# nebula-beta/MonocularSfM

Measured on AMD Instinct MI355X. Metric: descriptor-pairs/sec (and image-pairs/sec); match-index bit-parity vs CPU, higher is better.
Workload: dtype f32

## Files before the change

### include/msfm_match.h

```cpp
#ifndef MSFM_MATCH_H
#define MSFM_MATCH_H

#include <stdint.h>

#ifdef __cplusplus
extern "C" {
#endif

#define MSFM_DIM 128
#define MSFM_MAX_IMAGES 10000

enum {
    MSFM_OK = 0,
    MSFM_E_INVALID = 1,
    MSFM_E_DEVICE = 2,
    MSFM_E_NOIMAGE = 3,
    MSFM_E_CAPACITY = 4,
    MSFM_E_STATE = 5
};

enum { MSFM_DTYPE_F32 = 0, MSFM_DTYPE_U8 = 1 };

enum {
    MSFM_ORDER_SSE4X4 = 0,
    MSFM_ORDER_AVX2_FMA = 1,
    MSFM_ORDER_AVX512_FMA = 3
};

typedef struct msfm_ctx msfm_ctx;

typedef struct msfm_match_params {
    float ratio;
    int cross_check;
    double max_distance;
} msfm_match_params;

typedef struct msfm_profile {
    double dist_kernel_ms;
    int dist_kernel_launches;
    double total_device_ms;
    int64_t descriptor_pairs;
    int64_t dist_algo_bytes;
    double approx_kernel_ms;
    int approx_kernel_launches;
    int prefilter_pairs;
    int fallback_pairs;
    int64_t candidates;
    int64_t prefilter_descriptor_pairs;
    int64_t exact_descriptor_pairs;
    int64_t tie_rows;
    double sweep2_ms;
    int sweep2_launches;
    int compacted_pairs;
    int64_t sweep2_descriptor_pairs;
    double verify_ms;
    int sub_batches;
    int tie_queue_regrows;
    int plan_regrows;
    int sweep1_i8_launches;
    int sweep1_q8_launches;
    int sweep1b_launches;
    double sweep1b_ms;
    int64_t sweep1b_descriptor_pairs;
    int64_t order_sensitive_rows;
    int demoted_pairs;
    int mixed_route_sub_batches;
    int memory_shrinks;
} msfm_profile;

int msfm_create(int device_ordinal, msfm_ctx** out_ctx);
void msfm_destroy(msfm_ctx* ctx);
const char* msfm_last_error(const msfm_ctx* ctx);
int msfm_device_info(const msfm_ctx* ctx, char* name, int name_cap, int* cu_count, int* clock_mhz);
int msfm_set_accum_order(msfm_ctx* ctx, int order);
int msfm_set_prefilter(msfm_ctx* ctx, int enable);
int msfm_get_profile(const msfm_ctx* ctx, msfm_profile* out);
int msfm_set_limits(msfm_ctx* ctx, int max_pairs_per_batch, int64_t scratch_bytes);
int msfm_set_pipeline(msfm_ctx* ctx, int min_sub_batches);

int msfm_upload_image(msfm_ctx* ctx, int image_id, const void* desc, int n, int dim, int dtype);
int msfm_subset_image(msfm_ctx* ctx, int src_image_id, int dst_image_id, const int32_t* rows, int count);
int msfm_image_rows(const msfm_ctx* ctx, int image_id, int* out_n);
int msfm_clear_images(msfm_ctx* ctx);
int msfm_finalize_store(msfm_ctx* ctx);
int msfm_store_info(const msfm_ctx* ctx, int64_t* out_device_bytes, int64_t* out_rows, int64_t* out_pending_images);

int msfm_match_pair(msfm_ctx* ctx, int id1, int id2, float ratio, int cross_check,
                    double max_distance, int32_t* out_qt, float* out_dist, int* out_count);

int msfm_match_pairs(msfm_ctx* ctx, const int32_t* pairs, int n_pairs,
                     const msfm_match_params* params, int64_t* out_offsets);
int msfm_fetch_matches(msfm_ctx* ctx, int32_t* out_qt, float* out_dist);
int msfm_fetch_order_certificate(msfm_ctx* ctx, int32_t* out_sensitive_rows);
int msfm_view_matches(msfm_ctx* ctx, const int32_t** out_qt, const float** out_dist, int64_t* out_count);
int msfm_fetch_matches_device(msfm_ctx* ctx, int32_t* d_out_qt, float* d_out_dist);

typedef struct msfm_chunk {
    int first_pair;
    int n_pairs;
    int64_t count;
    const int64_t* offsets;
    const int32_t* qt;
    const float* dist;
    const int32_t* d_qt;
    const float* d_dist;
    const int32_t* sensitive_rows;
} msfm_chunk;
struct msfm_verify_params;
int msfm_match_pairs_begin(msfm_ctx* ctx, const int32_t* pairs, int n_pairs, const msfm_match_params* params,
                           int geometric_verification, const struct msfm_verify_params* verify);
int msfm_match_pairs_next(msfm_ctx* ctx, msfm_chunk* out);
int msfm_match_pairs_end(msfm_ctx* ctx);
typedef struct msfm_memory {
    int64_t device_free, device_total;
    int64_t store, inbox, scratch, results_device;
    int64_t page_locked_host;
} msfm_memory;
int msfm_memory_info(msfm_ctx* ctx, msfm_memory* out);
int msfm_read_device(msfm_ctx* ctx, void* host_dst, const void* device_src, int64_t bytes);

typedef struct msfm_verify_params {
    double threshold;
    double confidence;
    int max_iters;
    unsigned long long seed;
} msfm_verify_params;
int msfm_upload_keypoints(msfm_ctx* ctx, int image_id, const float* kpts, int n, int stride_floats);

#define MSFM_VERIFY_FUNDAMENTAL 0
#define MSFM_VERIFY_ESSENTIAL 1
#define MSFM_VERIFY_HOMOGRAPHY 2
typedef struct msfm_camera {
    double fx, fy, cx, cy, k1, k2, p1, p2;
} msfm_camera;
int msfm_set_verification_model(msfm_ctx* ctx, int model, const msfm_camera* camera);
int msfm_get_verification_stats(const msfm_ctx* ctx, int64_t* hypotheses_solved, int* rounds);

int msfm_set_model_selection(msfm_ctx* ctx, int enable, double h_ratio);
int msfm_fetch_model_selection(msfm_ctx* ctx, int32_t* out_model, int32_t* out_n_epipolar, int32_t* out_n_homography);

typedef struct msfm_two_view_params {
    int32_t min_num_inliers;
    int32_t reserved;
    double tri_max_error;
    double tri_min_angle;
} msfm_two_view_params;
typedef struct msfm_two_view_record {
    int32_t valid;
    int32_t reserved;
    double R[9];
// ... 238 lines not shown
```

### monocularsfm_amd/_lib.py

```python
import ctypes as C
import os

import numpy as np

_HERE = os.path.dirname(os.path.abspath(__file__))
LIB_PATH = os.path.join(_HERE, "csrc", "libmsfm_match.so")
if os.environ.get("MSFM_LIBRARY"):
    LIB_PATH = os.path.abspath(os.environ["MSFM_LIBRARY"])

OK, E_INVALID, E_DEVICE, E_NOIMAGE, E_CAPACITY, E_STATE = range(6)
DTYPE_F32, DTYPE_U8 = 0, 1
ORDER_SSE4X4, ORDER_AVX2_FMA, ORDER_AVX512_FMA = 0, 1, 3
MAX_IMAGES = 10000
DIM = 128

EXPORTS = [
    "msfm_create", "msfm_destroy", "msfm_last_error", "msfm_device_info", "msfm_set_accum_order", "msfm_set_prefilter",
    "msfm_get_profile", "msfm_upload_image", "msfm_image_rows", "msfm_clear_images",
    "msfm_match_pair", "msfm_match_pairs", "msfm_fetch_matches", "msfm_knn2_pair",
    "msfm_topscale_select", "msfm_pair_id", "msfm_pair_from_id", "msfm_swap_image_pair",
    "msfm_version", "msfm_upload_keypoints", "msfm_match_pairs_verified", "msfm_subset_image", "msfm_view_matches", "msfm_set_limits", "msfm_fetch_matches_device",
    "msfm_fetch_order_certificate", "msfm_set_pipeline", "msfm_device_count", "msfm_finalize_store", "msfm_store_info",
    "msfm_match_pairs_begin", "msfm_match_pairs_next", "msfm_read_device", "msfm_memory_info", "msfm_match_pairs_end",
    "msfm_train_vocabulary", "msfm_set_vocabulary", "msfm_image_words", "msfm_retrieve_pairs", "msfm_get_retrieval_profile",
# ... 87 lines not shown
    _fields_ = [(k, C.c_int64) for k in ("images", "eligible", "refined", "rejected_by_inliers", "iterations", "observations",
                                         "points_reposed", "points_lost", "points_gained")] + \
               [(k, C.c_double) for k in ("cost_before", "cost_after", "refine_ms", "prepare_ms")]


def reposed(points):
    return (np.asarray(points)["status"] & TRI_REPOSED) != 0


def succeeded(points):
    want = TRI_POINT | TRI_ERROR_OK | TRI_ANGLE_OK
    return (np.asarray(points)["status"] & want) == want


REG_ATTEMPTED, REG_POSE, REG_SUCCEEDED, REG_REFINED = 1, 2, 4, 8
REGISTRATION = np.dtype([("image_id", "<i4"), ("status", "<i4"), ("n_correspondences", "<i4"), ("n_inliers", "<i4"), ("hypotheses", "<i4"),
                         ("reserved", "<i4"), ("R", "<f8", (9,)), ("t", "<f8", (3,)), ("mean_residual", "<f8")])


class RegisterParams(C.Structure):
    _fields_ = [("max_error", C.c_double), ("confidence", C.c_double), ("max_iters", C.c_int32), ("min_inliers", C.c_int32),
                ("refine_iters", C.c_int32), ("reserved", C.c_int32)]


class RegisterStats(C.Structure):
    _fields_ = [("images", C.c_int32), ("attempted", C.c_int32), ("succeeded", C.c_int32), ("rounds", C.c_int32),
                ("correspondences", C.c_int64), ("hypotheses", C.c_int64), ("device_bytes", C.c_int64), ("register_ms", C.c_double)]


def registered(records):
    return (np.asarray(records)["status"] & REG_SUCCEEDED) != 0


def registered_poses(records, poses=None):
    out = dict(poses) if poses else {}
    for r in np.asarray(records)[registered(records)]:
        out[int(r["image_id"])] = (r["R"].reshape(3, 3).copy(), r["t"].copy())
    return out


def camera_struct(camera):
    keys = ("fx", "fy", "cx", "cy", "k1", "k2", "p1", "p2")
    vals = [camera.get(k, 0.0) for k in keys] if isinstance(camera, dict) else list(camera) + [0.0] * (8 - len(camera))
    return Camera(*[float(v) for v in vals[:8]])


def pose_table(poses):
    ids = np.asarray(sorted(int(i) for i in poses), np.int32)
    tab = np.zeros(max(len(ids), 1), POSE_RT)
    for k, i in enumerate(ids):
        if poses[int(i)] is None:
            continue
        R, t = poses[int(i)]
        tab[k]["valid"] = 1
        tab[k]["R"] = np.asarray(R, np.float64).reshape(9)
        tab[k]["t"] = np.asarray(t, np.float64).reshape(3)
    return ids, tab[:len(ids)]


class MatchParams(C.Structure):
    _fields_ = [("ratio", C.c_float), ("cross_check", C.c_int), ("max_distance", C.c_double)]


class Camera(C.Structure):
    _fields_ = [(k, C.c_double) for k in ("fx", "fy", "cx", "cy", "k1", "k2", "p1", "p2")]


class VerifyParams(C.Structure):
    _fields_ = [("threshold", C.c_double), ("confidence", C.c_double), ("max_iters", C.c_int), ("seed", C.c_ulonglong)]


class Profile(C.Structure):
    _fields_ = [("dist_kernel_ms", C.c_double), ("dist_kernel_launches", C.c_int),
                ("total_device_ms", C.c_double), ("descriptor_pairs", C.c_int64),
                ("dist_algo_bytes", C.c_int64), ("approx_kernel_ms", C.c_double),
                ("approx_kernel_launches", C.c_int), ("prefilter_pairs", C.c_int), ("fallback_pairs", C.c_int),
                ("candidates", C.c_int64), ("prefilter_descriptor_pairs", C.c_int64),
                ("exact_descriptor_pairs", C.c_int64), ("tie_rows", C.c_int64),
                ("sweep2_ms", C.c_double), ("sweep2_launches", C.c_int), ("compacted_pairs", C.c_int),
                ("sweep2_descriptor_pairs", C.c_int64), ("verify_ms", C.c_double),
                ("sub_batches", C.c_int), ("tie_queue_regrows", C.c_int), ("plan_regrows", C.c_int),
                ("sweep1_i8_launches", C.c_int), ("sweep1_q8_launches", C.c_int), ("sweep1b_launches", C.c_int),
                ("sweep1b_ms", C.c_double), ("sweep1b_descriptor_pairs", C.c_int64), ("order_sensitive_rows", C.c_int64),
                ("demoted_pairs", C.c_int), ("mixed_route_sub_batches", C.c_int), ("memory_shrinks", C.c_int)]


class Chunk(C.Structure):
    _fields_ = [("first_pair", C.c_int), ("n_pairs", C.c_int), ("count", C.c_int64), ("offsets", C.POINTER(C.c_int64)),
                ("qt", C.POINTER(C.c_int32)), ("dist", C.POINTER(C.c_float)), ("d_qt", C.c_void_p), ("d_dist", C.c_void_p),
                ("sensitive_rows", C.POINTER(C.c_int32))]


class Memory(C.Structure):
    _fields_ = [(k, C.c_int64) for k in ("device_free", "device_total", "store", "inbox", "scratch", "results_device", "page_locked_host")]


class RetrievalParams(C.Structure):
    _fields_ = [("num_words", C.c_int), ("train_iters", C.c_int), ("train_rows", C.c_int64)]


class RetrievalProfile(C.Structure):
    _fields_ = [("train_ms", C.c_double), ("train_iterations", C.c_int), ("assign_ms", C.c_double), ("score_ms", C.c_double),
                ("topk_ms", C.c_double), ("rows", C.c_int64), ("num_words", C.c_int)]


class MsfmError(RuntimeError):
    def __init__(self, code, msg):
        super().__init__("msfm error %d: %s" % (code, msg))
        self.code = code


_lib = None


def load():
    global _lib
    if _lib is not None:
        return _lib
    if not os.path.exists(LIB_PATH):
        raise ImportError(
            "%s is missing: the HIP extension is not built. Run `python -c 'import __graft_entry__ as g; "
            "g.build()'` (or `make -C monocularsfm_amd/csrc`). There is no CPU fallback." % LIB_PATH)
    L = C.CDLL(LIB_PATH)
    vp, ip, fp = C.c_void_p, C.POINTER(C.c_int32), C.POINTER(C.c_float)
    L.msfm_create.argtypes = [C.c_int, C.POINTER(vp)]
    L.msfm_destroy.argtypes = [vp]
    L.msfm_destroy.restype = None
    L.msfm_last_error.argtypes = [vp]
    L.msfm_last_error.restype = C.c_char_p
    L.msfm_device_info.argtypes = [vp, C.c_char_p, C.c_int, C.POINTER(C.c_int), C.POINTER(C.c_int)]
    L.msfm_set_accum_order.argtypes = [vp, C.c_int]
    L.msfm_set_prefilter.argtypes = [vp, C.c_int]
    L.msfm_get_profile.argtypes = [vp, C.POINTER(Profile)]
    L.msfm_set_limits.argtypes = [vp, C.c_int, C.c_int64]
    L.msfm_set_pipeline.argtypes = [vp, C.c_int]
    L.msfm_upload_image.argtypes = [vp, C.c_int, vp, C.c_int, C.c_int, C.c_int]
    L.msfm_image_rows.argtypes = [vp, C.c_int, C.POINTER(C.c_int)]
    L.msfm_subset_image.argtypes = [vp, C.c_int, C.c_int, ip, C.c_int]
    L.msfm_clear_images.argtypes = [vp]
    try:
        L.msfm_finalize_store.argtypes = [vp]
        L.msfm_store_info.argtypes = [vp, C.POINTER(C.c_int64), C.POINTER(C.c_int64), C.POINTER(C.c_int64)]
        L.msfm_match_pairs_begin.argtypes = [vp, ip, C.c_int, C.POINTER(MatchParams), C.c_int, C.POINTER(VerifyParams)]
        L.msfm_match_pairs_next.argtypes = [vp, C.POINTER(Chunk)]
        L.msfm_read_device.argtypes = [vp, vp, vp, C.c_int64]
        L.msfm_memory_info.argtypes = [vp, C.POINTER(Memory)]
        L.msfm_match_pairs_end.argtypes = [vp]
    except AttributeError:
        pass
    L.msfm_match_pair.argtypes = [vp, C.c_int, C.c_int, C.c_float, C.c_int, C.c_double, ip, fp, C.POINTER(C.c_int)]
    L.msfm_match_pairs.argtypes = [vp, ip, C.c_int, C.POINTER(MatchParams), C.POINTER(C.c_int64)]
    L.msfm_fetch_matches.argtypes = [vp, ip, fp]
    L.msfm_view_matches.argtypes = [vp, C.POINTER(ip), C.POINTER(fp), C.POINTER(C.c_int64)]
    L.msfm_fetch_matches_device.argtypes = [vp, vp, vp]
    L.msfm_fetch_order_certificate.argtypes = [vp, ip]
    L.msfm_upload_keypoints.argtypes = [vp, C.c_int, fp, C.c_int, C.c_int]
    L.msfm_match_pairs_verified.argtypes = [vp, ip, C.c_int, C.POINTER(MatchParams), C.POINTER(VerifyParams),
                                            C.POINTER(C.c_int64)]
    L.msfm_knn2_pair.argtypes = [vp, C.c_int, C.c_int, ip, fp, fp, ip, fp, fp]
    L.msfm_topscale_select.argtypes = [fp, C.c_int, C.c_int, ip, C.POINTER(C.c_int)]
    L.msfm_pair_id.argtypes = [C.c_int, C.c_int, ip]
    L.msfm_pair_from_id.argtypes = [C.c_int32, C.POINTER(C.c_int), C.POINTER(C.c_int)]
    L.msfm_swap_image_pair.argtypes = [C.c_int, C.c_int]
    L.msfm_version.restype = C.c_char_p
    try:
        L.msfm_device_count.argtypes = []
        L.msfm_device_count.restype = C.c_int
# ... 540 lines not shown
```

### monocularsfm_amd/csrc/msfm_batch.hip.h

```cpp
#pragma once
namespace {
struct Batch {
    std::vector<PairDesc> pairs;
    std::vector<PfPair> pf;
    std::vector<int> id1, id2;
    std::vector<int> item_base;
    size_t n_items = 0, items_per_xcd = 0;
    long long rp_elems = 0, cp_elems = 0, kf_elems = 0, kr_elems = 0, out_elems = 0, cand_elems = 0;
    int max_npad = 0;
    int64_t desc_pairs = 0;
    int64_t algo_bytes = 0;
    MsfmRoute route;
    std::vector<CandList> dense_lists;
    std::vector<VerifyPair> verify_pairs;
};

void build_items(Batch& b, int path, const std::vector<char>* only = nullptr, std::vector<int>* base_out = nullptr, size_t* per_out = nullptr) {
    std::vector<int> order(b.pairs.size());
    for (size_t p = 0; p < order.size(); ++p) order[p] = (int)p;
    if (b.id2.size() == b.pairs.size())
        std::stable_sort(order.begin(), order.end(), [&](int x, int y) { return b.id2[(size_t)x] < b.id2[(size_t)y]; });
    std::vector<int>& base = base_out ? *base_out : b.item_base;
    base.assign(b.pairs.size(), -1);
    long long n = 0;
// ... 67 lines not shown
    pp.b_c = b.c;
    const bool scales_ok = a.nrm_max <= 8.f * b.nrm_max && b.nrm_max <= 8.f * a.nrm_max;
    pp.use = (ctx->prefilter && pd.valid && a.pf_safe && b.pf_safe && scales_ok) ? 1 : 0;
    pd.path = pp.use;
    return MSFM_OK;
}

int prepare_batch_images(msfm_ctx* ctx, Batch& b, const PruneParams& prune) {
    const size_t P = b.pairs.size();
    std::vector<MsfmRoutePair> rp(P);
    for (size_t p = 0; p < P; ++p) {
        const Image &ia = ctx->images[(size_t)b.id1[p]], &ib = ctx->images[(size_t)b.id2[p]];
        rp[p] = MsfmRoutePair{b.pairs[p].valid != 0, b.pf[p].use != 0, ia.is_u8, ib.is_u8, ia.q8 != nullptr, ib.q8 != nullptr, b.pairs[p].n1, b.pairs[p].n2};
    }
    b.route = msfm_route(ctx->route_knobs(), prune.prune, prune.ratio, rp);
    std::vector<int> wide, panel;
    for (size_t p = 0; p < P; ++p) {
        if (!b.pairs[p].valid) continue;
        const bool brute = !b.pf[p].use || b.pairs[p].path == 0;
        if (brute || b.route.kind != kRouteI8) {
            wide.push_back(b.id1[p]);
            wide.push_back(b.id2[p]);
        }
        if (brute) {
            panel.push_back(b.id1[p]);
            panel.push_back(b.id2[p]);
        }
    }
    auto uniq = [](std::vector<int>& v) {
        std::sort(v.begin(), v.end());
        v.erase(std::unique(v.begin(), v.end()), v.end());
    };
    uniq(wide);
    uniq(panel);
    bool need = false;
    for (int id : wide) need |= ctx->images[(size_t)id].n > 0 && !ctx->images[(size_t)id].rawp;
    for (int id : panel) need |= ctx->images[(size_t)id].n > 0 && (!ctx->images[(size_t)id].panel || ctx->images[(size_t)id].panel_order != ctx->order);
    if (need) {
        const int rc = ensure_forms(ctx, wide, panel);
        if (rc != MSFM_OK) return rc;
    }
    for (size_t p = 0; p < P; ++p) {
        const Image& ia = ctx->images[(size_t)b.id1[p]];
        const Image& ib = ctx->images[(size_t)b.id2[p]];
        PairDesc& pd = b.pairs[p];
        PfPair& pp = b.pf[p];
        pd.a_panel = ia.panel;
        pd.b_panel = ib.panel;
        pd.a_rawp = ia.rawp;
        pd.b_rawp = ib.rawp;
        pp.a_h = ia.h16;
        pp.b_h = ib.h16;
        pp.a_nrm = ia.nrm;
        pp.b_nrm = ib.nrm;
    }
    return MSFM_OK;
}

void assign_common(Batch& b) {
    for (auto& pd : b.pairs) {
        pd.kf_off = b.kf_elems;
        pd.kr_off = b.kr_elems;
        pd.out_off = b.out_elems;
        if (!pd.valid) continue;
        b.kf_elems += pd.n1pad;
        b.kr_elems += pd.n2pad;
        b.out_elems += pd.n1;
        b.desc_pairs += (int64_t)pd.n1 * pd.n2;
        b.algo_bytes += ((int64_t)pd.n1 + pd.n2) * kDim * 4 + ((int64_t)pd.n1 + pd.n2) * 12;
        b.max_npad = std::max(b.max_npad, std::max(pd.n1pad, pd.n2pad));
    }
    for (auto& pd : b.pairs) pd.kr_off += b.kf_elems;
}

void assign_partials(Batch& b, int path, int target_items) {
    b.rp_elems = b.cp_elems = 0;
    long long total_ablocks = 0;
    for (auto& pd : b.pairs)
        if (pd.valid && pd.path == path) total_ablocks += (path == 1 ? pd.a_blocks256 : pd.a_blocks);
    const int rmult = 1;
    for (auto& pd : b.pairs) {
        if (!pd.valid || pd.path != path) continue;
        pd.ranges = 1;
        if (total_ablocks > 0 && total_ablocks < target_items) {
            long long r = (target_items + total_ablocks - 1) / total_ablocks;
            pd.ranges = (int)std::max<long long>(1, std::min<long long>(r, pd.b_tiles));
        }
        pd.rp_off = b.rp_elems;
        pd.cp_off = b.cp_elems;
        b.rp_elems += (long long)pd.ranges * rmult * pd.n1pad;
        b.cp_elems += (long long)(path == 1 ? pd.a_blocks256 : pd.a_blocks) * pd.n2pad;
    }
}

hipEvent_t get_event(msfm_ctx* ctx, size_t i) {
    while (ctx->ev_pool.size() <= i) {
        hipEvent_t e;
        if (hipEventCreate(&e) != hipSuccess) return nullptr;
        ctx->ev_pool.push_back(e);
    }
    return ctx->ev_pool[i];
}

__global__ void fill_segs_kernel(FillSegs segs) {
    MSFM_TAIL_PRIO();
    const unsigned long long tid = (unsigned long long)blockIdx.x * blockDim.x + threadIdx.x, nt = (unsigned long long)gridDim.x * blockDim.x;
    for (int k = 0; k < segs.n; ++k) {
        const FillSeg e = segs.s[k];
        const unsigned w = e.value * 0x01010101u;
        const unsigned long long n16 = e.bytes >> 4;
        uint4* p16 = reinterpret_cast<uint4*>(e.p);
        for (unsigned long long i = tid; i < n16; i += nt) p16[i] = make_uint4(w, w, w, w);
        for (unsigned long long i = (n16 << 4) + tid; i < e.bytes; i += nt) reinterpret_cast<unsigned char*>(e.p)[i] = (unsigned char)e.value;
    }
}

struct FillBatch {
    FillSegs segs = {};
    unsigned long long bytes = 0;
    std::vector<FillSegs> full;
    void add(void* p, size_t n, unsigned value) {
        if (!p || n == 0) return;
        if (segs.n == kFillSegs) {
            full.push_back(segs);
            segs = FillSegs{};
        }
        segs.s[segs.n++] = FillSeg{p, (unsigned long long)n, value & 255u};
        bytes += n;
    }
    hipError_t launch(hipStream_t stream) {
        if (segs.n) full.push_back(segs);
        const unsigned grid = (unsigned)std::max<unsigned long long>(1, std::min<unsigned long long>(256, (bytes + 65535) / 65536));
        for (const FillSegs& f : full) hipLaunchKernelGGL(fill_segs_kernel, dim3(grid), dim3(256), 0, stream, f);
        full.clear();
        segs = FillSegs{};
        bytes = 0;
        return hipGetLastError();
    }
};

int upload_pair_tables(msfm_ctx* ctx, Batch& b, int path, const std::vector<PfPair>* pfq, FillBatch& fills, const std::vector<PfPair>* pf16 = nullptr,
                       const std::vector<int>* item_base16 = nullptr, size_t per16 = 0) {
    const size_t P = b.pairs.size();
    const int slot = path == 1 ? 0 : 2;
    UploadPlan up;
    up.add(SC.d_pairs, b.pairs.data(), P * sizeof(PairDesc));
    up.add(SC.d_pf, b.pf.data(), P * sizeof(PfPair));
    if (pfq) up.add(SC.d_pfq, pfq->data(), P * sizeof(PfPair));
    if (pf16) up.add(SC.d_pf16, pf16->data(), P * sizeof(PfPair));
    if (item_base16) up.add(SC.d_item_base16, item_base16->data(), item_base16->size() * 4);
    up.add(SC.d_item_base, b.item_base.data(), b.item_base.size() * 4);
    HIPCHK(ctx, up.place_and_copy(SC.d_up[slot], SC.h_up[slot], SC.stream));
    HIPCHK(ctx, SC.d_items.ensure(std::max<size_t>(1, b.n_items) * sizeof(WorkItem)));
    fills.add(SC.d_items.p, b.n_items * sizeof(WorkItem), 0xff);
    if (item_base16 && per16) {
        HIPCHK(ctx, SC.d_items16.ensure(per16 * 8 * sizeof(WorkItem)));
        fills.add(SC.d_items16.p, per16 * 8 * sizeof(WorkItem), 0xff);
    }
    HIPCHK(ctx, fills.launch(SC.stream));
    if (b.n_items == 0) return MSFM_OK;
    hipLaunchKernelGGL(build_items_kernel, dim3((unsigned)P), dim3(64), 0, SC.stream, (const PairDesc*)SC.d_pairs.as<PairDesc>(),
                       (const int*)SC.d_item_base.as<int>(), path, (int)b.items_per_xcd, SC.d_items.as<WorkItem>());
    HIPCHK(ctx, hipGetLastError());
    if (item_base16 && per16) {
        hipLaunchKernelGGL(build_items_kernel, dim3((unsigned)P), dim3(64), 0, SC.stream, (const PairDesc*)SC.d_pairs.as<PairDesc>(),
                           (const int*)SC.d_item_base16.as<int>(), path, (int)per16, SC.d_items16.as<WorkItem>());
        HIPCHK(ctx, hipGetLastError());
    }
    return MSFM_OK;
}

struct CompactPlan {
    std::vector<PlanGroup> groups;
    std::vector<int> member_group;
    std::vector<int> gmembers;
    std::vector<int> member_pair;
    std::vector<PlanPair> ppair;
    long long rows_ub = 0;
    long long rows_ub_all_bits = 0;
    int pairs = 0;
};

void build_compact_plan(msfm_ctx* ctx, const Batch& b, CompactPlan& cp, bool no_ranges) {
    const size_t P = b.pairs.size();
    cp.ppair.assign(P, PlanPair{-1, 0, 0, 0});
    static thread_local std::vector<int> dense;
    dense.assign((size_t)kSlots, -1);
    std::vector<int> img_slot;
    auto dense_of = [&](int slot) {
        if (dense[(size_t)slot] < 0) {
            dense[(size_t)slot] = (int)img_slot.size();
            img_slot.push_back(slot);
        }
        return dense[(size_t)slot];
    };
    std::vector<int> fwd_group_of_img, rev_group0_of_img;
    std::vector<int>& member_group = cp.member_group;
    for (size_t p = 0; p < P; ++p) {
        const PairDesc& pd = b.pairs[p];
        const PfPair& pp = b.pf[p];
        if (!pd.valid || !pp.use) continue;
        ++cp.pairs;
        const int di = dense_of(b.id1[p]), dj = dense_of(b.id2[p]);
        const size_t need = img_slot.size();
        if (fwd_group_of_img.size() < need) {
            fwd_group_of_img.resize(need, -1);
            rev_group0_of_img.resize(need, -1);
        }
        if (fwd_group_of_img[(size_t)dj] < 0) {
            fwd_group_of_img[(size_t)dj] = (int)cp.groups.size();
            PlanGroup g = {};
            g.b_h = pp.b_h;
            g.b_nrm = pp.b_nrm;
            g.b_c = pp.b_c;
            g.a_c = pp.a_c;
            g.b_h0 = pp.b_h0;
            g.b_n2 = pp.b_n2;
            g.dir = 0;
            g.bt_begin = 0;
            g.bt_end = pd.b_tiles;
            g.n2 = pd.n2;
            g.n2pad = pd.n2pad;
            g.b_tiles = pd.b_tiles;
            g.ranges = 1;
            cp.groups.push_back(g);
        }
        cp.ppair[p].fwd_member = (int)cp.member_pair.size();
        cp.member_pair.push_back((int)p);
        member_group.push_back(fwd_group_of_img[(size_t)dj]);
        cp.rows_ub += pd.n1;
        const int nb = pd.a_blocks256, gshift = (nb + 31) / 32, bits = (nb + gshift - 1) / gshift;
        if (rev_group0_of_img[(size_t)di] < 0) {
            rev_group0_of_img[(size_t)di] = (int)cp.groups.size();
            for (int bit = 0; bit < bits; ++bit) {
                PlanGroup g = {};
                g.b_h = pp.a_h;
                g.b_nrm = pp.a_nrm;
                g.b_c = pp.a_c;
                g.a_c = pp.b_c;
                g.b_h0 = pp.a_h0;
                g.b_n2 = pp.a_n2;
                g.dir = 1;
                g.bt_begin = std::min(pd.a_blocks, bit * gshift * (kPfWgRows / kBM));
                g.bt_end = std::min(pd.a_blocks, (bit + 1) * gshift * (kPfWgRows / kBM));
                g.n2 = pd.n1;
                g.n2pad = pd.n1pad;
                g.b_tiles = pd.a_blocks;
                g.ranges = 1;
                cp.groups.push_back(g);
            }
        }
        cp.ppair[p].rev_member0 = (int)cp.member_pair.size();
        cp.ppair[p].rev_bits = bits;
        for (int bit = 0; bit < bits; ++bit) {
            cp.member_pair.push_back((int)p);
            member_group.push_back(rev_group0_of_img[(size_t)di] + bit);
        }
        cp.rows_ub += pd.n2;
        cp.rows_ub_all_bits += (long long)pd.n1 + (long long)pd.n2 * bits;
    }
    const size_t G = cp.groups.size(), M = cp.member_pair.size();
    for (size_t m = 0; m < M; ++m) cp.groups[(size_t)member_group[m]].count += 1;
    int at = 0;
    for (size_t g = 0; g < G; ++g) {
        cp.groups[g].first = at;
        at += cp.groups[g].count;
        cp.groups[g].count = 0;
    }
    cp.gmembers.assign(M, 0);
    for (size_t m = 0; m < M; ++m) {
        PlanGroup& g = cp.groups[(size_t)member_group[m]];
        cp.gmembers[(size_t)(g.first + g.count++)] = (int)m;
    }
    const long long target = 4LL * ctx->cu_count;
    if ((long long)G < target && !no_ranges)
        for (PlanGroup& g : cp.groups) {
            const long long r = (target + (long long)G - 1) / (long long)G;
            g.ranges = (int)std::max<long long>(1, std::min<long long>(r, g.bt_end - g.bt_begin));
        }
}

constexpr size_t kHsTotals = 2 * sizeof(PlanSummary), kHsOverflow = kHsTotals + 16;

struct PrefilterLaunch {
    msfm_ctx* ctx;
    Batch& b;
    size_t ev_base;
    PruneParams prune;
    size_t P = 0;
    HostClock hc;
    const MsfmRoute& route;
    std::vector<PfPair> pfq, pf16;
    long long dense_cand = 0;
    std::vector<int> item_base16;
    size_t per16 = 0;
    long long kn = 1;
    hipEvent_t e0 = nullptr, e1 = nullptr, e2 = nullptr, e3 = nullptr;
    dim3 block, mgrid;
    unsigned sweep_grid = 8;
    const PairDesc* dp = nullptr;
    const PfPair* dpf = nullptr;
    float* tuv = nullptr;
    unsigned* colmask = nullptr;
    size_t n_lists = 0;
    const CandList* dl = nullptr;
    CompactPlan cp;
    size_t G = 0, M = 0;
    long long rows_cap = 0, cand_cap = 0, items_cap = 0;
    const PlanPair* dpp = nullptr;
    PlanCounts pc = {};
    PlanOut po = {};

    PrefilterLaunch(msfm_ctx* c, Batch& batch, size_t ev, PruneParams pr) : ctx(c), b(batch), ev_base(ev), prune(pr), route(batch.route) {}

    int apply_route() {
        P = b.pairs.size();
        hc = HostClock();
        SC.pf_pending = PfPending{};
        assign_partials(b, 1, 4 * ctx->cu_count);
        SC.prof.demoted_pairs += route.demoted_pairs;
        SC.pf_pending.refine = route.kind == kRouteQ8Refine;
        dense_cand = 0;
        for (size_t p = 0; p < P; ++p) {
            b.pf[p].tu_off = b.pairs[p].kf_off;
            b.pf[p].tv_off = b.pairs[p].kr_off;
            b.pf[p].cand_off = 0;
            b.pf[p].cand_cap = 0;
            if (!route.compact() && b.pairs[p].valid && b.pf[p].use) {
                b.pf[p].cand_off = dense_cand;
                b.pf[p].cand_cap = 16 * (b.pairs[p].n1 + b.pairs[p].n2) + 2048;
                dense_cand += b.pf[p].cand_cap;
                SC.pf_pending.dense_swept += (long long)b.pairs[p].n1pad * b.pairs[p].n2;
            }
        }
        pfq.clear(), pf16.clear();
        if (route.q8()) pfq = b.pf;
        for (size_t p = 0; p < P && (route.kind == kRouteI8 || route.q8()); ++p) {
            if (!b.pairs[p].valid || !b.pf[p].use) continue;
            PfPair& pp = route.q8() ? pfq[p] : b.pf[p];
            pp.use = route.q8() ? route.twin[p] : 1;
            if (!pp.use) continue;
            const Image &ia = ctx->images[b.id1[p]], &ib = ctx->images[b.id2[p]];
            pp.i8 = 1;
            if (route.q8()) {
                pp.a_h = reinterpret_cast<const _Float16*>(ia.q8);
                pp.b_h = reinterpret_cast<const _Float16*>(ib.q8);
                pp.a_nrm = ia.nrm_q8, pp.b_nrm = ib.nrm_q8;
                pp.a_c = ia.err_q8_max, pp.b_c = ib.err_q8_max;
                pp.a_h0 = ia.h0_q8, pp.b_h0 = ib.h0_q8;
                pp.a_err = ia.err_q8, pp.b_err = ib.err_q8;
            } else {
                pp.a_h = reinterpret_cast<const _Float16*>(ia.i8);
                pp.b_h = reinterpret_cast<const _Float16*>(ib.i8);
                pp.a_nrm = ia.nrm_i8, pp.b_nrm = ib.nrm_i8;
                pp.a_nrm_max = ia.nrm_i8_max, pp.b_nrm_max = ib.nrm_i8_max;
                pp.a_c = pp.b_c = 0.f;
                pp.a_h0 = ia.h0_i8, pp.b_h0 = ib.h0_i8;
                pp.a_n2 = ia.n2_i8, pp.b_n2 = ib.n2_i8;
            }
        }
        if (route.kind == kRouteQ8Mixed) {
            pf16 = b.pf;
            for (size_t p = 0; p < P; ++p)
                if (route.twin[p]) pf16[p].use = 0, b.pairs[p].cp_off *= 2;
        }
        return MSFM_OK;
    }

    int build_and_upload() {
        item_base16.clear();
        per16 = 0;
        build_items(b, 1);
        if (b.n_items == 0) return MSFM_OK;
        if (route.kind == kRouteQ8Mixed) {
            std::vector<char> only(P, 0);
            for (size_t p = 0; p < P; ++p) only[p] = (b.pairs[p].valid && b.pf[p].use && !route.twin[p]) ? 1 : 0;
            build_items(b, 1, &only, &item_base16, &per16);
    }
    kn = std::max<long long>(1, b.kf_elems + b.kr_elems);
    HIPCHK(ctx, SC.d_rp_s0.ensure(std::max<long long>(1, b.rp_elems) * 4));
    HIPCHK(ctx, SC.d_rp_s1.ensure(std::max<long long>(1, b.rp_elems) * 4));
    HIPCHK(ctx, SC.d_cp_s0.ensure(std::max<long long>(1, b.cp_elems) * ((route.kind == kRouteI8 || route.kind == kRouteQ8Direct) ? 4 : 8)));
    HIPCHK(ctx, SC.d_tu.ensure(kn * 4));
    HIPCHK(ctx, SC.d_colmask.ensure(kn * 4));
    HIPCHK(ctx, SC.d_best.ensure(kn * 8));
    HIPCHK(ctx, SC.d_second.ensure(kn * 8));
    HIPCHK(ctx, SC.d_overflow.ensure(P));
    HIPCHK(ctx, SC.d_totals.ensure(128));
    FillBatch fills;
    if (!route.compact()) {
        fills.add(SC.d_best.p, (size_t)kn * 8, 0xff);
        fills.add(SC.d_second.p, (size_t)kn * 8, 0xff);
    }
    fills.add(SC.d_totals.p, 128, 0);
    fills.add(SC.d_overflow.p, P, 0);
    const int rc = upload_pair_tables(ctx, b, 1, route.q8() ? &pfq : nullptr, fills, route.kind == kRouteQ8Mixed ? &pf16 : nullptr,
                                        route.kind == kRouteQ8Mixed ? &item_base16 : nullptr, per16);
    if (rc != MSFM_OK) return rc;
    return MSFM_OK;
    }

    int launch_sweep1() {
        e0 = get_event(ctx, ev_base), e1 = get_event(ctx, ev_base + 1);
        e2 = get_event(ctx, ev_base + 2), e3 = get_event(ctx, ev_base + 3);
        if (!e0 || !e1 || !e2 || !e3) return fail(ctx, MSFM_E_DEVICE, "hipEventCreate failed");
        block = dim3(kPfThreads);
        sweep_grid = (unsigned)std::max(8, (ctx->cu_count / 8) * 8);
        dp = SC.d_pairs.as<PairDesc>();
        dpf = SC.d_pf.as<PfPair>();
        tuv = SC.d_tu.as<float>();
        colmask = SC.d_colmask.as<unsigned>();
        hc.lap("sweep-1 setup + uploads");
        if (ctx->last_sweep1 && ctx->last_sweep1 != ctx->cur)
            HIPCHK(ctx, hipStreamWaitEvent(SC.stream, ctx->last_sweep1->sweep1_done, 0));
        for (Scratch& other : ctx->sc)
            if (&other != ctx->cur && other.sweep2_recorded && other.seq + 2 <= SC.seq)
                HIPCHK(ctx, hipStreamWaitEvent(SC.stream, other.sweep2_done, 0));
        HIPCHK(ctx, hipEventRecord(e0, SC.stream));
        if (route.kind == kRouteI8 || route.q8())
            hipLaunchKernelGGL(sweep_i8_kernel<1>, dim3(std::min<unsigned>(sweep_grid, (unsigned)b.n_items)), dim3(kI8Threads), kI8LdsBytes, SC.stream, dp,
                               route.q8() ? (const PfPair*)SC.d_pfq.as<PfPair>() : dpf,
                               SC.d_items.as<WorkItem>(), SC.d_rp_s0.as<float>(), SC.d_rp_s1.as<float>(), SC.d_cp_s0.as<float>(),
                               (const float*)nullptr, (int2*)nullptr, (unsigned long long*)nullptr, (const int*)nullptr, (int)b.n_items, (int*)nullptr,
                               (int*)nullptr);
        else
            hipLaunchKernelGGL(sweep_kernel<1>, dim3(std::min<unsigned>(sweep_grid, (unsigned)b.n_items)), block, kPfLdsBytes, SC.stream, dp, dpf,
                               SC.d_items.as<WorkItem>(), SC.d_rp_s0.as<float>(), SC.d_rp_s1.as<float>(),
                               SC.d_cp_s0.as<float>(), (float*)nullptr, (const float*)nullptr, (const float*)nullptr,
                               (int2*)nullptr, (unsigned long long*)nullptr, (const int*)nullptr, (int)b.n_items, (int*)nullptr);
        HIPCHK(ctx, hipGetLastError());
        if (route.kind == kRouteQ8Mixed && per16) {
            hipLaunchKernelGGL(sweep_kernel<1>, dim3(std::min<unsigned>(sweep_grid, (unsigned)(per16 * 8))), block, kPfLdsBytes, SC.stream, dp,
                               (const PfPair*)SC.d_pf16.as<PfPair>(), SC.d_items16.as<WorkItem>(), SC.d_rp_s0.as<float>(), SC.d_rp_s1.as<float>(),
                               SC.d_cp_s0.as<float>(), (float*)nullptr, (const float*)nullptr, (const float*)nullptr,
                               (int2*)nullptr, (unsigned long long*)nullptr, (const int*)nullptr, (int)(per16 * 8), (int*)nullptr);
            HIPCHK(ctx, hipGetLastError());
            SC.prof.mixed_route_sub_batches += 1;
    }
    DBGSYNC(ctx, "sweep_kernel<1>");
    HIPCHK(ctx, hipEventRecord(e1, SC.stream));
    HIPCHK(ctx, hipEventRecord(SC.sweep1_done, SC.stream));
    SC.sweep1_recorded = true;
    ctx->last_sweep1 = ctx->cur;
    SC.prof.approx_kernel_launches += 1;
    if (route.kind == kRouteI8 || route.q8()) SC.prof.sweep1_i8_launches += 1;
    if (route.q8()) SC.prof.sweep1_q8_launches += 1;
    mgrid = dim3((unsigned)((b.max_npad + 255) / 256), (unsigned)P);
    if (!route.compact()) {
        hipLaunchKernelGGL(pf_thresholds_kernel, mgrid, dim3(256), 0, SC.stream, dp, dpf, SC.d_rp_s0.as<float>(),
                           SC.d_rp_s1.as<float>(), SC.d_cp_s0.as<float>(), (unsigned*)nullptr, tuv, tuv, prune, PlanCounts{}, 0);
        HIPCHK(ctx, hipGetLastError());
        DBGSYNC(ctx, "pf_thresholds_kernel");
    }
    hc.lap("launch sweep 1 (+ thresholds)");
    return MSFM_OK;
    }

    int plan_buffers() {
        cp = CompactPlan{};
        const bool refine = route.kind == kRouteQ8Refine;
        build_compact_plan(ctx, b, cp, refine);
        G = cp.groups.size(), M = cp.member_pair.size();
        n_lists = G;
        long long max_ranges = 1;
        for (const PlanGroup& g : cp.groups) max_ranges = std::max<long long>(max_ranges, g.ranges);
        const long long ub = refine ? cp.rows_ub_all_bits : cp.rows_ub;
        long long rows_have = (long long)std::min(std::min(SC.d_cmp_tu.cap / 4, SC.d_live_idx.cap / 4), std::min(SC.d_row_pair.cap / 4, SC.d_row_src.cap / 8));
        if (route.kind == kRouteI8) rows_have = std::min<long long>(rows_have, (long long)(SC.d_cmp_n2.cap / 4));
        if (refine) rows_have = std::min<long long>(rows_have, (long long)std::min(SC.d_cmp_s0.cap / 4, SC.d_cmp_s1.cap / 4));
        long long cand_have = (long long)(SC.d_cand.cap / sizeof(int2));
        if (route.kind == kRouteI8) cand_have = std::min<long long>(cand_have, (long long)(SC.d_cand_val.cap / 4));
        const long long items_have = (long long)(SC.d_vitems.cap / sizeof(WorkItem)) / 8 * 8;
        const MsfmPlanRoom room = msfm_plan_room(ub, refine ? cp.rows_ub_all_bits * 5 / 32 : cp.rows_ub * 5 / 16, (long long)G, max_ranges, kPfWgRows,
                                                 ctx->hint_rows_ub, ctx->cmp_rows_hint, ctx->cand_hint, ctx->items_hint, rows_have, cand_have, items_have);
        rows_cap = room.rows, cand_cap = room.cand, items_cap = room.items;
        SC.pf_pending.rows_ub = ub;
        HIPCHK(ctx, SC.d_gtot.ensure(std::max<size_t>(1, G) * 4));
        HIPCHK(ctx, SC.d_grow0.ensure((4 * std::max<size_t>(1, G) + 8) * 8));
        HIPCHK(ctx, SC.d_cnt.ensure(std::max<size_t>(1, M) * 4));
        HIPCHK(ctx, SC.d_mrow.ensure(std::max<size_t>(1, M) * 8));
        HIPCHK(ctx, SC.d_summary.ensure(sizeof(PlanSummary)));
        HIPCHK(ctx, SC.d_vpairs.ensure(std::max<size_t>(1, G) * sizeof(PairDesc)));
        HIPCHK(ctx, SC.d_vpf.ensure(std::max<size_t>(1, G) * sizeof(PfPair)));
        HIPCHK(ctx, SC.d_lists.ensure(std::max<size_t>(1, G) * sizeof(CandList)));
        HIPCHK(ctx, SC.d_vitems.ensure((size_t)items_cap * sizeof(WorkItem)));
        HIPCHK(ctx, SC.d_cmp_tu.ensure((size_t)rows_cap * 4));
        HIPCHK(ctx, SC.d_live_idx.ensure((size_t)rows_cap * 4));
        HIPCHK(ctx, SC.d_row_pair.ensure((size_t)rows_cap * 4));
        HIPCHK(ctx, SC.d_row_src.ensure((size_t)rows_cap * 8));
        HIPCHK(ctx, SC.d_cand.ensure((size_t)cand_cap * sizeof(int2)));
        if (route.kind == kRouteI8) {
            HIPCHK(ctx, SC.d_cand_val.ensure((size_t)cand_cap * 4));
            HIPCHK(ctx, SC.d_cmp_n2.ensure((size_t)rows_cap * 4));
        }
        HIPCHK(ctx, SC.d_cand_count.ensure(std::max<size_t>(1, G) * 8));
        {
            UploadPlan up;
            up.add(SC.d_groups, cp.groups.data(), G * sizeof(PlanGroup));
            up.add(SC.d_gmembers, cp.gmembers.data(), M * 4);
            up.add(SC.d_member_pair, cp.member_pair.data(), M * 4);
            up.add(SC.d_member_group, cp.member_group.data(), M * 4);
            up.add(SC.d_ppair, cp.ppair.data(), P * sizeof(PlanPair));
            HIPCHK(ctx, up.place_and_copy(SC.d_up[1], SC.h_up[1], SC.stream));
            FillBatch fb;
            fb.add(SC.d_gtot.p, std::max<size_t>(1, G) * 4, 0);
            fb.add(SC.d_cnt.p, std::max<size_t>(1, M) * 4, 0);
            fb.add(SC.d_vpairs.p, std::max<size_t>(1, G) * sizeof(PairDesc), 0);
            fb.add(SC.d_vpf.p, std::max<size_t>(1, G) * sizeof(PfPair), 0);
            fb.add(SC.d_lists.p, std::max<size_t>(1, G) * sizeof(CandList), 0);
            fb.add(SC.d_summary.p, sizeof(PlanSummary), 0);
            fb.add(SC.d_vitems.p, (size_t)items_cap * sizeof(WorkItem), 0xff);
            fb.add(SC.d_row_src.p, (size_t)rows_cap * 8, 0);
            fb.add(SC.d_cand_count.p, std::max<size_t>(1, G) * 8, 0);
            HIPCHK(ctx, fb.launch(SC.stream));
        }
        hc.lap("plan tables + uploads");
        dpp = SC.d_ppair.as<PlanPair>();
        pc = PlanCounts{dpp, (const int*)SC.d_member_group.as<int>(), SC.d_cnt.as<int>(), SC.d_gtot.as<int>()};
        HIPCHK(ctx, SC.d_summary_a.ensure(sizeof(PlanSummary)));
        po = PlanOut{};
        po.vpairs = SC.d_vpairs.as<PairDesc>();
        po.vpf = SC.d_vpf.as<PfPair>();
        po.lists = SC.d_lists.as<CandList>();
        po.items = SC.d_vitems.as<WorkItem>();
        po.grow0 = SC.d_grow0.as<long long>();
        po.gpos = SC.d_grow0.as<long long>() + std::max<size_t>(1, G);
        po.fwd_items_x = SC.d_grow0.as<long long>() + 4 * std::max<size_t>(1, G);
        po.summary = SC.d_summary.as<PlanSummary>();
        po.row_src = SC.d_row_src.as<const _Float16*>();
        po.zero_row = ctx->d_zero_row.as<_Float16>();
        po.live_idx = SC.d_live_idx.as<int>();
        po.row_pair = SC.d_row_pair.as<int>();
        po.rows_cap = rows_cap;
        po.cand_cap = cand_cap;
        po.items_cap = items_cap;
        po.cmp_tu = SC.d_cmp_tu.as<float>();
        po.cmp_n2 = route.kind == kRouteI8 ? SC.d_cmp_n2.as<int>() : nullptr;
        return MSFM_OK;
    }

    int launch_plan(PlanSummary* summary, int norms_only) {
        po.summary = summary;
        hipLaunchKernelGGL(pf_plan_scan_kernel, dim3(1), dim3(64), 0, SC.stream, SC.d_groups.as<PlanGroup>(), (int)G,
                           (const int*)SC.d_gtot.as<int>(), po);
        HIPCHK(ctx, hipGetLastError());
        DBGSYNC(ctx, "pf_plan_scan_kernel");
        if (G > 0)
            hipLaunchKernelGGL(pf_plan_write_kernel, dim3((unsigned)((G + 63) / 64)), dim3(64), 0, SC.stream, SC.d_groups.as<PlanGroup>(), (int)G,
                               (const int*)SC.d_gtot.as<int>(), po);
        HIPCHK(ctx, hipGetLastError());
        DBGSYNC(ctx, "pf_plan_write_kernel");
        if (G > 0)
            hipLaunchKernelGGL(pf_member_rows_kernel, dim3((unsigned)((G + 3) / 4)), dim3(256), 0, SC.stream, SC.d_groups.as<PlanGroup>(), (int)G,
                               (const int*)SC.d_gmembers.as<int>(), (const int*)SC.d_cnt.as<int>(),
                               (const long long*)SC.d_grow0.as<long long>(), SC.d_mrow.as<long long>());
        HIPCHK(ctx, hipGetLastError());
        DBGSYNC(ctx, "pf_member_rows_kernel");
        hipLaunchKernelGGL(pf_assign_kernel, dim3((unsigned)(2 * P), (unsigned)((b.max_npad + kAssignChunk - 1) / kAssignChunk)), dim3(256), 0,
                           SC.stream, dp, dpf, dpp, (const float*)tuv,
                           (const unsigned*)colmask, (const long long*)SC.d_mrow.as<long long>(), SC.d_cnt.as<int>(),
                           SC.d_live_idx.as<int>(), SC.d_row_pair.as<int>(), SC.d_cmp_tu.as<float>(),
                           SC.d_row_src.as<const _Float16*>(), route.kind == kRouteI8 ? kI8RowBytes / 2 : kPfRowHalfs,
                           SC.d_best.as<unsigned long long>(), SC.d_second.as<unsigned long long>(), norms_only,
                           route.kind == kRouteI8 ? SC.d_cmp_n2.as<int>() : (int*)nullptr);
        HIPCHK(ctx, hipGetLastError());
        DBGSYNC(ctx, "pf_assign_kernel");
        return MSFM_OK;
    }

    int launch_route_q() {
        hipLaunchKernelGGL(pf_prune_q8_kernel, mgrid, dim3(256), 0, SC.stream, dp, dpf, (const PfPair*)SC.d_pfq.as<PfPair>(),
                           (const float*)SC.d_rp_s0.as<float>(), (const float*)SC.d_rp_s1.as<float>(), (const float*)SC.d_cp_s0.as<float>(),
                           colmask, tuv, prune, pc, ctx->q8_level / 255.f, route.kind == kRouteQ8Refine ? 0 : 1);
        HIPCHK(ctx, hipGetLastError());
        DBGSYNC(ctx, "pf_prune_q8_kernel");
        if (route.kind == kRouteQ8Refine) {
            HIPCHK(ctx, hipMemsetAsync(SC.d_summary_a.p, 0, sizeof(PlanSummary), SC.stream));
            int rc = launch_plan(SC.d_summary_a.as<PlanSummary>(), 1);
            if (rc != MSFM_OK) return rc;
            HIPCHK(ctx, SC.d_cmp_s0.ensure((size_t)rows_cap * 4));
            HIPCHK(ctx, SC.d_cmp_s1.ensure((size_t)rows_cap * 4));
            hipEvent_t e4 = get_event(ctx, ev_base + 6), e5 = get_event(ctx, ev_base + 7);
            if (!e4 || !e5) return fail(ctx, MSFM_E_DEVICE, "hipEventCreate failed");
            HIPCHK(ctx, hipEventRecord(e4, SC.stream));
            hipLaunchKernelGGL(sweep_kernel<4>, dim3(sweep_grid), block, kPfLdsBytes, SC.stream,
                               (const PairDesc*)SC.d_vpairs.as<PairDesc>(), (const PfPair*)SC.d_vpf.as<PfPair>(),
                               (const WorkItem*)SC.d_vitems.as<WorkItem>(), SC.d_cmp_s0.as<float>(), SC.d_cmp_s1.as<float>(), (float*)nullptr,
                               (float*)nullptr, (const float*)SC.d_cmp_tu.as<float>(), (const float*)nullptr, (int2*)nullptr,
                               (unsigned long long*)nullptr, (const int*)&SC.d_summary_a.as<PlanSummary>()->n_items, 0,
                               SC.d_totals.as<int>() + 8);
            HIPCHK(ctx, hipGetLastError());
            DBGSYNC(ctx, "sweep_kernel<4>");
            HIPCHK(ctx, hipEventRecord(e5, SC.stream));
            SC.prof.sweep1b_launches += 1;
            if (G > 0)
                hipLaunchKernelGGL(q8_scatter_kernel, dim3(16, (unsigned)std::min<size_t>(G, 65535)), dim3(256), 0, SC.stream, dp,
                                   (const PairDesc*)SC.d_vpairs.as<PairDesc>(), (const CandList*)SC.d_lists.as<CandList>(),
                                   (const PlanGroup*)SC.d_groups.as<PlanGroup>(), (int)G, (const long long*)SC.d_grow0.as<long long>(),
                                   (const float*)SC.d_cmp_s0.as<float>(), (const float*)SC.d_cmp_s1.as<float>(),
                                   SC.d_rp_s0.as<float>(), SC.d_rp_s1.as<float>(), SC.d_cp_s0.as<float>());
            HIPCHK(ctx, hipGetLastError());
            DBGSYNC(ctx, "q8_scatter_kernel");
            FillBatch fb;
            fb.add(SC.d_gtot.p, std::max<size_t>(1, G) * 4, 0);
            fb.add(SC.d_cnt.p, std::max<size_t>(1, M) * 4, 0);
            fb.add(SC.d_vpairs.p, std::max<size_t>(1, G) * sizeof(PairDesc), 0);
            fb.add(SC.d_vpf.p, std::max<size_t>(1, G) * sizeof(PfPair), 0);
            fb.add(SC.d_lists.p, std::max<size_t>(1, G) * sizeof(CandList), 0);
            fb.add(SC.d_vitems.p, (size_t)items_cap * sizeof(WorkItem), 0xff);
            fb.add(SC.d_row_src.p, (size_t)rows_cap * 8, 0);
            fb.add(SC.d_totals.p, 64, 0);
            HIPCHK(ctx, fb.launch(SC.stream));
        }
        return MSFM_OK;
    }

    int launch_compact_sweep2() {
        if (route.kind != kRouteQ8Direct)
            hipLaunchKernelGGL(pf_thresholds_kernel, mgrid, dim3(256), 0, SC.stream, dp, route.kind == kRouteQ8Mixed ? (const PfPair*)SC.d_pf16.as<PfPair>() : dpf,
                               SC.d_rp_s0.as<float>(), SC.d_rp_s1.as<float>(), SC.d_cp_s0.as<float>(), colmask, tuv, tuv, prune, pc,
                               route.kind == kRouteQ8Refine ? 1 : 0);
        HIPCHK(ctx, hipGetLastError());
        DBGSYNC(ctx, "pf_thresholds_kernel");
        const int rc = launch_plan(SC.d_summary.as<PlanSummary>(), 0);
        if (rc != MSFM_OK) return rc;
        HIPCHK(ctx, hipEventRecord(e2, SC.stream));
        if (route.kind == kRouteI8)
            hipLaunchKernelGGL(sweep_i8_kernel<3>, dim3(sweep_grid), dim3(kI8Threads), kI8LdsBytes3, SC.stream,
                               (const PairDesc*)SC.d_vpairs.as<PairDesc>(), (const PfPair*)SC.d_vpf.as<PfPair>(),
                               (const WorkItem*)SC.d_vitems.as<WorkItem>(), (float*)nullptr, (float*)nullptr, (float*)nullptr,
                               (const float*)SC.d_cmp_tu.as<float>(), SC.d_cand.as<int2>(),
                               SC.d_cand_count.as<unsigned long long>(), (const int*)&SC.d_summary.as<PlanSummary>()->n_items, 0,
                               SC.d_totals.as<int>() + 8, SC.d_cand_val.as<int>());
        else
            hipLaunchKernelGGL(sweep_kernel<3>, dim3(sweep_grid), block, kPfLdsBytes, SC.stream,
                               (const PairDesc*)SC.d_vpairs.as<PairDesc>(), (const PfPair*)SC.d_vpf.as<PfPair>(),
                               (const WorkItem*)SC.d_vitems.as<WorkItem>(), (float*)nullptr, (float*)nullptr, (float*)nullptr,
                               (float*)nullptr, (const float*)SC.d_cmp_tu.as<float>(), (const float*)nullptr, SC.d_cand.as<int2>(),
                               SC.d_cand_count.as<unsigned long long>(), (const int*)&SC.d_summary.as<PlanSummary>()->n_items, 0,
                               SC.d_totals.as<int>() + 8);
        HIPCHK(ctx, hipGetLastError());
        DBGSYNC(ctx, "sweep_kernel<3>");
        SC.prof.sweep2_launches += 1;
        HIPCHK(ctx, hipEventRecord(e3, SC.stream));
        HIPCHK(ctx, hipEventRecord(SC.sweep2_done, SC.stream));
        SC.sweep2_recorded = true;
        dl = SC.d_lists.as<CandList>();
        SC.pf_pending.compact = true;
        SC.pf_pending.rows_cap = rows_cap;
        SC.pf_pending.cand_cap = cand_cap;
        SC.pf_pending.items_cap = items_cap;
        SC.pf_pending.compact_pairs = cp.pairs;
        return MSFM_OK;
    }

    int launch_dense_sweep2() {
        n_lists = P;
        std::vector<CandList>& lists = b.dense_lists;
        lists.resize(P);
        for (size_t p = 0; p < P; ++p)
            lists[p] = CandList{(int)p, 0, b.pf[p].cand_off, b.pf[p].cand_cap, 0, nullptr, nullptr};
        HIPCHK(ctx, SC.d_cand.ensure(std::max<long long>(1, dense_cand) * sizeof(int2)));
        HIPCHK(ctx, SC.d_cand_count.ensure(P * 8));
        HIPCHK(ctx, SC.d_lists.ensure(P * sizeof(CandList)));
        HIPCHK(ctx, hipMemsetAsync(SC.d_cand_count.p, 0, P * 8, SC.stream));
        HIPCHK(ctx, hipMemcpyAsync(SC.d_lists.p, lists.data(), P * sizeof(CandList), hipMemcpyHostToDevice, SC.stream));
        HIPCHK(ctx, hipEventRecord(e2, SC.stream));
        hipLaunchKernelGGL(sweep_kernel<2>, dim3(std::min<unsigned>(sweep_grid, (unsigned)b.n_items)), block, kPfLdsBytes, SC.stream, dp, dpf,
                           SC.d_items.as<WorkItem>(), (float*)nullptr, (float*)nullptr, (float*)nullptr, (float*)nullptr,
                           (const float*)tuv, (const float*)tuv, SC.d_cand.as<int2>(), SC.d_cand_count.as<unsigned long long>(),
                           (const int*)nullptr, (int)b.n_items, (int*)nullptr);
        HIPCHK(ctx, hipGetLastError());
        DBGSYNC(ctx, "sweep_kernel<2>");
        SC.prof.sweep2_launches += 1;
        HIPCHK(ctx, hipEventRecord(e3, SC.stream));
        HIPCHK(ctx, hipEventRecord(SC.sweep2_done, SC.stream));
        SC.sweep2_recorded = true;
        dl = SC.d_lists.as<CandList>();
        return MSFM_OK;
    }

    int launch_exact_and_finalize() {
        if (n_lists > 0) {
            const int wgs_per_xcd = std::max(1, ctx->cu_count / 8) * 8;
            const dim3 cgrid((unsigned)(8 * wgs_per_xcd));
            const unsigned long long* dcount = SC.d_cand_count.as<unsigned long long>();
#define MSFM_LAUNCH_EXACT(O)                                                                                             \
        hipLaunchKernelGGL(pf_exact_candidates_kernel<O>, cgrid, dim3(kExSpan), 0, SC.stream, dp, dl, dcount,                  \
                           (const int2*)SC.d_cand.as<int2>(), SC.d_best.as<unsigned long long>(), SC.d_second.as<unsigned long long>(), \
                           (int)n_lists, SC.d_totals.as<int>() + 16, (const int*)SC.d_cand_val.as<int>(), 0)
            if (route.kind == kRouteI8) MSFM_LAUNCH_EXACT(4);
            else if (ctx->order == MSFM_ORDER_SSE4X4) MSFM_LAUNCH_EXACT(0);
            else if (ctx->order == MSFM_ORDER_AVX2_FMA) MSFM_LAUNCH_EXACT(1);
            else MSFM_LAUNCH_EXACT(3);
#undef MSFM_LAUNCH_EXACT
            HIPCHK(ctx, hipGetLastError());
            DBGSYNC(ctx, "pf_exact_candidates_kernel");
    }
    if (!SC.keys_epilogue) {
        hipLaunchKernelGGL(pf_finalize_kernel, mgrid, dim3(256), 0, SC.stream, dp, dpf, (const float*)tuv, SC.d_best.as<unsigned long long>(),
                           SC.d_second.as<unsigned long long>(), SC.d_k_i0.as<int>(), SC.d_k_d0.as<float>(),
                           SC.d_k_d1.as<float>(), SC.d_fix_count.as<int>(), SC.d_fix_list.as<int4>(), SC.fix_cap_eff);
        HIPCHK(ctx, hipGetLastError());
        DBGSYNC(ctx, "pf_finalize_kernel");
    }
    if (n_lists > 0) {
        hipLaunchKernelGGL(pf_overflow_kernel, dim3((unsigned)((n_lists + 255) / 256)), dim3(256), 0, SC.stream, dl, (int)n_lists,
                           (const unsigned long long*)SC.d_cand_count.as<unsigned long long>(), (const PlanGroup*)SC.d_groups.as<PlanGroup>(),
                           (const int*)SC.d_gmembers.as<int>(), (const int*)SC.d_member_pair.as<int>(),
                           SC.d_overflow.as<unsigned char>(), SC.d_totals.as<unsigned long long>());
        HIPCHK(ctx, hipGetLastError());
    }
    SC.pf_pending.active = true;
    SC.pf_pending.n_lists = n_lists;
    SC.pf_pending.P = P;
    SC.pf_pending.ev_base = ev_base;
    hc.lap("launch sweep 2 .. finalize");
    return MSFM_OK;
    }

    int run() {
        int rc = apply_route();
        if (rc != MSFM_OK) return rc;
        rc = build_and_upload();
        if (rc != MSFM_OK || b.n_items == 0) return rc;
        rc = launch_sweep1();
        if (rc != MSFM_OK) return rc;
        if (route.compact()) {
            rc = plan_buffers();
            if (rc == MSFM_OK && route.q8()) rc = launch_route_q();
            if (rc == MSFM_OK) rc = launch_compact_sweep2();
        } else {
            rc = launch_dense_sweep2();
        }
        if (rc != MSFM_OK) return rc;
        return launch_exact_and_finalize();
    }
};

int run_prefilter(msfm_ctx* ctx, Batch& b, size_t ev_base, PruneParams prune) {
    PrefilterLaunch launch(ctx, b, ev_base, prune);
    return launch.run();
}

int finish_prefilter(msfm_ctx* ctx, Batch& b, std::vector<char>& force_exact, bool* retry) {
    *retry = false;
    PfPending& pe = SC.pf_pending;
    if (!pe.active) return MSFM_OK;
    pe.active = false;
    const char* hs = SC.h_summary.as<char>();
    PlanSummary sm = {};
    unsigned long long totals[2] = {0, 0};
    std::memcpy(totals, hs + kHsTotals, 16);
    float ms = 0.f;
    HIPCHK(ctx, hipEventElapsedTime(&ms, ctx->ev_pool[pe.ev_base], ctx->ev_pool[pe.ev_base + 1]));
    SC.prof.approx_kernel_ms += ms;
    HIPCHK(ctx, hipEventElapsedTime(&ms, ctx->ev_pool[pe.ev_base + 2], ctx->ev_pool[pe.ev_base + 3]));
    SC.prof.sweep2_ms += ms;
    if (std::getenv("MSFM_DEBUG_TIMING") && pe.compact) {
        PlanSummary d;
        std::memcpy(&d, hs, sizeof(PlanSummary));
        std::fprintf(stderr, "[msfm plan] ok %d, items %lld (room for %lld), compacted rows %lld (%lld; of at most %lld), candidate entries %lld (%lld), swept descriptor pairs %lld; sweep 1 %.3f ms, sweep 2 %.3f ms\n",
                     d.ok, d.items_needed, pe.items_cap, d.cmp_rows, pe.rows_cap, pe.rows_ub, d.cand_elems, pe.cand_cap, d.swept_desc_pairs, SC.prof.approx_kernel_ms, ms);
    }
    if (pe.compact) {
        std::memcpy(&sm, hs, sizeof(PlanSummary));
        ctx->cmp_rows_hint = sm.cmp_rows;
        ctx->items_hint = sm.items_needed;
        ctx->cand_hint = sm.cand_elems;
        ctx->hint_rows_ub = pe.rows_ub;
        if (pe.refine) {
            PlanSummary sa;
            std::memcpy(&sa, hs + sizeof(PlanSummary), sizeof(PlanSummary));
            ctx->cmp_rows_hint = std::max(ctx->cmp_rows_hint, sa.cmp_rows);
            ctx->items_hint = std::max(ctx->items_hint, sa.items_needed);
            ctx->cand_hint = std::max(ctx->cand_hint, sa.cand_elems);
            if (!sa.ok) sm.ok = 0;
            float ms1b = 0.f;
            HIPCHK(ctx, hipEventElapsedTime(&ms1b, ctx->ev_pool[pe.ev_base + 6], ctx->ev_pool[pe.ev_base + 7]));
            SC.prof.sweep1b_ms += ms1b;
            SC.prof.sweep1b_descriptor_pairs += sa.swept_desc_pairs;
        }
        if (!sm.ok) {
            SC.prof.plan_regrows += 1;
            *retry = true;
            return MSFM_OK;
        }
        SC.prof.sweep2_descriptor_pairs += sm.swept_desc_pairs;
    } else {
        SC.prof.sweep2_descriptor_pairs += pe.dense_swept;
    }
    const unsigned char* ov = reinterpret_cast<const unsigned char*>(hs + kHsOverflow);
    int n_over = 0;
    for (size_t p = 0; p < pe.P; ++p) {
        if (!b.pairs[p].valid || !b.pf[p].use) continue;
        if (ov[p]) {
            force_exact[p] = 1;
            ++n_over;
        }
    }
    if (n_over > 0) {
        SC.prof.fallback_pairs += n_over;
        *retry = true;
        return MSFM_OK;
    }
    SC.prof.candidates += (int64_t)totals[0];
    for (size_t p = 0; p < pe.P; ++p)
        if (b.pairs[p].valid && b.pf[p].use) {
            SC.prof.prefilter_pairs += 1;
            SC.prof.prefilter_descriptor_pairs += (int64_t)b.pairs[p].n1 * b.pairs[p].n2;
        }
    if (pe.compact) SC.prof.compacted_pairs += pe.compact_pairs;
    return MSFM_OK;
}

int run_exact(msfm_ctx* ctx, Batch& b, size_t ev_base) {
    const size_t P = b.pairs.size();
    assign_partials(b, 0, 4 * ctx->cu_count);
    build_items(b, 0);
    if (b.n_items == 0) return MSFM_OK;
    HIPCHK(ctx, SC.d_rp_s0.ensure(std::max<long long>(1, b.rp_elems) * 4));
    HIPCHK(ctx, SC.d_rp_i0.ensure(std::max<long long>(1, b.rp_elems) * 4));
    HIPCHK(ctx, SC.d_rp_s1.ensure(std::max<long long>(1, b.rp_elems) * 4));
    HIPCHK(ctx, SC.d_cp_s0.ensure(std::max<long long>(1, b.cp_elems) * 4));
    HIPCHK(ctx, SC.d_cp_i0.ensure(std::max<long long>(1, b.cp_elems) * 4));
    HIPCHK(ctx, SC.d_cp_s1.ensure(std::max<long long>(1, b.cp_elems) * 4));
    FillBatch fills;
    int rc = upload_pair_tables(ctx, b, 0, nullptr, fills);
    if (rc != MSFM_OK) return rc;
    hipEvent_t e0 = get_event(ctx, ev_base), e1 = get_event(ctx, ev_base + 1);
    if (!e0 || !e1) return fail(ctx, MSFM_E_DEVICE, "hipEventCreate failed");
    if (ctx->last_sweep1 && ctx->last_sweep1 != ctx->cur)
        HIPCHK(ctx, hipStreamWaitEvent(SC.stream, ctx->last_sweep1->sweep1_done, 0));
    HIPCHK(ctx, hipEventRecord(e0, SC.stream));
    const dim3 grid((unsigned)b.n_items), block(kThreads);
#define MSFM_LAUNCH_DIST(O)                                                                                               \
    hipLaunchKernelGGL(dist_top2_kernel<O>, grid, block, (O) == 3 ? kLdsBytesIdxStash : kLdsBytes, SC.stream, SC.d_pairs.as<PairDesc>(), SC.d_items.as<WorkItem>(), \
                       SC.d_rp_s0.as<float>(), SC.d_rp_i0.as<int>(), SC.d_rp_s1.as<float>(), SC.d_cp_s0.as<float>(),             \
                       SC.d_cp_i0.as<int>(), SC.d_cp_s1.as<float>())
    if (ctx->order == MSFM_ORDER_SSE4X4) MSFM_LAUNCH_DIST(0);
    else if (ctx->order == MSFM_ORDER_AVX2_FMA) MSFM_LAUNCH_DIST(1);
    else MSFM_LAUNCH_DIST(3);
#undef MSFM_LAUNCH_DIST
    HIPCHK(ctx, hipGetLastError());
    HIPCHK(ctx, hipEventRecord(e1, SC.stream));
    HIPCHK(ctx, hipEventRecord(SC.sweep1_done, SC.stream));
    SC.sweep1_recorded = true;
    ctx->last_sweep1 = ctx->cur;
    SC.prof.dist_kernel_launches += 1;
    for (auto& pd : b.pairs)
        if (pd.valid && pd.path == 0) SC.prof.exact_descriptor_pairs += (int64_t)pd.n1 * pd.n2;
    const dim3 mgrid((unsigned)((b.max_npad + 255) / 256), (unsigned)P);
    hipLaunchKernelGGL(merge_knn_kernel, mgrid, dim3(256), 0, SC.stream, SC.d_pairs.as<PairDesc>(),
                       SC.d_rp_s0.as<float>(), SC.d_rp_i0.as<int>(), SC.d_rp_s1.as<float>(),
                       SC.d_cp_s0.as<float>(), SC.d_cp_i0.as<int>(), SC.d_cp_s1.as<float>(),
                       SC.d_k_i0.as<int>(), SC.d_k_d0.as<float>(), SC.d_k_d1.as<float>(),
                       SC.d_fix_count.as<int>(), SC.d_fix_list.as<int4>(), SC.fix_cap_eff);
    HIPCHK(ctx, hipGetLastError());
    return MSFM_OK;
}

int run_knn(msfm_ctx* ctx, Batch& b, size_t ev_base, bool* exact_launched, PruneParams prune, bool need_fix, bool lists_only) {
    assign_common(b);
    SC.fix_cap_eff = need_fix ? ctx->fix_cap : 0;
    const long long kn = std::max<long long>(1, b.kf_elems + b.kr_elems);
    HIPCHK(ctx, SC.d_fix_count.ensure(4));
    HIPCHK(ctx, SC.d_fix_list.ensure((size_t)ctx->fix_cap * sizeof(int4)));
    HIPCHK(ctx, hipMemsetAsync(SC.d_fix_count.p, 0, 4, SC.stream));
    bool any_pf = false, any_exact = false;
    for (auto& pd : b.pairs) any_pf |= (pd.valid && pd.path == 1);
    for (auto& pd : b.pairs) any_exact |= (pd.valid && pd.path == 0);
// ... 105 lines not shown
```

### monocularsfm_amd/csrc/msfm_ctx.hip.h

```cpp
#pragma once
namespace {

struct AllocClock {
    double dev_ms = 0, pin_ms = 0, free_ms = 0;
    long long dev_bytes = 0, pin_bytes = 0;
    int dev_n = 0, pin_n = 0, free_n = 0;
    static double now() { return std::chrono::duration<double, std::milli>(std::chrono::steady_clock::now().time_since_epoch()).count(); }
};
inline AllocClock& alloc_clock() {
    static thread_local AllocClock c;
    return c;
}
inline hipError_t timed_malloc(void** p, size_t bytes) {
    const double t0 = AllocClock::now();
    const hipError_t e = hipMalloc(p, bytes);
    AllocClock& c = alloc_clock();
    c.dev_ms += AllocClock::now() - t0;
    c.dev_bytes += (long long)bytes;
    c.dev_n += 1;
    return e;
}
inline void timed_free(void* p) {
    const double t0 = AllocClock::now();
    (void)hipFree(p);
// ... 361 lines not shown
            if (!chunks[i].base) slot = (int)i;
        if (slot < 0) {
            chunks.push_back(StoreChunk{});
            slot = (int)chunks.size() - 1;
        }
        StoreChunk& c = chunks[(size_t)slot];
        const size_t want = std::max(bytes, min_chunk);
        hipError_t e = timed_malloc((void**)&c.base, want);
        if (e != hipSuccess) {
            c.base = nullptr;
            return e;
        }
        c.cap = want;
        c.used = 0;
        c.live = 0;
        cur = slot;
        return hipSuccess;
    }
    void* take(size_t bytes, int* chunk) {
        StoreChunk& c = chunks[(size_t)cur];
        const size_t at = (c.used + 255) & ~(size_t)255;
        if (at + bytes > c.cap) return nullptr;
        c.used = at + bytes;
        c.live += 1;
        *chunk = cur;
        return c.base + at;
    }
    void free_chunk(int i) {
        StoreChunk& c = chunks[(size_t)i];
        if (c.base) (void)hipFree(c.base);
        c = StoreChunk{};
        if (cur == i) cur = -1;
    }
    void drop(int& chunk) {
        if (chunk < 0) return;
        StoreChunk& c = chunks[(size_t)chunk];
        if (--c.live <= 0) {
            if (chunk == cur || recycle) c.used = 0, c.live = 0;
            else free_chunk(chunk);
        }
        chunk = -1;
    }
    size_t bytes() const {
        size_t s = 0;
        for (const StoreChunk& c : chunks) s += c.cap;
        return s;
    }
    void release_all() {
        for (size_t i = 0; i < chunks.size(); ++i) free_chunk((int)i);
        chunks.clear();
        cur = -1;
    }
};

constexpr int kSlots = 2 * MSFM_MAX_IMAGES + 2;
constexpr long long kDefaultScratchBytes = (long long)64 << 30;
constexpr int kDefaultMaxPairsPerBatch = 16384;
constexpr int kMaxPairsPerBatchLimit = 65535;
constexpr int kDefaultPipeline = 2;
constexpr double kDefaultTaper = 1.0;
constexpr int kInFlight = 3;
constexpr long long kMinPipelineCost = 15000000000LL;

}

struct PfPending {
    bool active = false, compact = false, refine = false;
    size_t n_lists = 0, P = 0;
    long long rows_cap = 0, cand_cap = 0, items_cap = 0;
    long long rows_ub = 0;
    int compact_pairs = 0;
    long long dense_swept = 0;
    size_t ev_base = 0;
};

struct Scratch {
    hipStream_t stream = nullptr;
    DevBuf d_up[3];
    PinnedBuf h_up[3];
    Ref d_pairs, d_pf, d_pfq, d_pf16, d_item_base, d_item_base16;
    Ref d_groups, d_gmembers, d_member_pair, d_member_group, d_ppair;
    DevBuf d_items;
    DevBuf d_rp_s0, d_rp_i0, d_rp_s1, d_cp_s0, d_cp_i0, d_cp_s1;
    DevBuf d_k_i0, d_k_d0, d_k_d1;
    DevBuf d_st_qt, d_st_d, d_counts, d_offsets, d_sens;
    DevBuf d_sub_qt, d_sub_d;
    PinnedBuf h_sub_qt, h_sub_d;
    DevBuf d_fix_count, d_fix_list;
    int fix_cap_eff = 0;
    bool keys_epilogue = false;
    DevBuf d_tu, d_tv, d_cand, d_cand_count, d_best, d_second;
    DevBuf d_cmp_tu, d_live_idx, d_row_pair, d_row_src, d_vpairs, d_vpf, d_vitems, d_lists, d_items16;
    DevBuf d_cmp_s0, d_cmp_s1, d_summary_a;
    DevBuf d_cand_val, d_cmp_n2;
    DevBuf d_colmask, d_gtot, d_grow0, d_cnt, d_mrow, d_summary, d_overflow, d_totals;
    PfPending pf_pending;
    PinnedBuf h_summary;
    PinnedBuf h_tail;
    DevBuf d_vf_pairs, d_vf_x1, d_vf_y1, d_vf_x2, d_vf_y2, d_vf_hyp, d_vf_best_it, d_vf_best_count, d_vf_flags,
        d_st2_qt, d_st2_d, d_counts2;
    DevBuf d_ve_x1, d_ve_y1, d_ve_x2, d_ve_y2, d_staged_state, d_staged_stats;
    DevBuf d_vs_records;
    DevBuf d_tv_records, d_tv_idx, d_tv_angles, d_tv_best_it;
    PinnedBuf h_tv;
    DevBuf d_tk_pairs;
    PinnedBuf h_tk_pairs;
    msfm_profile prof = {};
    hipEvent_t sweep1_done = nullptr;
    bool sweep1_recorded = false;
    hipEvent_t sweep2_done = nullptr;
    bool sweep2_recorded = false;
    long long seq = 0;
    void for_each_buf(void (*fn)(DevBuf&, void*), void* arg) {
        DevBuf* bufs[] = {&d_up[0], &d_up[1], &d_up[2], &d_items, &d_rp_s0, &d_rp_i0, &d_rp_s1, &d_cp_s0, &d_cp_i0, &d_cp_s1, &d_k_i0, &d_k_d0,
                          &d_k_d1, &d_st_qt, &d_st_d, &d_counts, &d_offsets, &d_sens, &d_sub_qt, &d_sub_d, &d_fix_count, &d_fix_list, &d_tu,
                          &d_tv, &d_cand, &d_cand_count, &d_best, &d_second, &d_cmp_tu, &d_live_idx, &d_row_pair, &d_row_src,
                          &d_vpairs, &d_vpf, &d_vitems, &d_lists, &d_colmask, &d_gtot, &d_grow0, &d_cnt, &d_mrow, &d_summary, &d_overflow,
                          &d_totals, &d_vf_pairs,
                          &d_vf_x1, &d_vf_y1, &d_vf_x2, &d_vf_y2, &d_vf_hyp, &d_vf_best_it, &d_vf_best_count, &d_vf_flags, &d_st2_qt,
                          &d_st2_d, &d_counts2, &d_ve_x1, &d_ve_y1, &d_ve_x2, &d_ve_y2, &d_staged_state, &d_staged_stats, &d_vs_records, &d_tv_records, &d_tv_idx, &d_tv_angles, &d_tv_best_it, &d_tk_pairs, &d_cmp_s0, &d_cmp_s1, &d_summary_a, &d_items16, &d_cand_val, &d_cmp_n2};
        for (DevBuf* b : bufs) fn(*b, arg);
    }
    long long device_bytes() {
        long long sum = 0;
        for_each_buf([](DevBuf& b, void* a) { *static_cast<long long*>(a) += (long long)b.cap; }, &sum);
        return sum;
    }
    void release_device() { for_each_buf([](DevBuf& b, void*) { b.release(); }, nullptr); }
    void release_all() {
        for_each_buf([](DevBuf& b, void*) { b.release(); }, nullptr);
        for (PinnedBuf& h : h_up) h.release();
        h_sub_qt.release();
        h_sub_d.release();
        h_summary.release();
        h_tail.release();
        h_tv.release();
        h_tk_pairs.release();
    }
};

struct MatchJob;

struct TrackSession {
    bool open = false;
    bool closed = false;
    bool finished = false;
    bool suppress = false;
    MsfmTrackNodes nd;
    std::vector<int> rank_of;
    int min_pair_matches = 0;
    bool add_only = false;
    DevBuf d_parent;
    DevBuf d_table;
    DevBuf d_base, d_ids;
    DevBuf r_offsets, r_img, r_idx, r_cons, r_tid;
    msfm_track_stats stats = {};
    DevBuf t_points, t_resid;
    bool tri_valid = false;
    DevBuf t_mask;
    bool mask_valid = false;
    msfm_camera tri_camera = {};
    msfm_triangulation_params tri_prm = {};
    std::vector<int32_t> tri_ids;
    std::vector<msfm_pose_rt> tri_poses;
    std::vector<msfm_pose_refinement> rp_records;
    bool rp_valid = false;
    DevBuf g_records, g_offsets, g_tid, g_inl, g_res;
    bool reg_valid = false;
    int reg_images = 0;
    long long reg_corr = 0;
    std::vector<std::pair<hipEvent_t, hipEvent_t>> ev_pending;
    std::vector<hipEvent_t> ev_free;
    bool declares(int id) const { return open && id >= 0 && id < (int)rank_of.size() && rank_of[(size_t)id] >= 0; }
    long long device_bytes() const {
        long long s = 0;
        for (const DevBuf* b : {&d_parent, &d_table, &d_base, &d_ids, &r_offsets, &r_img, &r_idx, &r_cons, &r_tid}) s += (long long)b->cap;
        return s;
    }
    void release() {
        for (DevBuf* b : {&d_parent, &d_table, &d_base, &d_ids, &r_offsets, &r_img, &r_idx, &r_cons, &r_tid, &t_points, &t_resid, &t_mask, &g_records, &g_offsets, &g_tid, &g_inl, &g_res}) b->release();
        for (auto& e : ev_pending) {
            (void)hipEventDestroy(e.first);
            (void)hipEventDestroy(e.second);
        }
        for (hipEvent_t e : ev_free) (void)hipEventDestroy(e);
        ev_pending.clear();
        ev_free.clear();
        rank_of.clear();
        tri_ids.clear();
        tri_poses.clear();
        rp_records.clear();
        rp_valid = false;
        nd = MsfmTrackNodes{};
        stats = msfm_track_stats{};
        open = closed = finished = suppress = add_only = tri_valid = mask_valid = reg_valid = false;
    }
};

struct msfm_ctx {
    int device = 0;
    int order = MSFM_ORDER_SSE4X4;
    int cu_count = 0, clock_mhz = 0;
    char dev_name[256] = {0};
    std::vector<Image> images;
    std::string err;

    Scratch sc[kInFlight];
    Scratch* cur = &sc[0];
    Scratch* last_sweep1 = nullptr;
    DevBuf d_zero_row;
    StoreArena store;
    StoreArena inbox;
    std::vector<int> pending;
    size_t inbox_waiting = 0;
    bool store_async = false;
    PinnedBuf up_ring;
    CopyHelper copier;
    bool copy_helper = true;
    hipEvent_t up_ev[2] = {nullptr, nullptr};
    bool up_ev_recorded[2] = {false, false};
    unsigned up_seq = 0;
    DevBuf d_jobs, d_store_maxima;
    PinnedBuf h_jobs, h_store_maxima;
    PinnedPool pinned_pool;
    hipEvent_t jobs_ev = nullptr;
    size_t store_peak_bytes = 0;
    std::vector<OutSeg> out_segs;
    size_t out_used = 0;
    int fix_cap = 1 << 16;
    int max_pairs_per_batch = kDefaultMaxPairsPerBatch;
    long long scratch_bytes = 0;
    int last_hip_error = 0;
    long long budget_cached = 0;
    size_t budget_for_store = 0;
    long long budget_for_limit = 0;
    long long issue_seq = 0;
    double pipeline_taper = kDefaultTaper;
    int in_flight = kInFlight;
    int pipeline = kDefaultPipeline;
    int prefilter = 1;
    int byte_detect = 1;
    float q8_level = 0.f;
    int q8_direct = 1;
    int q8_route = 1;
    MsfmRouteKnobs route_knobs() const { return MsfmRouteKnobs{prefilter, q8_route, q8_direct, q8_level}; }
    DeferredFrees deferred;
    long long cmp_rows_hint = 0;
    long long hint_rows_ub = 0;
    long long items_hint = 0, cand_hint = 0;

    bool have_results = false;
    std::vector<int64_t> res_offsets;
    std::vector<int32_t> res_sens;
    GrowPinned res_qt, res_dist;
    size_t res_count = 0;

    msfm_profile prof = {};
    std::vector<hipEvent_t> ev_pool;
    MatchJob* job = nullptr;
    bool series_open = false;
    DevBuf ret_words, ret_cn;
    int ret_v = 0;
    msfm_retrieval_profile ret_prof = {};
    int verify_model = MSFM_VERIFY_FUNDAMENTAL;
    msfm_emat::Camera camera = {};
    long long staged_solved = 0;
    int staged_rounds = 0;
    bool model_select = false;
    double h_ratio = 0.7;
    std::vector<int32_t> sel_records;
    bool sel_valid = false;
    bool two_view = false;
    msfm_two_view_params tv_params = {100, 0, 2.0, 4.0};
    std::vector<msfm_two_view_record> tv_records;
    bool tv_valid = false;
    TrackSession tracks;
};

#define SC (*ctx->cur)

namespace {

int fail(msfm_ctx* ctx, int code, const std::string& msg) {
    if (ctx) ctx->err = msg;
    return code;
}
inline void note_hip_error(msfm_ctx* ctx, hipError_t e) {
    if (ctx) ctx->last_hip_error = (int)e;
}
inline void note_hip_error(const msfm_ctx*, hipError_t) {}

void after_api_exception(msfm_ctx* ctx, const char* text) noexcept;
#define MSFM_API_BEGIN(ctxp) \
    return msfm_guard([&](int, const char* t__) noexcept { after_api_exception(ctxp, t__); }, [&]() -> int {
#define MSFM_API_END \
    });

#define HIPCHK(ctx, call)                                                                     \
    do {                                                                                      \
        hipError_t e__ = (call);                                                              \
        if (e__ != hipSuccess) {                                                              \
            note_hip_error(ctx, e__);                                                         \
            return fail(ctx, MSFM_E_DEVICE,                                                   \
                        std::string(#call) + ": " + hipGetErrorString(e__));                  \
        }                                                                                     \
    } while (0)


struct HostClock {
    bool on = std::getenv("MSFM_DEBUG_TIMING") != nullptr;
    std::chrono::steady_clock::time_point t = std::chrono::steady_clock::now();
    void lap(const char* what) {
        if (!on) return;
        const auto n = std::chrono::steady_clock::now();
        std::fprintf(stderr, "[msfm host] %-28s %.3f ms\n", what, std::chrono::duration<double, std::milli>(n - t).count());
        t = n;
    }
};

#define DBGSYNC(ctx, name)                                                        \
    do {                                                                          \
        static const bool on__ = std::getenv("MSFM_DEBUG_SYNC") != nullptr;       \
        if (on__) {                                                               \
            std::fprintf(stderr, "[msfm] %s ...", name);                          \
            hipError_t e__ = hipStreamSynchronize((ctx)->cur->stream);                \
            std::fprintf(stderr, " %s\n", hipGetErrorString(e__));                \
        }                                                                         \
    } while (0)
// ... 3 lines not shown
```

### monocularsfm_amd/csrc/msfm_hostutil.h

```cpp
#pragma once
#include <vector>

#if defined(__HIPCC__)
#include <hip/hip_runtime.h>
#define MSFM_HD __host__ __device__ inline __attribute__((always_inline))
#else
#define MSFM_HD inline
#endif

MSFM_HD int msfm_cp_pack(int hi, bool hi_valid, int lo, bool lo_valid) {
    unsigned c = 255u;
    if (lo_valid) {
        const unsigned x = (unsigned)(hi - lo) + 16u;
        int e = 27 - __builtin_clz(x);
        unsigned m = (x + (1u << e) - 1u) >> e;
        e += (int)(m >> 5);
        m = (m >> 5) ? 16u : m;
        const unsigned code = ((unsigned)e << 4) | (m - 16u);
        c = code >= 255u ? 255u : code;
    }
    return hi_valid ? (int)(((unsigned)hi << 8) | c) : (int)0x80000000;
}
constexpr int kCpNone = -(1 << 23);
MSFM_HD int msfm_cp_hi(int code) { return code >> 8; }
MSFM_HD bool msfm_cp_has_second(int code) { return (code & 255) != 255; }
MSFM_HD int msfm_cp_gap(int code) { const int c = code & 255; return ((16 + (c & 15)) << (c >> 4)) - 16; }

inline std::vector<long long> msfm_pipeline_marks(long long total, long long n_sub, double taper) {
    std::vector<long long> marks;
    if (n_sub < 2) return marks;
    const double last = taper, first = 2.0 - last;
    double acc = 0.0;
    marks.push_back(0);
    for (long long k = 0; k < n_sub; ++k) {
        acc += first - (first - last) * (double)k / (double)(n_sub - 1);
        marks.push_back(k + 1 == n_sub ? total : (long long)((double)total * acc / (double)n_sub));
    }
    return marks;
}

inline long long msfm_pair_two_view_bytes(int n1, int n2) {
    if (n1 <= 0 || n2 <= 0) return 0;
    return 12LL * n1 + 148;
}

inline long long msfm_pair_scratch_bytes(int n1, int n2, int n1pad, int n2pad, int blocks128, int blocks512, int route,
                                         bool two_view = false) {
    if (n1 <= 0 || n2 <= 0) return 0;
    const long long slots = (long long)n1pad + n2pad;
    const long long common = (route == 3 ? 24LL : 36LL) * slots + 24LL * n1 + 1024 + (two_view ? msfm_pair_two_view_bytes(n1, n2) : 0);
    if (route == 0) return common + 12LL * n1pad + 12LL * (long long)blocks128 * n2pad;
    const long long partials = 8LL * n1pad + (route == 3 ? 4LL : 8LL) * (long long)blocks512 * n2pad;
    if (route == 2) return common + partials + 128LL * ((long long)n1 + n2) + 16384;
    const long long bits = blocks512 < 32 ? blocks512 : 32;
    const long long cmp_rows = ((long long)n1 + (long long)n2 * bits) / (route == 4 ? 8 : 16) + 1024;
    return common + partials + (route == 3 ? 120LL : 84LL) * cmp_rows;
}

constexpr float kQ8DirectMaxLevel = 0.625f;
struct MsfmRouteKnobs { int prefilter, q8_route, q8_direct; float q8_level; };
inline bool msfm_compact_sweep2(int prune, float ratio) { return prune != 0 && ratio > 0.f && ratio <= 0.95f; }
inline bool msfm_twin_route_on(const MsfmRouteKnobs& k) { return k.prefilter == 1 && k.q8_route != 0; }
inline bool msfm_fine_twins(const MsfmRouteKnobs& k) { return k.q8_direct == 2 || (k.q8_direct == 1 && k.q8_level <= kQ8DirectMaxLevel); }
inline bool msfm_byte_pair(bool a_is_u8, bool b_is_u8) { return a_is_u8 && b_is_u8; }

enum MsfmRouteKind {
    kRouteDense,
    kRouteFp16,
    kRouteI8,
    kRouteQ8Direct,
    kRouteQ8Mixed,
    kRouteQ8Refine,
};
struct MsfmRoute {
    MsfmRouteKind kind = kRouteDense;
    std::vector<char> twin;
    long long demoted_pairs = 0;
    bool compact() const { return kind != kRouteDense; }
    bool q8() const { return kind >= kRouteQ8Direct; }
};
struct MsfmRoutePair { bool valid, use, a_is_u8, b_is_u8, a_twin, b_twin; int n1, n2; };

inline MsfmRoute msfm_route(const MsfmRouteKnobs& k, int prune, float ratio, const std::vector<MsfmRoutePair>& pairs) {
    MsfmRoute r;
    r.twin.assign(pairs.size(), 0);
    if (!msfm_compact_sweep2(prune, ratio)) return r;
    r.kind = kRouteFp16;
    if (k.prefilter != 1) return r;
    long long rows = 0, n_pairs = 0, twin_pairs = 0, twin_rows = 0;
    bool bytes = true;
    for (const MsfmRoutePair& q : pairs) {
        if (!q.valid || !q.use) continue;
        bytes = bytes && msfm_byte_pair(q.a_is_u8, q.b_is_u8);
        rows += q.n1 + q.n2;
        n_pairs += 1;
        if (q.a_twin && q.b_twin) twin_pairs += 1, twin_rows += q.n1 + q.n2;
    }
    if (bytes) {
        r.kind = kRouteI8;
        return r;
    }
    const bool fine = msfm_fine_twins(k), mixed = twin_pairs < n_pairs;
    bool q8 = msfm_twin_route_on(k) && (!mixed || (fine && twin_pairs > 0 && 4 * twin_rows >= rows));
    if (q8 && k.q8_route < 2 && (twin_pairs == 0 || twin_rows < 2 * 1024 * twin_pairs)) q8 = false;
    if (q8) {
        r.kind = mixed ? kRouteQ8Mixed : (fine ? kRouteQ8Direct : kRouteQ8Refine);
        for (std::size_t p = 0; p < pairs.size(); ++p) r.twin[p] = pairs[p].valid && pairs[p].use && pairs[p].a_twin && pairs[p].b_twin;
        return r;
    }
    for (const MsfmRoutePair& q : pairs)
        if (q.valid && q.use && (msfm_byte_pair(q.a_is_u8, q.b_is_u8) ||
                                 (k.q8_route && q.a_twin && q.b_twin && (k.q8_route == 2 || q.n1 + q.n2 >= 2048))))
            r.demoted_pairs += 1;
    return r;
}

inline int msfm_scratch_route(const MsfmRouteKnobs& k, int prune, float ratio, bool use, bool a_is_u8, bool b_is_u8) {
    if (!use || k.prefilter == 0) return 0;
    if (!msfm_compact_sweep2(prune, ratio)) return 2;
    if (k.prefilter == 1 && msfm_byte_pair(a_is_u8, b_is_u8)) return 3;
    if (msfm_twin_route_on(k) && k.q8_level > 0.f && !msfm_fine_twins(k)) return 4;
    return 1;
}

struct MsfmPlanRoom { long long rows, cand, items; bool hinted; };
inline MsfmPlanRoom msfm_plan_room(long long ub, long long ub_prior, long long groups, long long max_ranges, int wg_rows,
                                   long long hint_ub, long long hint_rows, long long hint_cand, long long hint_items,
                                   long long have_rows, long long have_cand, long long have_items) {
    auto mx = [](long long a, long long b) { return a > b ? a : b; };
    const long long slack = (long long)wg_rows * groups + wg_rows;
    const bool hinted = hint_rows > 0 && hint_ub > 0 && ub <= 2 * hint_ub && 2 * ub >= hint_ub;
    const double s = hinted ? (double)ub / (double)hint_ub : 0.0;
    const long long h_rows = (long long)((double)hint_rows * s), h_cand = (long long)((double)hint_cand * s), h_items = (long long)((double)hint_items * s);
    const long long prior = mx(ub_prior, ub < (1LL << 21) ? ub : (1LL << 21));
    const long long rows_min = (hinted ? h_rows + h_rows / 8 : prior) + slack;
    MsfmPlanRoom r;
    r.hinted = hinted;
    r.rows = have_rows >= rows_min ? have_rows : mx(h_rows + h_rows / 2, prior) + slack;
    const long long cand_min = mx(8 * rows_min + 2048 * groups, h_cand);
    r.cand = have_cand >= cand_min ? have_cand : mx(8 * r.rows + 2048 * groups, h_cand);
    const long long items_min = mx(2 * ((rows_min / wg_rows + groups) * max_ranges + 64) / 8 * 8, (h_items + 64) / 8 * 8);
    r.items = have_items >= items_min ? have_items : mx(2 * ((r.rows / wg_rows + groups) * max_ranges + 64) / 8 * 8, (h_items + 64) / 8 * 8);
    return r;
}

inline unsigned long long msfm_pinned_piece_end(unsigned long long off) {
    const unsigned long long piece = 32ull << 20;
    if (off >= piece) return (off / piece + 1) * piece;
    unsigned long long end = 1ull << 20;
    while (end <= off) end *= 2;
    return end;
}

template <class AtomicMin>
MSFM_HD void msfm_fold_key(unsigned long long* best, unsigned long long* second, unsigned long long key, unsigned long long seen_best,
                           unsigned long long seen_second, AtomicMin amin) {
    if (key == seen_best) return;
    unsigned long long loser = key;
    if (key < seen_best) {
        const unsigned long long old = amin(best, key);
        if (old == key) return;
        loser = old > key ? old : key;
        if (loser == ~0ull) return;
    }
    if (loser < seen_second) (void)amin(second, loser);
}

MSFM_HD bool msfm_select_homography(int n_epipolar, int n_homography, double h_ratio) {
    return n_epipolar > 0 && (double)n_homography >= h_ratio * (double)n_epipolar;
}

MSFM_HD bool msfm_initial_candidate(int n_triangulated, double median_tri_angle, double mean_tri_angle, double mean_residual,
                                    int min_num_inliers, double tri_max_error, double tri_min_angle) {
    return n_triangulated >= min_num_inliers && median_tri_angle >= tri_min_angle && mean_tri_angle >= tri_min_angle &&
           mean_residual <= tri_max_error;
}
```

### monocularsfm_amd/csrc/msfm_kernels.hip.h

```cpp
#pragma once
#include <hip/hip_runtime.h>
#include <stdint.h>

#pragma clang fp contract(off)

namespace msfm {

constexpr int kDim = 128;
constexpr int kBM = 128;
constexpr int kBN = 128;
constexpr int kTM = 8;
constexpr int kTN = 4;
constexpr int kThreads = 512;
constexpr int kChunkPos = 32;
constexpr int kChunks = kDim / kChunkPos;
constexpr int kPanelFloats = kBM * kDim;
constexpr int kSlotFloats = kChunkPos * kBN;
constexpr int kWaveCols = kBN / 8;
constexpr int kWaveSlotFloats = kChunkPos * kWaveCols;
constexpr int kLdsA = 0;
constexpr int kLdsB = kPanelFloats;
constexpr int kLdsFloats = kLdsB + 8 * 2 * kWaveSlotFloats;
constexpr int kLdsBytes = kLdsFloats * 4;

constexpr int kLdsBytesIdxStash = kLdsBytes + kTM * kThreads * 4;
template <int ORDER> struct OrderTraits;
template <> struct OrderTraits<0> {
    static constexpr int kGroups = 4, kIters = 8, kGroupPos = 32;
    static constexpr bool kFused = false;
    __host__ __device__ static int pos_to_k(int pos) {
        const int g = pos >> 5, v = (pos >> 3) & 3, it = pos & 7;
        const int lane = (g == 0) ? 0 : (g == 1) ? 2 : (g == 2) ? 1 : 3;
        return 16 * it + 4 * v + lane;
    }
};
template <> struct OrderTraits<1> {
    static constexpr int kGroups = 8, kIters = 4, kGroupPos = 16;
    static constexpr bool kFused = true;
    __host__ __device__ static int pos_to_k(int pos) {
        const int g = pos >> 4, v = (pos >> 2) & 3, it = pos & 3;
        return 32 * it + 8 * v + g;
    }
};

#define MSFM_TAIL_PRIO() __builtin_amdgcn_s_setprio(3)

template <> struct OrderTraits<3> {
    static constexpr int kGroups = 16, kIters = 2, kGroupPos = 8;
    static constexpr bool kFused = true;
    __host__ __device__ static int pos_to_k(int pos) {
        const int g = pos >> 3, v = (pos >> 1) & 3, it = pos & 1;
        const int a = g >> 2, b = g & 3;
        const int lane = ((a == 0) ? 0 : (a == 1) ? 2 : (a == 2) ? 1 : 3) + ((b == 0) ? 0 : (b == 1) ? 8 : (b == 2) ? 4 : 12);
        return 64 * it + 16 * v + lane;
    }
};

struct PairDesc {
    const float* a_panel;
    const float* b_panel;
    const float* a_rawp;
    const float* b_rawp;
    int n1, n2;
    int a_blocks, b_tiles;
    int n1pad, n2pad;
    int ranges;
    int valid;
    int path;
    int a_blocks256;
    int exact_int;
    long long rp_off;
    long long cp_off;
    long long kf_off;
    long long kr_off;
    long long out_off;
};

struct WorkItem {
    int pair;
    int a_blk;
    int bt_begin, bt_end;
    int range;
    int pad[3];
};

struct Top2 {
    float s0; int i0; float s1;
};

__device__ __forceinline__ float f_inf() { return __builtin_huge_valf(); }

__device__ __forceinline__ void top2_push(float& s0, int& i0, float& s1, float s, int idx) {
    const bool lt = s < s0;
    s1 = __builtin_amdgcn_fmed3f(s0, s1, s);
    i0 = lt ? idx : i0;
    s0 = fminf(s0, s);
}
__device__ __forceinline__ void top2_merge(float& s0, int& i0, float& s1, float bs0, int bi0, float bs1) {
    const bool take_b = (bs0 < s0) || (bs0 == s0 && (unsigned)bi0 < (unsigned)i0);
    s1 = fminf(fmaxf(s0, bs0), fminf(s1, bs1));
    i0 = take_b ? bi0 : i0;
    s0 = fminf(s0, bs0);
}

__device__ __forceinline__ void glds_copy(const float* __restrict__ g, float* lds, int floats, int tid) {
    const int wave = tid >> 6, lane = tid & 63;
#pragma unroll 1
    for (int piece = wave; piece * 256 < floats; piece += kThreads / 64) {
        const float* gp = g + piece * 256 + lane * 4;
        float* lp = lds + piece * 256;
        __builtin_amdgcn_global_load_lds((const __attribute__((address_space(1))) void*)gp,
                                         (__attribute__((address_space(3))) void*)lp, 16, 0, 0);
    }
}

typedef float v2f __attribute__((ext_vector_type(2)));
typedef float v4f __attribute__((ext_vector_type(4)));

template <int ORDER>
__device__ __forceinline__ void group_chains(const float* __restrict__ sa, const float* __restrict__ sb,
                                             v2f (&s)[4][kTN]) {
    using OT = OrderTraits<ORDER>;
    constexpr int kPos = 4 * OT::kIters;
    v4f a_lo = *reinterpret_cast<const v4f*>(sa);
    v4f a_hi = *reinterpret_cast<const v4f*>(sa + 64);
    v4f bb = *reinterpret_cast<const v4f*>(sb);
#pragma unroll
    for (int v = 0; v < 4; ++v) {
        v2f p[4][kTN];
#pragma unroll
        for (int it = 0; it < OT::kIters; ++it) {
            const int pos = v * OT::kIters + it;
            const v2f ap[4] = {a_lo.xy, a_lo.zw, a_hi.xy, a_hi.zw};
            const float bj[kTN] = {bb.x, bb.y, bb.z, bb.w};
#pragma unroll
            for (int h = 0; h < 2; ++h) {
                if (OT::kGroups != 16 && h == 1 && pos + 1 < kPos) {
                    __builtin_amdgcn_sched_barrier(0);
                    a_lo = *reinterpret_cast<const v4f*>(sa + (pos + 1) * kBM);
                    a_hi = *reinterpret_cast<const v4f*>(sa + (pos + 1) * kBM + 64);
                    bb = *reinterpret_cast<const v4f*>(sb + (pos + 1) * kWaveCols);
                }
                if (OT::kGroups == 16) {
#pragma unroll
                    for (int i = 0; i < 2; ++i) {
                        v2f u[kTN];
#pragma unroll
                        for (int j = 0; j < kTN; ++j) u[j] = ap[2 * h + i] - (v2f)(bj[j]);
#pragma unroll
                        for (int j = 0; j < kTN; ++j)
                            p[2 * h + i][j] = (it == 0) ? u[j] * u[j] : __builtin_elementwise_fma(u[j], u[j], p[2 * h + i][j]);
                    }
                    continue;
                }
                v2f t[2][kTN];
#pragma unroll
                for (int i = 0; i < 2; ++i)
#pragma unroll
                    for (int j = 0; j < kTN; ++j) t[i][j] = ap[2 * h + i] - (v2f)(bj[j]);
                if (OT::kFused) {
#pragma unroll
                    for (int i = 0; i < 2; ++i)
#pragma unroll
                        for (int j = 0; j < kTN; ++j)
                            p[2 * h + i][j] = (it == 0) ? t[i][j] * t[i][j]
                                                        : __builtin_elementwise_fma(t[i][j], t[i][j], p[2 * h + i][j]);
// ... 469 lines not shown
```

### monocularsfm_amd/csrc/msfm_match.hip

```cpp
#include "msfm_match.h"
#include "msfm_hostutil.h"
#include "msfm_guard.h"
#include "msfm_tracks.h"
#include "msfm_kernels.hip.h"
#include "msfm_prefilter.hip.h"
#include "msfm_verify.hip.h"
#include "msfm_verify_e.hip.h"
#include "msfm_verify_h.hip.h"
#include "msfm_verify_select.hip.h"
#include "msfm_verify_pose.hip.h"
#include "msfm_retrieval.hip.h"

#include <sys/mman.h>

#include <algorithm>
#include <atomic>
#include <chrono>
#include <condition_variable>
#include <mutex>
#include <thread>
#include <cstdio>
#include <cstdlib>
#include <cmath>
#include <cstring>
// ... 37 lines not shown
static void delete_match_job(MatchJob* j);

int ensure_scratch_set(msfm_ctx* ctx, int k) {
    Scratch& sc = ctx->sc[k];
    if (sc.stream) return MSFM_OK;
    hipError_t e = hipSuccess;
    if ((e = hipStreamCreateWithFlags(&sc.stream, hipStreamNonBlocking)) != hipSuccess ||
        (e = hipEventCreateWithFlags(&sc.sweep1_done, hipEventDisableTiming)) != hipSuccess ||
        (e = hipEventCreateWithFlags(&sc.sweep2_done, hipEventDisableTiming)) != hipSuccess)
        return fail(ctx, MSFM_E_DEVICE, std::string("stream / events of a scratch set: ") + hipGetErrorString(e));
    return MSFM_OK;
}

static int create_rest(msfm_ctx* ctx) {
    auto bad = [ctx](const char* what, hipError_t e) { return fail(ctx, MSFM_E_DEVICE, std::string("msfm_create: ") + what + ": " + hipGetErrorString(e)); };
    hipError_t e = hipSuccess;
    if (ensure_scratch_set(ctx, 0) != MSFM_OK) return MSFM_E_DEVICE;
    struct { const void* f; int bytes; } attrs[] = {
        {reinterpret_cast<const void*>(dist_top2_kernel<0>), kLdsBytes},     {reinterpret_cast<const void*>(dist_top2_kernel<1>), kLdsBytes},
        {reinterpret_cast<const void*>(dist_top2_kernel<3>), kLdsBytesIdxStash},
        {reinterpret_cast<const void*>(sweep_kernel<1>), kPfLdsBytes},       {reinterpret_cast<const void*>(sweep_kernel<2>), kPfLdsBytes},
        {reinterpret_cast<const void*>(sweep_kernel<3>), kPfLdsBytes},       {reinterpret_cast<const void*>(sweep_kernel<4>), kPfLdsBytes},
        {reinterpret_cast<const void*>(sweep_i8_kernel<1>), kI8LdsBytes},    {reinterpret_cast<const void*>(sweep_i8_kernel<3>), kI8LdsBytes3},
    };
    for (const auto& a : attrs)
        if ((e = hipFuncSetAttribute(a.f, hipFuncAttributeMaxDynamicSharedMemorySize, a.bytes)) != hipSuccess)
            return bad("cannot reserve the kernels' LDS", e);
    if ((e = ctx->d_zero_row.ensure(kPfRowBytes)) != hipSuccess || (e = hipMemset(ctx->d_zero_row.p, 0, kPfRowBytes)) != hipSuccess)
        return bad("the zero row", e);
    return MSFM_OK;
}

int msfm_create(int device_ordinal, msfm_ctx** out_ctx) {
    MSFM_API_BEGIN(nullptr)
    if (!out_ctx) return MSFM_E_INVALID;
    *out_ctx = nullptr;
    int count = 0;
    HostClock hc;
    if (hipGetDeviceCount(&count) != hipSuccess || count <= 0) return MSFM_E_DEVICE;
    hc.lap("create: hipGetDeviceCount");
    if (device_ordinal < 0 || device_ordinal >= count) return MSFM_E_INVALID;
    if (hipSetDevice(device_ordinal) != hipSuccess) return MSFM_E_DEVICE;
    hipDeviceProp_t prop;
    if (hipGetDeviceProperties(&prop, device_ordinal) != hipSuccess) return MSFM_E_DEVICE;
    hc.lap("create: set device, properties");
    if (std::strncmp(prop.gcnArchName, "gfx950", 6) != 0) {
        std::fprintf(stderr, "msfm_create: device %d is %s, this library is built for gfx950 only\n",
                     device_ordinal, prop.gcnArchName);
        return MSFM_E_DEVICE;
    }
    msfm_ctx* ctx = new (std::nothrow) msfm_ctx();
    if (!ctx) return MSFM_E_DEVICE;
    ctx->device = device_ordinal;
    ctx->images.resize(kSlots);
    ctx->inbox.recycle = true;
    ctx->job = new_match_job();
    for (Scratch& sc : ctx->sc) {
        for (PinnedBuf& h : sc.h_up) h.pool = &ctx->pinned_pool;
        sc.h_summary.pool = sc.h_tail.pool = sc.h_tk_pairs.pool = &ctx->pinned_pool;
    }
    ctx->h_jobs.pool = ctx->h_store_maxima.pool = &ctx->pinned_pool;
    ctx->cu_count = prop.multiProcessorCount;
    ctx->clock_mhz = prop.clockRate / 1000;
    std::snprintf(ctx->dev_name, sizeof(ctx->dev_name), "%s (%s)", prop.name, prop.gcnArchName);
    if (create_rest(ctx) != MSFM_OK) {
        std::fprintf(stderr, "%s\n", ctx->err.c_str());
        destroy_streams(ctx);
        ctx->d_zero_row.release();
        delete_match_job(ctx->job);
        delete ctx;
        return MSFM_E_DEVICE;
    }
    hc.lap("create: streams, events, kernel attributes, zero row");
    if (const char* e = std::getenv("MSFM_PREFILTER")) ctx->prefilter = e[0] == '2' ? 2 : (e[0] != '0');
    if (const char* e = std::getenv("MSFM_MAX_PAIRS_PER_BATCH"))
        if (std::atoi(e) > 0) ctx->max_pairs_per_batch = std::min(std::atoi(e), kMaxPairsPerBatchLimit);
    if (const char* e = std::getenv("MSFM_PIPELINE_TAPER")) {
        const double t = std::atof(e);
        if (t >= 0.05 && t <= 1.0) ctx->pipeline_taper = t;
    }
    if (const char* e = std::getenv("MSFM_BYTE_DETECT")) ctx->byte_detect = e[0] != '0';
    if (const char* e = std::getenv("MSFM_UPLOAD_THREADS")) ctx->copy_helper = std::atoi(e) != 1;
    if (const char* e = std::getenv("MSFM_Q8_DIRECT")) ctx->q8_direct = e[0] == '2' ? 2 : (e[0] != '0');
    if (const char* e = std::getenv("MSFM_Q8")) ctx->q8_route = e[0] == '2' ? 2 : (e[0] != '0');
    if (const char* e = std::getenv("MSFM_IN_FLIGHT"))
        if (std::atoi(e) >= 1 && std::atoi(e) <= kInFlight) ctx->in_flight = std::atoi(e);
    if (const char* e = std::getenv("MSFM_PIPELINE"))
        if (std::atoi(e) > 0) ctx->pipeline = std::min(std::atoi(e), 64);
    if (const char* e = std::getenv("MSFM_SCRATCH_MIB"))
        if (std::atoll(e) > 0) ctx->scratch_bytes = std::atoll(e) * (1LL << 20);
    *out_ctx = ctx;
    return MSFM_OK;
    MSFM_API_END
}

static void destroy_streams(msfm_ctx* ctx) {
    for (Scratch& sc : ctx->sc) {
        if (sc.sweep1_done) (void)hipEventDestroy(sc.sweep1_done);
        if (sc.sweep2_done) (void)hipEventDestroy(sc.sweep2_done);
        sc.sweep2_done = nullptr;
        if (sc.stream) (void)hipStreamDestroy(sc.stream);
        sc.sweep1_done = nullptr;
        sc.stream = nullptr;
    }
}

void msfm_destroy(msfm_ctx* ctx) {
    if (!ctx) return;
    try {
    HostClock hc;
    (void)hipSetDevice(ctx->device);
    for (Scratch& sc : ctx->sc)
        if (sc.stream) (void)hipStreamSynchronize(sc.stream);
    ctx->deferred.flush();
    ctx->tracks.release();
    ctx->store.release_all();
    ctx->inbox.release_all();
    hc.lap("destroy: store");
    for (Scratch& sc : ctx->sc) sc.release_all();
    hc.lap("destroy: scratch sets");
    DevBuf* bufs[] = {&ctx->d_jobs, &ctx->d_store_maxima, &ctx->d_zero_row, &ctx->ret_words, &ctx->ret_cn};
    for (DevBuf* b : bufs) b->release();
    for (OutSeg& s : ctx->out_segs) {
        s.qt.release();
        s.d.release();
    }
    ctx->res_qt.release();
    ctx->res_dist.release();
    ctx->up_ring.release();
    ctx->h_jobs.release();
    ctx->h_store_maxima.release();
    ctx->pinned_pool.release();
    hc.lap("destroy: result lists, page-locked memory");
    for (hipEvent_t e : ctx->up_ev)
        if (e) (void)hipEventDestroy(e);
    if (ctx->jobs_ev) (void)hipEventDestroy(ctx->jobs_ev);
    delete_match_job(ctx->job);
    for (hipEvent_t e : ctx->ev_pool) (void)hipEventDestroy(e);
    destroy_streams(ctx);
    hc.lap("destroy: events, streams");
    delete ctx;
    } catch (...) {
    }
}

const char* msfm_last_error(const msfm_ctx* ctx) { return ctx ? ctx->err.c_str() : "null context"; }

int msfm_device_info(const msfm_ctx* ctx, char* name, int name_cap, int* cu_count, int* clock_mhz) {
    MSFM_API_BEGIN(nullptr)
    if (!ctx) return MSFM_E_INVALID;
    if (name && name_cap > 0) std::snprintf(name, (size_t)name_cap, "%s", ctx->dev_name);
    if (cu_count) *cu_count = ctx->cu_count;
    if (clock_mhz) *clock_mhz = ctx->clock_mhz;
    return MSFM_OK;
    MSFM_API_END
}

int msfm_set_prefilter(msfm_ctx* ctx, int enable) {
    MSFM_API_BEGIN(ctx)
    if (!ctx) return MSFM_E_INVALID;
    ctx->prefilter = enable == 2 ? 2 : (enable ? 1 : 0);
    return MSFM_OK;
    MSFM_API_END
}

int msfm_set_limits(msfm_ctx* ctx, int max_pairs_per_batch, int64_t scratch_bytes) {
    MSFM_API_BEGIN(ctx)
    if (!ctx) return MSFM_E_INVALID;
    ctx->max_pairs_per_batch = max_pairs_per_batch > 0 ? std::min(max_pairs_per_batch, kMaxPairsPerBatchLimit) : kDefaultMaxPairsPerBatch;
    ctx->scratch_bytes = scratch_bytes > 0 ? scratch_bytes : 0;
    return MSFM_OK;
    MSFM_API_END
}

int msfm_set_pipeline(msfm_ctx* ctx, int min_sub_batches) {
    MSFM_API_BEGIN(ctx)
    if (!ctx) return MSFM_E_INVALID;
    ctx->pipeline = min_sub_batches > 0 ? std::min(min_sub_batches, 64) : kDefaultPipeline;
    return MSFM_OK;
    MSFM_API_END
}

int msfm_get_profile(const msfm_ctx* ctx, msfm_profile* out) {
    MSFM_API_BEGIN(nullptr)
    if (!ctx || !out) return MSFM_E_INVALID;
    *out = ctx->prof;
    return MSFM_OK;
    MSFM_API_END
}

static int drained(msfm_ctx* ctx, int rc) {
    if (rc != MSFM_OK && ctx) {
        ctx->series_open = false;
        for (Scratch& sc : ctx->sc)
            if (sc.stream) (void)hipStreamSynchronize(sc.stream);
        ctx->cur = &ctx->sc[0];
    }
    return rc;
}

namespace {

struct SubBatch {
    bool active = false;
    Batch b;
    int begin = 0, end = 0;
    size_t ev_base = 0;
    bool exact_launched = false;
    int begin_of_cost = -1;
    long long cost_begin = 0;
    std::vector<int64_t> offsets;
    std::vector<int32_t> sens;
    std::vector<int32_t> sel;
    std::vector<msfm_two_view_record> tv;
};

void add_profile(msfm_profile& to, const msfm_profile& d) {
    to.dist_kernel_ms += d.dist_kernel_ms;
    to.dist_kernel_launches += d.dist_kernel_launches;
    to.descriptor_pairs += d.descriptor_pairs;
    to.dist_algo_bytes += d.dist_algo_bytes;
    to.approx_kernel_ms += d.approx_kernel_ms;
    to.approx_kernel_launches += d.approx_kernel_launches;
    to.prefilter_pairs += d.prefilter_pairs;
    to.fallback_pairs += d.fallback_pairs;
    to.candidates += d.candidates;
    to.prefilter_descriptor_pairs += d.prefilter_descriptor_pairs;
    to.exact_descriptor_pairs += d.exact_descriptor_pairs;
    to.tie_rows += d.tie_rows;
    to.sweep2_ms += d.sweep2_ms;
    to.sweep2_launches += d.sweep2_launches;
    to.compacted_pairs += d.compacted_pairs;
    to.sweep2_descriptor_pairs += d.sweep2_descriptor_pairs;
    to.verify_ms += d.verify_ms;
    to.sub_batches += d.sub_batches;
    to.tie_queue_regrows += d.tie_queue_regrows;
    to.plan_regrows += d.plan_regrows;
    to.sweep1_i8_launches += d.sweep1_i8_launches;
    to.order_sensitive_rows += d.order_sensitive_rows;
    to.sweep1_q8_launches += d.sweep1_q8_launches;
    to.sweep1b_launches += d.sweep1b_launches;
    to.sweep1b_ms += d.sweep1b_ms;
    to.sweep1b_descriptor_pairs += d.sweep1b_descriptor_pairs;
    to.demoted_pairs += d.demoted_pairs;
    to.mixed_route_sub_batches += d.mixed_route_sub_batches;
    to.memory_shrinks += d.memory_shrinks;
}

int drain_streams(msfm_ctx* ctx) {
    for (Scratch& s : ctx->sc)
        if (s.stream) HIPCHK(ctx, hipStreamSynchronize(s.stream));
    return MSFM_OK;
}

}

extern "C++" {
#include "msfm_job.hip.h"
}

namespace {
void after_api_exception(msfm_ctx* ctx, const char* text) noexcept {
    if (!ctx) return;
    try {
        ctx->err = text ? text : "C++ exception";
    } catch (...) {
    }
    ctx->series_open = false;
    ctx->have_results = false;
    if (ctx->job) ctx->job->open = false;
    for (Scratch& sc : ctx->sc)
        if (sc.stream) (void)hipStreamSynchronize(sc.stream);
    ctx->cur = &ctx->sc[0];
}
}

static int abandon_series(msfm_ctx* ctx) {
    MatchJob& job = *ctx->job;
    if (ctx->series_open || (job.open && job.streaming)) {
        const int rc = drain_streams(ctx);
        ctx->series_open = false;
        job.open = false;
        if (rc != MSFM_OK) return rc;
        for (SubBatch& w : job.sb) w.active = false;
    }
    job.open = false;
    return MSFM_OK;
}

static int match_pairs_impl(msfm_ctx* ctx, const int32_t* pairs, int n_pairs, const msfm_match_params* params,
                            const msfm_verify_params* verify, int64_t* out_offsets) {
    if (!ctx) return MSFM_E_INVALID;
    if (n_pairs < 0 || (n_pairs > 0 && !pairs) || !out_offsets) return fail(ctx, MSFM_E_INVALID, "bad pair list");
    MatchJob& job = *ctx->job;
    const int rc0 = abandon_series(ctx);
    if (rc0 != MSFM_OK) return rc0;
    int rc = job.start(ctx, pairs, n_pairs, params, verify, false);
    if (rc != MSFM_OK) return rc;
    while (job.more()) {
        int slot = 0;
        rc = job.step(&slot);
        if (rc != MSFM_OK) return rc;
    }
    rc = job.finish();
    if (rc != MSFM_OK) return rc;
    std::memcpy(out_offsets, ctx->res_offsets.data(), ((size_t)n_pairs + 1) * sizeof(int64_t));
    ctx->have_results = true;
    ctx->sel_valid = job.select;
    ctx->tv_valid = job.pose;
    return MSFM_OK;
}

int msfm_match_pairs(msfm_ctx* ctx, const int32_t* pairs, int n_pairs, const msfm_match_params* params,
                     int64_t* out_offsets) {
    MSFM_API_BEGIN(ctx)
    return drained(ctx, match_pairs_impl(ctx, pairs, n_pairs, params, nullptr, out_offsets));
    MSFM_API_END
}

int msfm_match_pairs_verified(msfm_ctx* ctx, const int32_t* pairs, int n_pairs, const msfm_match_params* params,
                              const msfm_verify_params* verify, int64_t* out_offsets) {
    MSFM_API_BEGIN(ctx)
    msfm_verify_params v = {3.0, 0.99, 1000, 0x5eed5eedULL};
    if (verify) v = *verify;
    if (!(v.threshold >= 0.0) || !(v.confidence > 0.0) || !(v.confidence < 1.0) || v.max_iters < 1 || v.max_iters > (1 << 16))
        return fail(ctx, MSFM_E_INVALID, "bad verification parameters");
    return drained(ctx, match_pairs_impl(ctx, pairs, n_pairs, params, &v, out_offsets));
    MSFM_API_END
}
// ... 609 lines not shown
```

### monocularsfm_amd/csrc/msfm_plan.hip.h

```cpp
#pragma once

struct PlanGroup {
    const _Float16* b_h;
    const float* b_nrm;
    float b_c, a_c;
    int dir;
    int bt_begin, bt_end;
    int n2, n2pad, b_tiles;
    int first, count;
    int ranges;
    int b_h0;
    const int* b_n2;
};

struct PlanSummary {
    int ok;
    int n_items;
    long long cmp_rows;
    long long cand_elems;
    long long items_needed;
    long long swept_desc_pairs;
};

struct PlanOut {
    PairDesc* vpairs;
    PfPair* vpf;
    CandList* lists;
    WorkItem* items;
    long long* grow0;
    long long* gpos;
    long long* fwd_items_x;
    PlanSummary* summary;
    const _Float16* const* row_src;
    const _Float16* zero_row;
    int* live_idx;
    int* row_pair;
    long long rows_cap, cand_cap, items_cap;
    const float* cmp_tu;
    const int* cmp_n2;
};

__device__ __forceinline__ int plan_group_cap_units(long long rows) {
    return rows > 0 ? (int)min((rows + 127) / 128 + 1, 1LL << 20) : 0;
}

__device__ __forceinline__ int plan_wave_scan(int v) {
    const int lane = threadIdx.x & 63;
#pragma unroll
    for (int d = 1; d < 64; d <<= 1) {
        const int o = __shfl_up(v, d);
        if (lane >= d) v += o;
    }
    return v;
}

__global__ __launch_bounds__(64) void pf_plan_scan_kernel(const PlanGroup* __restrict__ groups, int n_groups,
                                                        const int* __restrict__ gtot, PlanOut out) {
    MSFM_TAIL_PRIO();
    const int lane = threadIdx.x;
    long long base_rows = 0, base_cand = 0, tot_swept = 0;
    int carry_f = 0, carry_r = 0;
#pragma unroll 1
    for (int g0 = 0; g0 < n_groups; g0 += 64) {
        const int g = g0 + lane;
        const bool in = g < n_groups;
        const long long rows = in ? gtot[g] : 0;
        const int dir = in ? groups[g].dir : 0, ranges = in ? groups[g].ranges : 0;
        const long long rows512 = (rows + kPfWgRows - 1) / kPfWgRows * kPfWgRows;
        const int items = (int)(rows512 / kPfWgRows) * ranges;
        long long swept = 0;
        if (in) {
            const int n2 = groups[g].n2, bt0 = groups[g].bt_begin, bt1 = groups[g].bt_end;
            swept = rows512 * (long long)min(n2 - min(n2, bt0 * kBN), (bt1 - bt0) * kBN);
        }
        const int capu = plan_group_cap_units(rows), ablocks = (int)(rows512 / kPfWgRows);
        tot_swept += swept;
        const int ir = plan_wave_scan(ablocks), ic = plan_wave_scan(capu);
        int vf = dir == 0 ? items : 0, vr = dir == 1 ? items : 0;
        const int f0 = vf, r0 = vr;
#pragma unroll
        for (int d = 8; d < 64; d <<= 1) {
            const int of = __shfl_up(vf, d), orv = __shfl_up(vr, d);
            if (lane >= d) { vf += of; vr += orv; }
        }
        if (in) {
            out.gpos[3 * (long long)g] = (base_rows + (ir - ablocks)) * kPfWgRows;
            out.gpos[3 * (long long)g + 1] = (base_cand + (ic - capu)) * 1024;
            out.gpos[3 * (long long)g + 2] = dir == 0 ? (long long)(carry_f + vf - f0) : (long long)(carry_r + vr - r0);
        }
        base_rows += __shfl(ir, 63);
        base_cand += __shfl(ic, 63);
        carry_f += __shfl(vf, 56 + (lane & 7));
        carry_r += __shfl(vr, 56 + (lane & 7));
    }
#pragma unroll
    for (int d = 1; d < 64; d <<= 1) tot_swept += __shfl_xor(tot_swept, d);
    int n_items = carry_f + carry_r;
#pragma unroll
    for (int d = 1; d < 8; d <<= 1) n_items = max(n_items, __shfl_xor(n_items, d));
    if (lane < 8) out.fwd_items_x[lane] = carry_f;
    if (lane == 0) {
        const long long n8 = 8LL * n_items;
        PlanSummary sm;
        sm.ok = (base_rows * kPfWgRows <= out.rows_cap && base_cand * 1024 <= out.cand_cap && n8 <= out.items_cap) ? 1 : 0;
        sm.n_items = sm.ok ? (int)n8 : 0;
        sm.cmp_rows = base_rows * kPfWgRows;
        sm.cand_elems = base_cand * 1024;
        sm.items_needed = n8;
        sm.swept_desc_pairs = tot_swept;
        *out.summary = sm;
    }
}

__global__ void pf_plan_write_kernel(const PlanGroup* __restrict__ groups, int n_groups, const int* __restrict__ gtot, PlanOut out) {
    MSFM_TAIL_PRIO();
    const int g = blockIdx.x * blockDim.x + threadIdx.x;
    if (g >= n_groups) return;
    const int ok = out.summary->ok;
    const long long rows = gtot[g];
    const long long rows512 = (rows + kPfWgRows - 1) / kPfWgRows * kPfWgRows;
    const int ablocks = (int)(rows512 / kPfWgRows);
    const long long row0 = out.gpos[3 * (long long)g], cand0 = out.gpos[3 * (long long)g + 1];
    const int cap = ok ? plan_group_cap_units(rows) * 1024 : 0;
    const PlanGroup* G = groups + g;
#define MSFM_PLAN_FENCE() asm volatile("" ::: "memory")
    PairDesc* vd = out.vpairs + g;
    vd->n1 = ok ? (int)rows : 0;
    vd->n2 = G->n2;
    vd->a_blocks256 = ok ? ablocks : 0;
    MSFM_PLAN_FENCE();
    vd->b_tiles = G->b_tiles;
    vd->n1pad = ok ? (int)rows512 : 0;
    vd->n2pad = G->n2pad;
    MSFM_PLAN_FENCE();
    vd->valid = 1;
    vd->path = 1;
    vd->ranges = G->ranges;
    vd->rp_off = row0;
    MSFM_PLAN_FENCE();
    PfPair* vp = out.vpf + g;
    vp->a_h = out.zero_row;
    vp->a_rows = out.row_src + row0;
    MSFM_PLAN_FENCE();
    vp->b_h = G->b_h;
    vp->b_nrm = G->b_nrm;
    MSFM_PLAN_FENCE();
    vp->b_c = G->b_c;
    vp->a_c = G->a_c;
    vp->b_h0 = G->b_h0;
    MSFM_PLAN_FENCE();
    vp->tu_off = row0;
    vp->cand_off = cand0;
    vp->cand_cap = cap;
    vp->use = (ok && rows > 0) ? 1 : 0;
    MSFM_PLAN_FENCE();
    CandList* L = out.lists + g;
    L->pair = -1;
    L->mode = 1 + G->dir;
    L->off = cand0;
    L->cap = cap;
    MSFM_PLAN_FENCE();
    L->live_idx = out.live_idx + row0;
    L->row_pair = out.row_pair + row0;
    MSFM_PLAN_FENCE();
    L->cmp_tu = out.cmp_tu + row0;
    L->cmp_n2 = out.cmp_n2 ? out.cmp_n2 + row0 : nullptr;
    L->b_n2 = G->b_n2;
    MSFM_PLAN_FENCE();
    out.grow0[g] = ok ? row0 : -1;
    if (!ok) return;
    const int nblk = G->bt_end - G->bt_begin, ranges = G->ranges, bt0 = G->bt_begin;
    long long k = out.gpos[3 * (long long)g + 2] + (G->dir == 1 ? out.fwd_items_x[g & 7] : 0);
    for (int rg = 0; rg < ranges; ++rg) {
        const int t0 = bt0 + (int)((long long)nblk * rg / ranges), t1 = bt0 + (int)((long long)nblk * (rg + 1) / ranges);
        for (int ab = 0; ab < ablocks; ++ab, ++k) {
            WorkItem* w = out.items + (k * 8 + (g & 7));
            w->pair = g;
            w->a_blk = ab;
            w->bt_begin = t0;
            w->bt_end = t1;
            w->range = rg;
        }
    }
}

__global__ void pf_member_rows_kernel(const PlanGroup* __restrict__ groups, int n_groups, const int* __restrict__ gmembers,
                                      const int* __restrict__ cnt, const long long* __restrict__ grow0, long long* __restrict__ mrow) {
    MSFM_TAIL_PRIO();
    const int g = blockIdx.x * (blockDim.x >> 6) + (threadIdx.x >> 6), lane = threadIdx.x & 63;
    if (g >= n_groups) return;
    const PlanGroup G = groups[g];
    const long long row0 = grow0[g];
    long long base = 0;
    for (int k0 = 0; k0 < G.count; k0 += 64) {
        const int k = k0 + lane;
        const int m = k < G.count ? gmembers[G.first + k] : -1;
        const int c = m >= 0 ? cnt[m] : 0;
        int inc = c;
        for (int d = 1; d < 64; d <<= 1) {
            const int o = __shfl_up(inc, d);
            if (lane >= d) inc += o;
        }
        if (m >= 0) mrow[m] = row0 >= 0 ? row0 + base + (inc - c) : -1;
        base += __shfl(inc, 63);
    }
}

constexpr int kAssignChunk = 1024;
__global__ __launch_bounds__(256) void pf_assign_kernel(
    const PairDesc* __restrict__ pairs, const PfPair* __restrict__ pf, const PlanPair* __restrict__ pp_plan,
    const float* __restrict__ tuv, const unsigned* __restrict__ colmask, const long long* __restrict__ mrow, int* __restrict__ cnt,
    int* __restrict__ live_idx, int* __restrict__ row_pair, float* __restrict__ cmp_tu,
    const _Float16** __restrict__ row_src, int row_halfs ,
    unsigned long long* __restrict__ best, unsigned long long* __restrict__ second,
    int norms_only ,
    int* __restrict__ cmp_n2 ) {
    MSFM_TAIL_PRIO();
    const int p = blockIdx.x >> 1, dir = blockIdx.x & 1;
    const PlanPair pl = pp_plan[p];
    if (pl.fwd_member < 0) return;
    const PairDesc pd = pairs[p];
    const int n = dir ? pd.n2 : pd.n1;
    const int e_begin = blockIdx.y * kAssignChunk;
    if (e_begin >= n) return;
    const PfPair pp = pf[p];
    const long long off = dir ? pp.tv_off : pp.tu_off;
    const float* nrm = dir ? pp.b_nrm : pp.a_nrm;
    const _Float16* src = dir ? pp.b_h : pp.a_h;
    const int* n2 = dir ? pp.b_n2 : pp.a_n2;
    const bool with_n2 = cmp_n2 != nullptr && n2 != nullptr;
    const int bits = dir ? pl.rev_bits : 1, member0 = dir ? pl.rev_member0 : pl.fwd_member;
    __shared__ int hist[32];
    __shared__ long long base[32];
    float t4[4], n4[4];
    unsigned m4[4];
    int x4[4] = {0, 0, 0, 0};
#pragma unroll
    for (int j = 0; j < 4; ++j) {
        const int e = e_begin + (int)threadIdx.x + j * 256, ec = e < n ? e : n - 1;
        t4[j] = tuv[off + ec];
        m4[j] = dir ? colmask[off + ec] : 1u;
        n4[j] = nrm[ec];
        if (with_n2) x4[j] = n2[ec];
        if (e >= n) t4[j] = -f_inf();
    }
    long long my_row0 = -1;
    if ((int)threadIdx.x < bits) my_row0 = mrow[member0 + threadIdx.x];
    if (threadIdx.x < 32) hist[threadIdx.x] = 0;
    __syncthreads();
#pragma unroll
    for (int j = 0; j < 4; ++j) {
        if (t4[j] == -f_inf()) continue;
        for (unsigned m = m4[j]; m; m &= m - 1) atomicAdd(&hist[__builtin_ctz(m)], 1);
    }
    __syncthreads();
    if ((int)threadIdx.x < bits) {
        const int h = hist[threadIdx.x];
        base[threadIdx.x] = (h > 0 && my_row0 >= 0) ? my_row0 + (long long)(atomicSub(&cnt[member0 + threadIdx.x], h) - h) : -1;
        hist[threadIdx.x] = 0;
    }
    __syncthreads();
#pragma unroll
    for (int j = 0; j < 4; ++j) {
        const float t = t4[j];
        if (t == -f_inf()) continue;
        const int e = e_begin + (int)threadIdx.x + j * 256;
        best[off + e] = ~0ull;
        second[off + e] = ~0ull;
        for (unsigned m = m4[j]; m; m &= m - 1) {
            const int b = __builtin_ctz(m);
            const long long r0 = base[b];
            if (r0 < 0) continue;
            const long long k = r0 + atomicAdd(&hist[b], 1);
            live_idx[k] = e;
            row_pair[k] = p;
            cmp_tu[k] = norms_only ? -n4[j] : t - n4[j];
            if (with_n2) cmp_n2[k] = x4[j];
            row_src[k] = src + (size_t)e * row_halfs;
        }
    }
}

__global__ void pf_overflow_kernel(const CandList* __restrict__ lists, int n_lists, const unsigned long long* __restrict__ cand_count,
                                   const PlanGroup* __restrict__ groups, const int* __restrict__ gmembers, const int* __restrict__ member_pair,
                                   unsigned char* __restrict__ overflow_pair, unsigned long long* __restrict__ totals ) {
    MSFM_TAIL_PRIO();
    for (int l = blockIdx.x * blockDim.x + threadIdx.x; l < n_lists; l += gridDim.x * blockDim.x) {
        const CandList L = lists[l];
        if (L.cap == 0) continue;
        const unsigned long long c = cand_count[l];
        if (c <= (unsigned long long)L.cap) {
            atomicAdd(&totals[0], c);
            continue;
        }
        atomicAdd(&totals[1], 1ull);
        if (L.mode == 0) overflow_pair[L.pair] = 1;
        else
            for (int k = 0; k < groups[l].count; ++k) overflow_pair[member_pair[gmembers[groups[l].first + k]]] = 1;
    }
}
```

### monocularsfm_amd/csrc/msfm_prefilter.hip.h

```cpp
#pragma once
#include "msfm_kernels.hip.h"

namespace msfm {

constexpr float kEpsRel = 1.5e-3f;
constexpr float kEpsAbs = 1.0e-6f;
constexpr float kF16Safe = 6.0e4f;

constexpr int kPfRB = 2;
constexpr int kPfWaveRows = 32 * kPfRB;
constexpr int kPfWaves = 8;
constexpr int kPfWgRows = kPfWaves * kPfWaveRows;
constexpr int kPfThreads = 64 * kPfWaves;
constexpr int kPfBT = 64;
constexpr int kPfRowHalfs = 136;
constexpr int kPfRowBytes = kPfRowHalfs * 2;
constexpr int kPfTileBytes = kPfBT * kPfRowBytes;
constexpr int kPfTilePieces = kPfTileBytes / 1024;
constexpr int kPfRing = 4;
constexpr int kPfColClasses = 4;
constexpr int kPfCandBuf = 256;
constexpr int kPfLdsBytes = kPfRing * kPfTileBytes + kPfWaves * kPfRing * 64 * 4 + kPfWaves * kPfCandBuf * 8 +
                            2 * kPfBT * kPfColClasses * 4;
static_assert(kPfTileBytes % 1024 == 0 && kPfTilePieces == 17, "tile = 17 DMA pieces");

typedef _Float16 h8 __attribute__((ext_vector_type(8)));
typedef float f16v __attribute__((ext_vector_type(16)));

struct PfPair {
    const _Float16* a_h;
    const _Float16* b_h;
    const _Float16* const* a_rows;
    const float* a_nrm;
    const float* b_nrm;
    float a_c, b_c;
    float a_nrm_max, b_nrm_max;
    long long tu_off;
    long long tv_off;
    long long cand_off;
    int cand_cap;
    int use;
    int i8;
    int a_h0, b_h0;
    int pad;
    const float* a_err;
    const float* b_err;
    const int* a_n2;
    const int* b_n2;
};

__device__ __forceinline__ void glds_copy_bytes(const void* g, void* lds, int bytes, int tid, int nthreads) {
    const int wave = __builtin_amdgcn_readfirstlane(tid >> 6), lane = tid & 63;
    const char* gp = reinterpret_cast<const char*>(g);
    char* lp = reinterpret_cast<char*>(lds);
#pragma unroll 1
    for (int piece = wave; piece * 1024 < bytes; piece += nthreads / 64)
        __builtin_amdgcn_global_load_lds((const __attribute__((address_space(1))) void*)(gp + piece * 1024 + lane * 16),
                                         (__attribute__((address_space(3))) void*)(lp + piece * 1024), 16, 0, 0);
}

__device__ __forceinline__ void v2_merge(float& s0, float& s1, float b0, float b1) {
    s1 = fminf(fmaxf(s0, b0), fminf(s1, b1));
    s0 = fminf(s0, b0);
}

#include "msfm_sweep.hip.h"
#include "msfm_sweep_i8.hip.h"

struct PruneParams {
    int prune;
    float ratio;
    float max_distance;
};

__device__ __forceinline__ bool pf_dead(float s0, float s1, float nrm, float eps, float other_max, PruneParams pr) {
    if (!pr.prune) return false;
    const float tiny = 1e-5f * (fabsf(s0) + fabsf(s1) + nrm + other_max);
    const float s0lb = fmaxf(s0 - eps - tiny, 0.f);
    const float s1ub = s1 + eps + tiny;
    const float d0lb = sqrtf(s0lb) * (1.f - 1e-6f);
    const bool ratio_fails = pr.ratio > 0.f && d0lb >= pr.ratio * sqrtf(s1ub) * (1.f + 1e-5f);
    const bool too_far = d0lb > pr.max_distance * (1.f + 1e-5f);
    return ratio_fails || too_far;
}

struct PlanPair {
    int fwd_member;
    int rev_member0;
    int rev_bits;
    int pad;
};


struct PlanCounts {
    const PlanPair* pp_plan;
    const int* member_group;
    int* cnt;
    int* gtot;
};

__global__ void pf_thresholds_kernel(const PairDesc* __restrict__ pairs, const PfPair* __restrict__ pf,
                                     const float* __restrict__ rp_s0, const float* __restrict__ rp_s1,
                                     const float* __restrict__ cp_s0, unsigned* __restrict__ colmask,
                                     float* __restrict__ tu, float* __restrict__ tv, PruneParams pr, PlanCounts plan,
                                     int marked ) {
    MSFM_TAIL_PRIO();
    const PairDesc pd = pairs[blockIdx.y];
    const PfPair pp = pf[blockIdx.y];
    if (!pd.valid || !pp.use) return;
    const int e = blockIdx.x * blockDim.x + threadIdx.x;
    bool row_live = false;
    unsigned col_bits = 0;
    const float eps_norm = 4.8828125e-4f * fmaxf(pp.a_c, pp.b_c);
    const float2* cp2 = reinterpret_cast<const float2*>(cp_s0);
    const int* cpk = reinterpret_cast<const int*>(cp_s0);
    const int nb = pd.a_blocks256;
    const bool in_r = e < pd.n1pad, in_c = e < pd.n2pad;
    const int er = in_r ? e : 0, ec = in_c ? e : 0;
    const float ld_rs0 = rp_s0[pd.rp_off + er], ld_rs1 = rp_s1[pd.rp_off + er];
    const float ld_anrm = pp.a_nrm[er], ld_bnrm = pp.b_nrm[ec];
    const float ld_tu = marked ? tu[pp.tu_off + er] : 0.f, ld_tv = marked ? tv[pp.tv_off + ec] : 0.f;
    float2 ld_cp[16];
#pragma unroll
    for (int p = 0; p < 16; ++p) {
        const long long i = pd.cp_off + (long long)min(p, nb - 1) * pd.n2pad + ec;
        ld_cp[p] = pp.i8 ? make_float2(__int_as_float(cpk[i]), 0.f) : cp2[i];
    }
    auto partial16 = [&](int p) -> float2 { return pp.i8 ? i8_cp_unpack(__float_as_int(ld_cp[p].x)) : ld_cp[p]; };
    if (in_r && !(marked && ld_tu == -f_inf())) {
        float s0 = f_inf(), s1 = f_inf();
        v2_merge(s0, s1, ld_rs0, ld_rs1);
        for (int p = 1; p < pd.ranges; ++p) {
            const long long o = pd.rp_off + (long long)p * pd.n1pad + e;
            v2_merge(s0, s1, rp_s0[o], rp_s1[o]);
        }
        const float na = ld_anrm;
        const float eps = pp.i8 ? kI8Eps : kEpsRel * (na + pp.b_nrm_max) + kEpsAbs * (sqrtf(na) + sqrtf(pp.b_nrm_max)) + eps_norm;
        const float slack = pp.i8 ? 2.f * eps : 2.f * eps + 1e-5f * (fabsf(s1) + na + pp.b_nrm_max);
        const bool live = (e < pd.n1) && !pf_dead(s0, s1, na, eps, pp.b_nrm_max, pr);
        tu[pp.tu_off + e] = live ? s1 + slack : -f_inf();
        row_live = live;
    }
    if (in_c && marked && ld_tv == -f_inf()) {
        if (colmask) colmask[pp.tv_off + e] = 0;
    } else if (in_c) {
        float s0 = f_inf(), s1 = f_inf();
        auto partial = [&](long long i) -> float2 { return pp.i8 ? i8_cp_unpack(cpk[i]) : cp2[i]; };
        float bmin[16];
        if (nb <= 16) {
#pragma unroll
            for (int p = 0; p < 16; ++p) {
                bmin[p] = f_inf();
                if (p < nb) {
                    const float2 m = partial16(p);
                    bmin[p] = -2.f * m.x;
                    v2_merge(s0, s1, -2.f * m.x, -2.f * m.y);
                }
            }
        } else {
            for (int p = 0; p < nb; ++p) {
                const float2 m = partial(pd.cp_off + (long long)p * pd.n2pad + e);
                v2_merge(s0, s1, -2.f * m.x, -2.f * m.y);
            }
        }
        const float nb_ = ld_bnrm;
        const float eps = pp.i8 ? kI8Eps : kEpsRel * (nb_ + pp.a_nrm_max) + kEpsAbs * (sqrtf(nb_) + sqrtf(pp.a_nrm_max)) + eps_norm;
        const float slack = pp.i8 ? 2.f * eps : 2.f * eps + 1e-5f * (fabsf(s1) + nb_ + pp.a_nrm_max);
        const bool live = (e < pd.n2) && !pf_dead(s0, s1, nb_, eps, pp.a_nrm_max, pr);
        const float T = live ? s1 + slack : -f_inf();
        tv[pp.tv_off + e] = T;
        if (colmask) {
            const int g = (nb + 31) / 32;
            unsigned mask = 0;
// ... 276 lines not shown
```

### monocularsfm_amd/csrc/msfm_q8.hip.h

```cpp
#pragma once

constexpr float kQ8LevelStep = 1.f / 16.f;

__global__ void pf_prune_q8_kernel(const PairDesc* __restrict__ pairs, const PfPair* __restrict__ pf, const PfPair* __restrict__ pfq,
                                   const float* __restrict__ rp_s0, const float* __restrict__ rp_s1, const float* __restrict__ cp_s0,
                                   unsigned* __restrict__ colmask, float* __restrict__ tuv, PruneParams pr, PlanCounts plan,
                                   float inv, int direct) {
    MSFM_TAIL_PRIO();
    const PairDesc pd = pairs[blockIdx.y];
    const PfPair pp = pf[blockIdx.y];
    if (!pd.valid || !pp.use) return;
    const PfPair pq = pfq[blockIdx.y];
    if (!pq.use) return;
    const int e = blockIdx.x * blockDim.x + threadIdx.x;
    bool row_live = false;
    unsigned col_bits = 0;
    auto lower = [&](float s0, float err) -> float { return fmaxf(sqrtf(fmaxf(s0, 0.f)) * inv * (1.f - 1e-6f) - err, 0.f); };
    auto upper = [&](float s1, float err) -> float { return sqrtf(s1 + 2.f) * inv * (1.f + 1e-6f) + err; };
    auto dead = [&](float s0, float s1, float err) -> bool {
        const float l0 = lower(s0, err), u1 = upper(s1, err);
        const bool ratio_fails = pr.ratio > 0.f && l0 * (1.f - 1e-5f) >= pr.ratio * u1 * (1.f + 1e-5f);
        const bool too_far = l0 * (1.f - 1e-5f) > pr.max_distance * (1.f + 1e-5f);
        return ratio_fails || too_far;
    };
    const float eps_norm = 4.8828125e-4f * fmaxf(pp.a_c, pp.b_c);
    auto threshold = [&](float u1, float nrm, float other_max) -> float {
        const float eps = kEpsRel * (nrm + other_max) + kEpsAbs * (sqrtf(nrm) + sqrtf(other_max)) + eps_norm;
        const float u2 = u1 * u1;
        return u2 * (1.f + 3e-5f) + eps + 1e-5f * (u2 + nrm + other_max);
    };
    const int* cpk = reinterpret_cast<const int*>(cp_s0);
    const int nb = pd.a_blocks256;
    const bool in_r = e < pd.n1pad, in_c = e < pd.n2pad;
    const int er = in_r ? e : 0, ec = in_c ? e : 0;
    const float ld_rs0 = rp_s0[pd.rp_off + er], ld_rs1 = rp_s1[pd.rp_off + er];
    const float ld_aerr = pq.a_err[min(er, pd.n1 - 1)], ld_anrm = pp.a_nrm[er];
    const float ld_berr = pq.b_err[min(ec, pd.n2 - 1)], ld_bnrm = pp.b_nrm[ec];
    int ld_cp[16];
#pragma unroll
    for (int p = 0; p < 16; ++p) ld_cp[p] = cpk[pd.cp_off + (long long)min(p, nb - 1) * pd.n2pad + ec];
    if (in_r) {
        float s0 = f_inf(), s1 = f_inf();
        v2_merge(s0, s1, ld_rs0, ld_rs1);
        for (int p = 1; p < pd.ranges; ++p) {
            const long long o = pd.rp_off + (long long)p * pd.n1pad + e;
            v2_merge(s0, s1, rp_s0[o], rp_s1[o]);
        }
        bool live = e < pd.n1;
        const float err = live ? (ld_aerr + pq.b_c) * (1.f + 1e-6f) : 0.f;
        if (live) live = !dead(s0, s1, err);
        float T = live ? f_inf() : -f_inf();
        if (live && direct) T = threshold(upper(s1, err), ld_anrm, pp.b_nrm_max);
        tuv[pp.tu_off + e] = T;
        row_live = live;
    }
    if (in_c) {
        float s0 = f_inf(), s1 = f_inf();
        float bmin[16];
        if (nb <= 16) {
#pragma unroll
            for (int p = 0; p < 16; ++p) {
                float2 m = make_float2(-f_inf(), -f_inf());
                if (p < nb) m = i8_cp_unpack(ld_cp[p]);
                bmin[p] = -2.f * m.x;
                v2_merge(s0, s1, -2.f * m.x, -2.f * m.y);
            }
        } else {
            for (int p = 0; p < nb; ++p) {
                const float2 m = i8_cp_unpack(cpk[pd.cp_off + (long long)p * pd.n2pad + e]);
                v2_merge(s0, s1, -2.f * m.x, -2.f * m.y);
            }
        }
        bool live = e < pd.n2;
        const float err = live ? (ld_berr + pq.a_c) * (1.f + 1e-6f) : 0.f;
        if (live) live = !dead(s0, s1, err);
        const int g = (nb + 31) / 32, bits = (nb + g - 1) / g;
        if (!direct) {
            tuv[pp.tv_off + e] = live ? f_inf() : -f_inf();
            col_bits = live ? (bits >= 32 ? 0xffffffffu : ((1u << bits) - 1u)) : 0u;
        } else {
            const float u1 = live ? upper(s1, err) : 0.f;
            tuv[pp.tv_off + e] = live ? threshold(u1, ld_bnrm, pp.a_nrm_max) : -f_inf();
            if (live) {
                if (nb <= 16) {
#pragma unroll
                    for (int p = 0; p < 16; ++p)
                        if (p < nb && lower(bmin[p], err) * (1.f - 1e-5f) <= u1 * (1.f + 1e-5f)) col_bits |= 1u << p;
                } else {
                    for (int p = 0; p < nb; ++p) {
                        const float smin = -2.f * i8_cp_unpack(cpk[pd.cp_off + (long long)p * pd.n2pad + e]).x;
                        if (lower(smin, err) * (1.f - 1e-5f) <= u1 * (1.f + 1e-5f)) col_bits |= 1u << (p / g);
                    }
                }
            }
        }
        colmask[pp.tv_off + e] = col_bits;
    }
    if (plan.pp_plan) {
        const PlanPair pl = plan.pp_plan[blockIdx.y];
        if (pl.fwd_member < 0) return;
        __shared__ int hist[33];
        if (threadIdx.x < 33) hist[threadIdx.x] = 0;
        __syncthreads();
        const unsigned long long rl = __ballot(row_live);
        if ((threadIdx.x & 63) == 0 && rl) atomicAdd(&hist[32], __popcll(rl));
        if (!direct) {
            const unsigned long long cl = __ballot(col_bits != 0u);
            if ((threadIdx.x & 63) == 0 && cl) atomicAdd(&hist[0], __popcll(cl));
        } else {
            while (col_bits) {
                const int bit = __builtin_ctz(col_bits);
                col_bits &= col_bits - 1;
                atomicAdd(&hist[bit], 1);
            }
        }
        __syncthreads();
        if (threadIdx.x == 0 && hist[32]) {
            atomicAdd(&plan.cnt[pl.fwd_member], hist[32]);
            atomicAdd(&plan.gtot[plan.member_group[pl.fwd_member]], hist[32]);
        }
        const int mine = direct ? hist[threadIdx.x < 33 ? threadIdx.x : 0] : hist[0];
        if ((int)threadIdx.x < pl.rev_bits && mine) {
            atomicAdd(&plan.cnt[pl.rev_member0 + threadIdx.x], mine);
            atomicAdd(&plan.gtot[plan.member_group[pl.rev_member0 + threadIdx.x]], mine);
        }
    }
}

__global__ void q8_scatter_kernel(const PairDesc* __restrict__ pairs, const PairDesc* __restrict__ vpairs, const CandList* __restrict__ lists,
                                  const PlanGroup* __restrict__ groups, int n_groups, const long long* __restrict__ grow0,
                                  const float* __restrict__ cmp_s0, const float* __restrict__ cmp_s1,
                                  float* __restrict__ rp_s0, float* __restrict__ rp_s1, float* __restrict__ cp_s0) {
    MSFM_TAIL_PRIO();
    const int g = blockIdx.y;
    if (g >= n_groups) return;
    const long long row0 = grow0[g];
    if (row0 < 0) return;
    const int rows = vpairs[g].n1;
    const CandList L = lists[g];
    const PlanGroup G = groups[g];
    for (int k = blockIdx.x * blockDim.x + threadIdx.x; k < rows; k += gridDim.x * blockDim.x) {
        const int e = L.live_idx[k];
        const PairDesc pd = pairs[L.row_pair[k]];
        const float s0 = cmp_s0[row0 + k], s1 = cmp_s1[row0 + k];
        if (G.dir == 0) {
            for (int p = 0; p < pd.ranges; ++p) {
                rp_s0[pd.rp_off + (long long)p * pd.n1pad + e] = p == 0 ? s0 : f_inf();
                rp_s1[pd.rp_off + (long long)p * pd.n1pad + e] = p == 0 ? s1 : f_inf();
            }
        } else {
            const int p0 = G.bt_begin / (kPfWgRows / kBM), p1 = (G.bt_end + kPfWgRows / kBM - 1) / (kPfWgRows / kBM);
            float2* cp2 = reinterpret_cast<float2*>(cp_s0);
            for (int p = p0; p < p1 && p < pd.a_blocks256; ++p)
                cp2[pd.cp_off + (long long)p * pd.n2pad + e] = p == p0 ? make_float2(-0.5f * s0, -0.5f * s1) : make_float2(-f_inf(), -f_inf());
        }
    }
}
```

### monocularsfm_amd/csrc/msfm_sweep.hip.h

```cpp
#pragma once

template <int N>
__device__ __forceinline__ void wait_vmcnt() {
    asm volatile("s_waitcnt vmcnt(%0)" ::"n"(N) : "memory");
}

__device__ __forceinline__ void lds_barrier() {
    __builtin_amdgcn_sched_barrier(0);
    asm volatile("s_waitcnt lgkmcnt(0)" ::: "memory");
    __builtin_amdgcn_s_barrier();
    asm volatile("" ::: "memory");
    __builtin_amdgcn_sched_barrier(0);
}

__device__ __forceinline__ float max3f(float a, float b, float c) { return fmaxf(fmaxf(a, b), c); }

template <int PASS>
__global__ __launch_bounds__(kPfThreads, 2) void sweep_kernel(
    const PairDesc* __restrict__ pairs, const PfPair* __restrict__ pf, const WorkItem* __restrict__ items,
    float* __restrict__ rp_s0, float* __restrict__ rp_s1, float* __restrict__ cp_s0, float* __restrict__ cp_s1,
    const float* __restrict__ tu, const float* __restrict__ tv, int2* __restrict__ cand,
    unsigned long long* __restrict__ cand_count ,
    const int* __restrict__ n_items_dev , int n_items_host,
    int* __restrict__ dyn_next ) {
    typedef const __attribute__((address_space(1))) float* gfloat_p;
    typedef const __attribute__((address_space(1))) h8* gh8_p;
    extern __shared__ __attribute__((aligned(16))) char pf_smem[];
    char* sB = pf_smem;
    float* sThr = reinterpret_cast<float*>(pf_smem + kPfRing * kPfTileBytes);
    char* sCand = reinterpret_cast<char*>(sThr + kPfWaves * kPfRing * 64);
    float* sCol = reinterpret_cast<float*>(sCand + kPfWaves * kPfCandBuf * 8);

    const int n_items = n_items_dev ? *n_items_dev : n_items_host;
    __shared__ int s_next_item;
    bool first_item = true;
#pragma unroll 1
    for (int it = blockIdx.x;; it += gridDim.x) {
    if (!first_item || dyn_next) lds_barrier();
    first_item = false;
    if (dyn_next) {
        if (threadIdx.x == 0) s_next_item = atomicAdd(&dyn_next[blockIdx.x & 7], 1);
        lds_barrier();
        it = s_next_item * 8 + (int)(blockIdx.x & 7);
    }
    if (it >= n_items) break;
    const WorkItem item = items[it];
    if (item.pair < 0) continue;
    const PfPair pp = pf[item.pair];
    if (!pp.use) continue;
    const PairDesc pd = pairs[item.pair];

    const int tid = threadIdx.x, lane = tid & 63;
    const int wave = __builtin_amdgcn_readfirstlane(tid >> 6);
    const int grp = wave >> 2;
    const int lcol = lane & 31, lhalf = lane >> 5;

    const int t_begin = item.bt_begin * 2, t_end = min(item.bt_end * 2, max(item.bt_begin * 2 + 1, (pd.n2 + kPfBT - 1) / kPfBT));
    const char* gB = reinterpret_cast<const char*>(pp.b_h);
    const gfloat_p g_anrm = (gfloat_p)pp.a_nrm;
    const gfloat_p g_tu = (gfloat_p)tu;
    float* thr_w = sThr + wave * (kPfRing * 64);

    const unsigned lane_off = (unsigned)(wave * 1024 + lane * 16);
    auto dma_tile = [&](int tt) {
        const int tc = tt < t_end ? tt : t_end - 1;
        const int sl = (tt - t_begin) & (kPfRing - 1);
        const unsigned off = (unsigned)tc * (unsigned)kPfTileBytes + lane_off;
        char* l = sB + sl * kPfTileBytes + wave * 1024;
        __builtin_amdgcn_global_load_lds((const __attribute__((address_space(1))) void*)(gB + off), (__attribute__((address_space(3))) void*)l, 16, 0, 0);
        __builtin_amdgcn_global_load_lds((const __attribute__((address_space(1))) void*)(gB + (off + 8192u)),
                                         (__attribute__((address_space(3))) void*)(l + 8192), 16, 0, 0);
        if (wave == 0)
            __builtin_amdgcn_global_load_lds((const __attribute__((address_space(1))) void*)(gB + (off + 16384u)),
                                             (__attribute__((address_space(3))) void*)(l + 16384), 16, 0, 0);
        if (PASS == 2)
            __builtin_amdgcn_global_load_lds((const __attribute__((address_space(1))) void*)(tv + pp.tv_off + tc * kPfBT + lane),
                                             (__attribute__((address_space(3))) void*)(thr_w + sl * 64), 4, 0, 0);
    };
    constexpr int kDmaOps = (PASS == 2) ? 3 : 2;
    auto wait_older_group = [&]() {
        if (wave == 0) wait_vmcnt<kDmaOps + 1>();
        else wait_vmcnt<kDmaOps>();
    };

    dma_tile(t_begin);
    dma_tile(t_begin + 1);
    dma_tile(t_begin + 2);
    if (PASS == 1) sCol[tid] = -f_inf();

    typedef _Float16 h4 __attribute__((ext_vector_type(4)));
    h8 af[kPfRB][8];
    h4 ae[kPfRB];
    const float inv_c = 1.f / pp.b_c;
#pragma unroll
    for (int rb = 0; rb < kPfRB; ++rb) {
        const int frow = item.a_blk * kPfWgRows + wave * kPfWaveRows + rb * 32 + lcol;
        const _Float16* arow = pp.a_h + (size_t)frow * kPfRowHalfs;
        if (PASS >= 3) {
            const _Float16* r = pp.a_rows[frow];
            arow = r ? r : pp.a_h;
        }
        const gh8_p ga = (gh8_p)arow;
#pragma unroll
        for (int ks = 0; ks < 8; ++ks) af[rb][ks] = ga[2 * ks + lhalf];
        float X;
        if (PASS >= 3) X = frow < pd.n1 ? 0.5f * g_tu[pp.tu_off + frow] : -f_inf();
        else X = frow < pd.n1 ? -0.5f * g_anrm[frow] : -f_inf();
        const float xs = X * inv_c;
        const _Float16 hi = (_Float16)xs;
        const float rest = xs - (float)hi;
        const _Float16 lo = (rest == rest && fabsf(rest) < 3.0e38f) ? (_Float16)rest : (_Float16)0.f;
        h4 e;
#pragma unroll
        for (int j = 0; j < 4; ++j) e[j] = (_Float16)0.f;
        if (lhalf == 0) {
            e[0] = (_Float16)(-pp.b_c);
            e[1] = (_Float16)(-pp.b_c);
            e[2] = hi;
            e[3] = lo;
        }
        ae[rb] = e;
    }

    const int arow_base = item.a_blk * kPfWgRows + wave * kPfWaveRows + 4 * lhalf;
    float rs0[kPfRB][16];
#pragma unroll
    for (int rb = 0; rb < kPfRB; ++rb)
#pragma unroll
        for (int r = 0; r < 16; ++r) {
            const int rr = arow_base + rb * 32 + (r & 3) + 8 * (r >> 2);
            if (PASS == 2) {
                const float lvl = -0.5f * g_tu[pp.tu_off + rr];
                rs0[rb][r] = rr < pd.n1 ? lvl : f_inf();
            } else {
                rs0[rb][r] = -f_inf();
            }
        }
#pragma unroll
    for (int rb = 0; rb < kPfRB; ++rb) {
#pragma unroll
        for (int ks = 0; ks < 8; ++ks) asm volatile("" ::"v"(af[rb][ks]));
        asm volatile("" ::"v"(ae[rb]));
    }
    wait_vmcnt<0>();

    int2* cbuf = reinterpret_cast<int2*>(sCand) + wave * kPfCandBuf;
    const unsigned cbuf_lds = (unsigned)(unsigned long long)(__attribute__((address_space(3))) char*)cbuf;
    int n_buf = 0;
    auto flush_candidates = [&]() {
        if (n_buf == 0) return;
        unsigned long long base64 = 0;
        if (lane == 0) base64 = atomicAdd(&cand_count[item.pair], (unsigned long long)n_buf);
        const int base = __builtin_amdgcn_readfirstlane((int)(base64 < (unsigned long long)pp.cand_cap ? base64 : (unsigned long long)pp.cand_cap));
        asm volatile("s_waitcnt lgkmcnt(0)" ::: "memory");
        for (int k = lane; k < n_buf; k += 64)
            if (base + k < pp.cand_cap) cand[pp.cand_off + base + k] = cbuf[k];
        n_buf = 0;
    };

    const bool wave_active = __builtin_amdgcn_readfirstlane((int)(item.a_blk * kPfWgRows + wave * kPfWaveRows < pd.n1)) != 0;

    const int lane_row_off = lcol * kPfRowBytes + lhalf * 16;
    const int lane_ext_off = lcol * kPfRowBytes + 2 * kDim + lhalf * 8;
    auto load_bf = [&](int sl, h8 (&bf)[8], h4 (&be)[2]) {
        const char* pb = sB + sl * kPfTileBytes + lane_row_off;
#pragma unroll
        for (int ks = 0; ks < 8; ++ks) bf[ks] = *reinterpret_cast<const h8*>(pb + ks * 32);
        const char* pe = sB + sl * kPfTileBytes + lane_ext_off;
        be[0] = *reinterpret_cast<const h4*>(pe);
        be[1] = *reinterpret_cast<const h4*>(pe + 32 * kPfRowBytes);
    };
    auto mfma_block = [&](const h8 (&bf)[8], h4 be, f16v (&acc)[kPfRB]) {
#pragma unroll
        for (int r = 0; r < 16; ++r)
#pragma unroll
            for (int rb = 0; rb < kPfRB; ++rb) acc[rb][r] = 0.f;
#pragma unroll
        for (int ks = 0; ks < 8; ++ks)
#pragma unroll
            for (int rb = 0; rb < kPfRB; ++rb) acc[rb] = __builtin_amdgcn_mfma_f32_32x32x16_f16(af[rb][ks], bf[ks], acc[rb], 0, 0, 0);
#pragma unroll
        for (int rb = 0; rb < kPfRB; ++rb)
            acc[rb] = __builtin_amdgcn_mfma_f32_32x32x8f16(ae[rb], be, acc[rb], 0, 0, 0);
    };
    auto mfma_block_reload = [&](int sl, h8 (&bf)[8], h4 be, f16v (&acc)[kPfRB]) {
#pragma unroll
        for (int r = 0; r < 16; ++r)
#pragma unroll
            for (int rb = 0; rb < kPfRB; ++rb) acc[rb][r] = 0.f;
        const char* pb = sB + sl * kPfTileBytes + 32 * kPfRowBytes + lane_row_off;
#pragma unroll
        for (int ks = 0; ks < 8; ++ks) {
#pragma unroll
            for (int rb = 0; rb < kPfRB; ++rb) acc[rb] = __builtin_amdgcn_mfma_f32_32x32x16_f16(af[rb][ks], bf[ks], acc[rb], 0, 0, 0);
            bf[ks] = *reinterpret_cast<const h8*>(pb + ks * 32);
        }
#pragma unroll
        for (int rb = 0; rb < kPfRB; ++rb)
            acc[rb] = __builtin_amdgcn_mfma_f32_32x32x8f16(ae[rb], be, acc[rb], 0, 0, 0);
#pragma unroll
        for (int ks = 0; ks < 8; ++ks) {
            __builtin_amdgcn_sched_group_barrier(0x008, 2, 0);
            __builtin_amdgcn_sched_group_barrier(0x100, 1, 0);
        }
        __builtin_amdgcn_sched_group_barrier(0x008, 2, 0);
    };
    auto column_max = [&](const f16v (&acc)[kPfRB]) -> float {
        static_assert(kPfRB == 2, "two chains");
        float m[kPfRB];
#pragma unroll
        for (int rb = 0; rb < kPfRB; ++rb) {
            m[rb] = max3f(acc[rb][0], acc[rb][1], acc[rb][2]);
#pragma unroll
            for (int r = 3; r < 15; r += 2) m[rb] = max3f(m[rb], acc[rb][r], acc[rb][r + 1]);
        }
        float last;
        asm("v_max_f32 %0, %1, %2" : "=v"(last) : "v"(acc[0][15]), "v"(acc[1][15]));
        return max3f(m[0], m[1], last);
    };
    auto record_hits = [&](bool hit, int row, int col) {
        const unsigned long long mm = __ballot(hit);
        if (mm == 0ull) return;
        if (n_buf + 64 > kPfCandBuf) flush_candidates();
        if (hit) {
            const int slt = n_buf + __popcll(mm & ((1ull << lane) - 1ull));
            const int2 e = make_int2(row, col);
            asm volatile("ds_write_b64 %0, %1" ::"v"(cbuf_lds + slt * 8), "v"(e) : "memory");
        }
        n_buf += __popcll(mm);
    };
    auto scan_hits3 = [&](const f16v (&a0)[kPfRB], const f16v (&a1)[kPfRB], int col0) {
        unsigned nm[2] = {0u, 0u};
#pragma unroll
        for (int blk = 0; blk < 2; ++blk)
#pragma unroll
            for (int rb = 0; rb < kPfRB; ++rb)
#pragma unroll
                for (int r = 0; r < 16; ++r) nm[blk] = __builtin_amdgcn_alignbit(nm[blk], __float_as_uint((blk ? a1 : a0)[rb][r]), 31);
        static_assert(kPfRB == 2, "32 elements per column block and mask");
#pragma unroll 1
        for (int blk = 0; blk < 2; ++blk) {
            unsigned hm = ~(blk ? nm[1] : nm[0]);
            const int col = col0 + blk * 32;
            for (unsigned long long mm = __ballot(hm != 0u); mm != 0ull; mm = __ballot(hm != 0u)) {
                const bool hit = hm != 0u;
                const int k = __clz((int)hm);
                if (n_buf + 64 > kPfCandBuf) flush_candidates();
                if (hit) {
                    hm &= ~(0x80000000u >> k);
                    const int slt = n_buf + __popcll(mm & ((1ull << lane) - 1ull));
                    const int2 e = make_int2(arow_base + (k >> 4) * 32 + (k & 3) + 8 * ((k & 15) >> 2), col);
                    asm volatile("ds_write_b64 %0, %1" ::"v"(cbuf_lds + slt * 8), "v"(e) : "memory");
                }
                n_buf += __popcll(mm);
            }
        }
    };
    auto scan_hits2 = [&](const f16v (&acc)[kPfRB], float hc, int col) {
        float mr = -f_inf(), mc = -f_inf();
#pragma unroll
        for (int rb = 0; rb < kPfRB; ++rb)
#pragma unroll
            for (int r = 0; r < 16; r += 2) {
                mr = max3f(mr, acc[rb][r] - rs0[rb][r], acc[rb][r + 1] - rs0[rb][r + 1]);
                mc = max3f(mc, acc[rb][r], acc[rb][r + 1]);
            }
        if (__ballot(mr >= 0.f || mc >= hc) == 0ull) return;
#pragma unroll
        for (int rb = 0; rb < kPfRB; ++rb)
#pragma unroll
            for (int r = 0; r < 16; ++r)
                record_hits(acc[rb][r] > -f_inf() && (acc[rb][r] >= rs0[rb][r] || acc[rb][r] >= hc),
                            arow_base + rb * 32 + (r & 3) + 8 * (r >> 2), col);
    };
    const unsigned col_lds = (unsigned)(unsigned long long)(__attribute__((address_space(3))) char*)sCol +
                             (unsigned)((2 * (wave & 1) + lhalf) * kPfBT + lcol) * 4u;
    auto fold_columns = [&](float mA, float mB, int cs) {
        const unsigned a = col_lds + (unsigned)cs * (kPfBT * kPfColClasses * 4);
        asm volatile("ds_max_f32 %0, %1\n\tds_max_f32 %0, %2 offset:128" ::"v"(a), "v"(mA), "v"(mB) : "memory");
    };
    const unsigned colrow_lds = (unsigned)(unsigned long long)(__attribute__((address_space(3))) char*)sCol + (unsigned)lane * 4u;
    auto store_columns = [&](int tt) {
        const unsigned a = colrow_lds + (unsigned)((tt - t_begin) & 1) * (kPfBT * kPfColClasses * 4);
        v4f v;
        const float ninf = -f_inf();
        asm volatile("ds_read_b32 %0, %4\n\tds_read_b32 %1, %4 offset:256\n\tds_read_b32 %2, %4 offset:512\n\tds_read_b32 %3, %4 offset:768\n\t"
                     "s_waitcnt lgkmcnt(0)\n\t"
                     "ds_write_b32 %4, %5\n\tds_write_b32 %4, %5 offset:256\n\tds_write_b32 %4, %5 offset:512\n\tds_write_b32 %4, %5 offset:768"
                     : "=&v"(v.x), "=&v"(v.y), "=&v"(v.z), "=&v"(v.w) : "v"(a), "v"(ninf) : "memory");
        const float m01 = fmaxf(v.x, v.y), n01 = fminf(v.x, v.y), m23 = fmaxf(v.z, v.w), n23 = fminf(v.z, v.w);
        v2f o;
        o.x = fmaxf(m01, m23);
        o.y = fmaxf(fminf(m01, m23), fmaxf(n01, n23));
        reinterpret_cast<v2f*>(cp_s0)[pd.cp_off + (long long)item.a_blk * pd.n2pad + tt * kPfBT + lane] = o;
    };

    lds_barrier();
    constexpr bool kPreRead = PASS != 2;
    h8 bf[8];
    h4 be[2];
    if (kPreRead && wave_active) load_bf(0, bf, be);
    if (grp == 1) lds_barrier();

    f16v accA[kPfRB], accB[kPfRB];
#pragma unroll 1
    for (int t = t_begin; t < t_end; ++t) {
        const int sl = (t - t_begin) & (kPfRing - 1);
        if (wave_active) {
            __builtin_amdgcn_s_setprio(1);
            if (!kPreRead) load_bf(sl, bf, be);
            mfma_block_reload(sl, bf, be[0], accA);
            mfma_block(bf, be[1], accB);
            __builtin_amdgcn_s_setprio(0);
        }
        if (grp == 0) wait_older_group();
        lds_barrier();
        if (PASS == 1 && grp == 0 && t > t_begin && wave == ((t - t_begin) & 3)) store_columns(t - 1);
        dma_tile(t + 3);
        if (wave_active) {
            if (PASS == 1 || PASS == 4) {
                if (PASS == 1) fold_columns(column_max(accA), column_max(accB), (t - t_begin) & 1);
#pragma unroll
                for (int rb = 0; rb < kPfRB; ++rb)
#pragma unroll
                    for (int r = 0; r < 16; ++r) rs0[rb][r] = max3f(rs0[rb][r], accA[rb][r], accB[rb][r]);
            } else if (PASS == 3) {
                scan_hits3(accA, accB, t * kPfBT + lcol);
            } else {
                const float* thr = thr_w + sl * 64;
                scan_hits2(accA, -0.5f * thr[lcol], t * kPfBT + lcol);
                scan_hits2(accB, -0.5f * thr[32 + lcol], t * kPfBT + 32 + lcol);
            }
        }
        if (kPreRead && wave_active && t + 1 < t_end) load_bf((sl + 1) & (kPfRing - 1), bf, be);
        if (grp == 1) wait_older_group();
        lds_barrier();
    }
    if (grp == 0) lds_barrier();
    if (PASS == 2 || PASS == 3) flush_candidates();
    if (PASS == 1 && wave == 0) store_columns(t_end - 1);

    if (PASS == 1 || PASS == 4) {
        wait_vmcnt<0>();
        lds_barrier();
        float* tr = reinterpret_cast<float*>(sB) + wave * (kPfWaveRows * 33);
        static_assert(kPfWaves * kPfWaveRows * 33 * 4 <= kPfRing * kPfTileBytes, "the transposition fits the ring");
#pragma unroll
        for (int rb = 0; rb < kPfRB; ++rb)
#pragma unroll
            for (int r = 0; r < 16; ++r) tr[(rb * 32 + (r & 3) + 8 * (r >> 2) + 4 * lhalf) * 33 + lcol] = rs0[rb][r];
        float m0 = -f_inf(), m1 = -f_inf();
#pragma unroll 8
        for (int k = 0; k < 32; ++k) {
            const float v = tr[lane * 33 + k];
            m1 = fmaxf(m1, fminf(m0, v));
            m0 = fmaxf(m0, v);
        }
        const long long o = pd.rp_off + (long long)item.range * pd.n1pad + item.a_blk * kPfWgRows + wave * kPfWaveRows + lane;
        rp_s0[o] = -2.f * m0;
        rp_s1[o] = -2.f * m1;
    }
    }
}
```

### monocularsfm_amd/csrc/msfm_sweep_i8.hip.h

```cpp
#pragma once

constexpr int kI8RowBytes = 176;
constexpr int kI8TileBytes = kPfBT * kI8RowBytes;
constexpr int kI8DigitLo = -243968, kI8DigitHi = 245759;
constexpr int kI8Waves = 16;
constexpr int kI8Threads = 64 * kI8Waves;
constexpr int kI8WaveRows = kPfWgRows / kI8Waves;
constexpr int kI8Ring = 8;
constexpr int kI8LdsBytes = kI8Ring * kI8TileBytes + kI8Waves * kPfCandBuf * 8 + 4 * kPfBT * kPfColClasses * 4;
constexpr int kI8LdsBytes3 = kI8LdsBytes + kI8Waves * kPfCandBuf * 4;
static_assert(kI8WaveRows == 32, "one 32-row block per wave");
constexpr int kI8Pad = -(1 << 29);
constexpr int kI8PadTest = -(1 << 27);
constexpr float kI8Eps = 2.f;
static_assert(kI8TileBytes % 1024 == 0 && kI8TileBytes / 1024 == 11, "tile = 11 DMA pieces");

typedef int i4v __attribute__((ext_vector_type(4)));
typedef int i16v __attribute__((ext_vector_type(16)));

__device__ __forceinline__ int max3i(int a, int b, int c) { return max(max(a, b), c); }

__device__ __forceinline__ float2 i8_cp_unpack(int code) {
    const int hi = msfm_cp_hi(code);
    if (hi == kCpNone) return make_float2(-f_inf(), -f_inf());
    return make_float2((float)hi, msfm_cp_has_second(code) ? (float)(hi - msfm_cp_gap(code)) : -f_inf());
}

template <int PASS>
__global__ __launch_bounds__(kI8Threads) void sweep_i8_kernel(
    const PairDesc* __restrict__ pairs, const PfPair* __restrict__ pf, const WorkItem* __restrict__ items,
    float* __restrict__ rp_s0, float* __restrict__ rp_s1, float* __restrict__ cp_s0, const float* __restrict__ tu,
    int2* __restrict__ cand, unsigned long long* __restrict__ cand_count, const int* __restrict__ n_items_dev, int n_items_host,
    int* __restrict__ dyn_next, int* __restrict__ cand_val ) {
    static_assert(PASS == 1 || PASS == 3, "sweep 1 and the compacted sweep 2");
    typedef const __attribute__((address_space(1))) float* gfloat_p;
    typedef const __attribute__((address_space(1))) i4v* gi4_p;
    extern __shared__ __attribute__((aligned(16))) char pf_smem[];
    char* sB = pf_smem;
    char* sCand = pf_smem + kI8Ring * kI8TileBytes;
    int* sCol = reinterpret_cast<int*>(sCand + kI8Waves * kPfCandBuf * 8);
    int* sVal = sCol + 4 * kPfBT * kPfColClasses;

    const int n_items = n_items_dev ? *n_items_dev : n_items_host;
    __shared__ int s_next_item;
    bool first_item = true;
#pragma unroll 1
    for (int it = blockIdx.x;; it += gridDim.x) {
    if (!first_item || dyn_next) lds_barrier();
    first_item = false;
    if (dyn_next) {
        if (threadIdx.x == 0) s_next_item = atomicAdd(&dyn_next[blockIdx.x & 7], 1);
        lds_barrier();
        it = s_next_item * 8 + (int)(blockIdx.x & 7);
    }
    if (it >= n_items) break;
    const WorkItem item = items[it];
    if (item.pair < 0) continue;
    const PfPair pp = pf[item.pair];
    if (!pp.use) continue;
    const PairDesc pd = pairs[item.pair];

    const int tid = threadIdx.x, lane = tid & 63;
    const int wave = __builtin_amdgcn_readfirstlane(tid >> 6);
    const int grp = (wave >> 2) & 1;
    const int lcol = lane & 31, lhalf = lane >> 5;

    const int t_begin = item.bt_begin * 2, t_end = min(item.bt_end * 2, max(item.bt_begin * 2 + 1, (pd.n2 + kPfBT - 1) / kPfBT));
    const char* gB = reinterpret_cast<const char*>(pp.b_h);
    const gfloat_p g_tu = (gfloat_p)tu;

    const bool dma_wave = wave < kI8TileBytes / 1024;
    const unsigned lane_off = (unsigned)(wave * 1024 + lane * 16);
    auto dma_tile = [&](int tt) {
        if (!dma_wave) return;
        const int tc = tt < t_end ? tt : t_end - 1;
        const int sl = (tt - t_begin) & (kI8Ring - 1);
        const unsigned long long tile = (unsigned long long)gB + (unsigned long long)(unsigned)tc * (unsigned long long)kI8TileBytes;
        const unsigned dst = (unsigned)(unsigned long long)(__attribute__((address_space(3))) char*)(sB + sl * kI8TileBytes + wave * 1024);
#pragma clang diagnostic push
#pragma clang diagnostic ignored "-Winline-asm"
        asm volatile("s_mov_b32 m0, %2\n\ts_nop 0\n\tglobal_load_lds_dwordx4 %0, %1"
                     :: "v"(lane_off), "s"(tile), "s"(dst) : "memory", "m0");
#pragma clang diagnostic pop
    };
    auto wait_older_group = [&]() {
        if (dma_wave) wait_vmcnt<kI8Ring - 3>();
    };

#pragma unroll
    for (int k = 0; k < kI8Ring - 1; ++k) dma_tile(t_begin + k);
    if (PASS == 1 && tid < 4 * kPfBT * kPfColClasses) sCol[tid] = (int)0x80000000;

    i4v af[4], a_digit;
    {
        const int frow = item.a_blk * kPfWgRows + wave * kI8WaveRows + lcol;
        const char* arow = reinterpret_cast<const char*>(pp.a_h) + (size_t)frow * kI8RowBytes;
        if (PASS == 3) {
            const char* r = reinterpret_cast<const char*>(pp.a_rows[frow]);
            arow = r ? r : reinterpret_cast<const char*>(pp.a_h);
        }
        const gi4_p ga = (gi4_p)arow;
#pragma unroll
        for (int ks = 0; ks < 4; ++ks) af[ks] = ga[2 * ks + lhalf];
        const i4v cdig = {(int)0x80808001u, (int)0x80808080u, (int)0x80808080u, (int)0x80808080u};
        if (PASS == 1) {
            a_digit = ga[8];
            if (lhalf == 0) a_digit = cdig;
        } else {
            a_digit = lhalf == 0 ? cdig : i4v(0);
        }
    }
    const int arow_base = item.a_blk * kPfWgRows + wave * kI8WaveRows + 4 * lhalf;
    i16v rowc = i16v(0);
    if (PASS == 3) {
        float xs[16];
#pragma unroll
// ... 138 lines not shown
        bf[0][1] = *reinterpret_cast<const i4v*>(pb2 + 32 * kI8RowBytes);
        accA = __builtin_amdgcn_mfma_i32_32x32x32_i8(af[1], bf[1][0], accA, 0, 0, 0);
        accB = __builtin_amdgcn_mfma_i32_32x32x32_i8(af[1], bf[1][1], accB, 0, 0, 0);
        bf[1][0] = *reinterpret_cast<const i4v*>(pb2 + 32);
        bf[1][1] = *reinterpret_cast<const i4v*>(pb2 + 32 * kI8RowBytes + 32);
        accA = __builtin_amdgcn_mfma_i32_32x32x32_i8(af[2], bf[0][0], accA, 0, 0, 0);
        accB = __builtin_amdgcn_mfma_i32_32x32x32_i8(af[2], bf[0][1], accB, 0, 0, 0);
        bf[0][0] = *reinterpret_cast<const i4v*>(pb2 + 64);
        bf[0][1] = *reinterpret_cast<const i4v*>(pb2 + 32 * kI8RowBytes + 64);
        accA = __builtin_amdgcn_mfma_i32_32x32x32_i8(af[3], bf[1][0], accA, 0, 0, 0);
        accB = __builtin_amdgcn_mfma_i32_32x32x32_i8(af[3], bf[1][1], accB, 0, 0, 0);
        accA = __builtin_amdgcn_mfma_i32_32x32x32_i8(a_digit, bf[0][0], accA, 0, 0, 0);
        accB = __builtin_amdgcn_mfma_i32_32x32x32_i8(a_digit, bf[0][1], accB, 0, 0, 0);
    };
    auto epilogue_half = [&](int t) {
        const bool last_tile = (t + 1) * kPfBT > pd.n2;
        if (PASS == 1 && last_tile) {
            const bool v0 = t * kPfBT + lcol < pd.n2, v1 = t * kPfBT + 32 + lcol < pd.n2;
#pragma unroll
            for (int r = 0; r < 16; ++r) {
                accA[r] = v0 ? accA[r] : kI8Pad;
                accB[r] = v1 ? accB[r] : kI8Pad;
            }
        }
        if (wave_partial) {
            int row_lim = pd.n1 - arow_base;
            asm volatile("" : "+v"(row_lim));
#pragma unroll
            for (int r = 0; r < 16; ++r) {
                const bool real_row = (r & 3) + 8 * (r >> 2) < row_lim;
                accA[r] = real_row ? accA[r] : kI8Pad;
                accB[r] = real_row ? accB[r] : kI8Pad;
            }
        }
        if (PASS == 3 && last_tile) {
            if (!(t * kPfBT + lcol < pd.n2)) accA = i16v(-1);
            if (!(t * kPfBT + 32 + lcol < pd.n2)) accB = i16v(-1);
        }
        if (PASS == 1) {
            fold_columns(column_max(accA), column_max(accB), (t - t_begin) & 3);
#pragma unroll
            for (int r = 0; r < 16; ++r) rs0[r] = max3i(rs0[r], accA[r], accB[r]);
        } else {
            scan_hits3(accA, accB, t * kPfBT + lcol);
        }
    };

    auto next_interval = [&](int v) {
        wait_older_group();
        lds_barrier();
        dma_tile(v + kI8Ring - 1);
        if (PASS == 1 && v - 2 >= t_begin && wave == ((v - t_begin) & 3)) store_columns(v - 2);
    };
#pragma unroll 1
    for (int u = t_begin; u < t_end; ++u) {
        if (wave_active) matrix_half(u);
        if (grp == 1) next_interval(u + 1);
        if (wave_active) {
            epilogue_half(u);
            if (u + 1 < t_end) preread((u + 1 - t_begin) & (kI8Ring - 1), bf);
        }
        if (grp == 0) next_interval(u + 1);
    }
    if (PASS == 3) flush_candidates();

    if (PASS == 1) {
        wait_vmcnt<0>();
        lds_barrier();
        if (wave == 0) store_columns(t_end - 1);
        int* tr = reinterpret_cast<int*>(sB) + wave * (kI8WaveRows * 33);
        static_assert(kI8Waves * kI8WaveRows * 33 * 4 <= kI8Ring * kI8TileBytes, "the transposition fits the ring");
#pragma unroll
        for (int r = 0; r < 16; ++r) tr[((r & 3) + 8 * (r >> 2) + 4 * lhalf) * 33 + lcol] = rs0[r];
        if (lane < kI8WaveRows) {
            int m0 = (int)0x80000000, m1 = (int)0x80000000;
#pragma unroll 8
            for (int k = 0; k < 32; ++k) {
                const int v = tr[lane * 33 + k];
                m1 = max(m1, min(m0, v));
                m0 = max(m0, v);
            }
            const long long o = pd.rp_off + (long long)item.range * pd.n1pad + item.a_blk * kPfWgRows + wave * kI8WaveRows + lane;
            rp_s0[o] = m0 > kI8PadTest ? (float)(-2 * (m0 - item_k)) : f_inf();
            rp_s1[o] = m1 > kI8PadTest ? (float)(-2 * (m1 - item_k)) : f_inf();
        }
    }
    }
}
```

Baseline: 5621 billion.

## Split forward sweep-2 into 32 column classes pruned by per-row class masks

Sweep 1 now records, for each query row, a 32-bit mask of which column classes (columns congruent mod 32) could still hold a candidate within a conservative quantization-slack bound. The compacted sweep 2 splits each forward group into 32 strided column-class groups, and only rows whose mask bit is set are scheduled for each class. Strided DMA offsets and masking of the tail columns are added to the sweep kernel. The aim is to cut exact-distance work in sweep 2 for the Q8 direct route, at the cost of more groups, per-row mask storage, strided global loads and extra plan-room accounting.

```diff
diff --git a/include/msfm_match.h b/include/msfm_match.h
--- a/include/msfm_match.h
+++ b/include/msfm_match.h
@@ -66,6 +66,9 @@
     int demoted_pairs;
     int mixed_route_sub_batches;
     int memory_shrinks;
+    int fwd_class_groups;
+    int64_t sweep2_fwd_descriptor_pairs;
+    int64_t sweep2_rev_descriptor_pairs;
 } msfm_profile;
 
 int msfm_create(int device_ordinal, msfm_ctx** out_ctx);
diff --git a/monocularsfm_amd/_lib.py b/monocularsfm_amd/_lib.py
--- a/monocularsfm_amd/_lib.py
+++ b/monocularsfm_amd/_lib.py
@@ -193,7 +193,8 @@
                 ("sub_batches", C.c_int), ("tie_queue_regrows", C.c_int), ("plan_regrows", C.c_int),
                 ("sweep1_i8_launches", C.c_int), ("sweep1_q8_launches", C.c_int), ("sweep1b_launches", C.c_int),
                 ("sweep1b_ms", C.c_double), ("sweep1b_descriptor_pairs", C.c_int64), ("order_sensitive_rows", C.c_int64),
-                ("demoted_pairs", C.c_int), ("mixed_route_sub_batches", C.c_int), ("memory_shrinks", C.c_int)]
+                ("demoted_pairs", C.c_int), ("mixed_route_sub_batches", C.c_int), ("memory_shrinks", C.c_int),
+                ("fwd_class_groups", C.c_int), ("sweep2_fwd_descriptor_pairs", C.c_int64), ("sweep2_rev_descriptor_pairs", C.c_int64)]
 
 
 class Chunk(C.Structure):
diff --git a/monocularsfm_amd/csrc/msfm_batch.hip.h b/monocularsfm_amd/csrc/msfm_batch.hip.h
--- a/monocularsfm_amd/csrc/msfm_batch.hip.h
+++ b/monocularsfm_amd/csrc/msfm_batch.hip.h
@@ -173,7 +173,7 @@
     for (auto& pd : b.pairs) {
         if (!pd.valid || pd.path != path) continue;
         pd.ranges = 1;
-        if (total_ablocks > 0 && total_ablocks < target_items) {
+        if (total_ablocks > 0 && total_ablocks < target_items && !(path == 1 && b.route.fwd_classes)) {
             long long r = (target_items + total_ablocks - 1) / total_ablocks;
             pd.ranges = (int)std::max<long long>(1, std::min<long long>(r, pd.b_tiles));
         }
@@ -274,7 +274,10 @@
 
 void build_compact_plan(msfm_ctx* ctx, const Batch& b, CompactPlan& cp, bool no_ranges) {
     const size_t P = b.pairs.size();
-    cp.ppair.assign(P, PlanPair{-1, 0, 0, 0});
+    const bool classes = b.route.fwd_classes;
+    const int fwd_bits = classes ? 32 : 1;
+    int class_imgs = 0;
+    cp.ppair.assign(P, PlanPair{-1, 0, 0, 1});
     static thread_local std::vector<int> dense;
     dense.assign((size_t)kSlots, -1);
     std::vector<int> img_slot;
@@ -286,6 +289,7 @@
         return dense[(size_t)slot];
     };
     std::vector<int> fwd_group_of_img, rev_group0_of_img;
+    int class_block0 = 0;
     std::vector<int>& member_group = cp.member_group;
     for (size_t p = 0; p < P; ++p) {
         const PairDesc& pd = b.pairs[p];
@@ -298,9 +302,39 @@
             fwd_group_of_img.resize(need, -1);
             rev_group0_of_img.resize(need, -1);
         }
+        if (classes && fwd_group_of_img[(size_t)dj] < 0) {
+            const int m = class_imgs++ & 7;
+            if (m == 0) {
+                const size_t g0 = (cp.groups.size() + 7) / 8 * 8;
+                PlanGroup none = {};
+                none.ranges = 1, none.stride = 1;
+                cp.groups.resize(g0 + 256, none);
+                class_block0 = (int)g0;
+            }
+            fwd_group_of_img[(size_t)dj] = class_block0 + m;
+            for (int c = 0; c < 32; ++c) {
+                PlanGroup& g = cp.groups[(size_t)(class_block0 + 8 * c + m)];
+                g.b_h = pp.b_h;
+                g.b_nrm = pp.b_nrm;
+                g.b_c = pp.b_c;
+                g.a_c = pp.a_c;
+                g.b_h0 = pp.b_h0;
+                g.b_n2 = pp.b_n2;
+                g.dir = 0;
+                g.col0 = c;
+                g.stride = 32;
+                g.n2 = pd.n2 > c ? (pd.n2 - c + 31) / 32 : 0;
+                g.n2pad = pd.n2pad;
+                g.b_tiles = std::max(1, (g.n2 + kBN - 1) / kBN);
+                g.bt_begin = 0;
+                g.bt_end = g.b_tiles;
+                g.ranges = 1;
+            }
+        }
         if (fwd_group_of_img[(size_t)dj] < 0) {
             fwd_group_of_img[(size_t)dj] = (int)cp.groups.size();
             PlanGroup g = {};
+            g.stride = 1;
             g.b_h = pp.b_h;
             g.b_nrm = pp.b_nrm;
             g.b_c = pp.b_c;
@@ -317,14 +351,18 @@
             cp.groups.push_back(g);
         }
         cp.ppair[p].fwd_member = (int)cp.member_pair.size();
-        cp.member_pair.push_back((int)p);
-        member_group.push_back(fwd_group_of_img[(size_t)dj]);
-        cp.rows_ub += pd.n1;
+        cp.ppair[p].fwd_bits = fwd_bits;
+        for (int c = 0; c < fwd_bits; ++c) {
+            cp.member_pair.push_back((int)p);
+            member_group.push_back(fwd_group_of_img[(size_t)dj] + 8 * c);
+        }
+        cp.rows_ub += (classes ? 3LL : 1LL) * pd.n1;
         const int nb = pd.a_blocks256, gshift = (nb + 31) / 32, bits = (nb + gshift - 1) / gshift;
         if (rev_group0_of_img[(size_t)di] < 0) {
             rev_group0_of_img[(size_t)di] = (int)cp.groups.size();
             for (int bit = 0; bit < bits; ++bit) {
                 PlanGroup g = {};
+                g.stride = 1;
                 g.b_h = pp.a_h;
                 g.b_nrm = pp.a_nrm;
                 g.b_c = pp.a_c;
@@ -440,6 +478,7 @@
                 pp.a_c = ia.err_q8_max, pp.b_c = ib.err_q8_max;
                 pp.a_h0 = ia.h0_q8, pp.b_h0 = ib.h0_q8;
                 pp.a_err = ia.err_q8, pp.b_err = ib.err_q8;
+                pp.cls_slack = msfm_class_slack(ia.err_q8_max, ib.err_q8_max, msfm_class_scale(ctx->q8_level / 255.f));
             } else {
                 pp.a_h = reinterpret_cast<const _Float16*>(ia.i8);
                 pp.b_h = reinterpret_cast<const _Float16*>(ib.i8);
@@ -471,6 +510,9 @@
     kn = std::max<long long>(1, b.kf_elems + b.kr_elems);
     HIPCHK(ctx, SC.d_rp_s0.ensure(std::max<long long>(1, b.rp_elems) * 4));
     HIPCHK(ctx, SC.d_rp_s1.ensure(std::max<long long>(1, b.rp_elems) * 4));
+    if (route.fwd_classes) {
+        HIPCHK(ctx, SC.d_rp_cls.ensure(std::max<long long>(1, b.rp_elems) * 4));
+    }
     HIPCHK(ctx, SC.d_cp_s0.ensure(std::max<long long>(1, b.cp_elems) * ((route.kind == kRouteI8 || route.kind == kRouteQ8Direct) ? 4 : 8)));
     HIPCHK(ctx, SC.d_tu.ensure(kn * 4));
     HIPCHK(ctx, SC.d_colmask.ensure(kn * 4));
@@ -513,7 +555,7 @@
                                route.q8() ? (const PfPair*)SC.d_pfq.as<PfPair>() : dpf,
                                SC.d_items.as<WorkItem>(), SC.d_rp_s0.as<float>(), SC.d_rp_s1.as<float>(), SC.d_cp_s0.as<float>(),
                                (const float*)nullptr, (int2*)nullptr, (unsigned long long*)nullptr, (const int*)nullptr, (int)b.n_items, (int*)nullptr,
-                               (int*)nullptr);
+                               (int*)nullptr, route.fwd_classes ? SC.d_rp_cls.as<unsigned>() : (unsigned*)nullptr);
         else
             hipLaunchKernelGGL(sweep_kernel<1>, dim3(std::min<unsigned>(sweep_grid, (unsigned)b.n_items)), block, kPfLdsBytes, SC.stream, dp, dpf,
                                SC.d_items.as<WorkItem>(), SC.d_rp_s0.as<float>(), SC.d_rp_s1.as<float>(),
@@ -562,7 +604,10 @@
         long long cand_have = (long long)(SC.d_cand.cap / sizeof(int2));
         if (route.kind == kRouteI8) cand_have = std::min<long long>(cand_have, (long long)(SC.d_cand_val.cap / 4));
         const long long items_have = (long long)(SC.d_vitems.cap / sizeof(WorkItem)) / 8 * 8;
-        const MsfmPlanRoom room = msfm_plan_room(ub, refine ? cp.rows_ub_all_bits * 5 / 32 : cp.rows_ub * 5 / 16, (long long)G, max_ranges, kPfWgRows,
+        long long g_room = 0;
+        for (const PlanGroup& g : cp.groups) g_room += g.b_h == nullptr ? 0 : (g.stride > 1 ? 1 : 2);
+        g_room = (g_room + 1) / 2;
+        const MsfmPlanRoom room = msfm_plan_room(ub, refine ? cp.rows_ub_all_bits * 5 / 32 : cp.rows_ub * 5 / 16, g_room, max_ranges, kPfWgRows,
                                                  ctx->hint_rows_ub, ctx->cmp_rows_hint, ctx->cand_hint, ctx->items_hint, rows_have, cand_have, items_have);
         rows_cap = room.rows, cand_cap = room.cand, items_cap = room.items;
         SC.pf_pending.rows_ub = ub;
@@ -662,7 +707,8 @@
     int launch_route_q() {
         hipLaunchKernelGGL(pf_prune_q8_kernel, mgrid, dim3(256), 0, SC.stream, dp, dpf, (const PfPair*)SC.d_pfq.as<PfPair>(),
                            (const float*)SC.d_rp_s0.as<float>(), (const float*)SC.d_rp_s1.as<float>(), (const float*)SC.d_cp_s0.as<float>(),
-                           colmask, tuv, prune, pc, ctx->q8_level / 255.f, route.kind == kRouteQ8Refine ? 0 : 1);
+                           colmask, tuv, prune, pc, ctx->q8_level / 255.f, route.kind == kRouteQ8Refine ? 0 : 1,
+                           route.fwd_classes ? (const unsigned*)SC.d_rp_cls.as<unsigned>() : (const unsigned*)nullptr);
         HIPCHK(ctx, hipGetLastError());
         DBGSYNC(ctx, "pf_prune_q8_kernel");
         if (route.kind == kRouteQ8Refine) {
@@ -722,7 +768,7 @@
                                (const WorkItem*)SC.d_vitems.as<WorkItem>(), (float*)nullptr, (float*)nullptr, (float*)nullptr,
                                (const float*)SC.d_cmp_tu.as<float>(), SC.d_cand.as<int2>(),
                                SC.d_cand_count.as<unsigned long long>(), (const int*)&SC.d_summary.as<PlanSummary>()->n_items, 0,
-                               SC.d_totals.as<int>() + 8, SC.d_cand_val.as<int>());
+                               SC.d_totals.as<int>() + 8, SC.d_cand_val.as<int>(), (unsigned*)nullptr);
         else
             hipLaunchKernelGGL(sweep_kernel<3>, dim3(sweep_grid), block, kPfLdsBytes, SC.stream,
                                (const PairDesc*)SC.d_vpairs.as<PairDesc>(), (const PfPair*)SC.d_vpf.as<PfPair>(),
@@ -878,6 +924,9 @@
             return MSFM_OK;
         }
         SC.prof.sweep2_descriptor_pairs += sm.swept_desc_pairs;
+        SC.prof.sweep2_fwd_descriptor_pairs += sm.swept_fwd;
+        SC.prof.sweep2_rev_descriptor_pairs += sm.swept_desc_pairs - sm.swept_fwd;
+        SC.prof.fwd_class_groups += sm.class_groups;
     } else {
         SC.prof.sweep2_descriptor_pairs += pe.dense_swept;
     }
diff --git a/monocularsfm_amd/csrc/msfm_ctx.hip.h b/monocularsfm_amd/csrc/msfm_ctx.hip.h
--- a/monocularsfm_amd/csrc/msfm_ctx.hip.h
+++ b/monocularsfm_amd/csrc/msfm_ctx.hip.h
@@ -467,6 +467,7 @@
     Ref d_groups, d_gmembers, d_member_pair, d_member_group, d_ppair;
     DevBuf d_items;
     DevBuf d_rp_s0, d_rp_i0, d_rp_s1, d_cp_s0, d_cp_i0, d_cp_s1;
+    DevBuf d_rp_cls;
     DevBuf d_k_i0, d_k_d0, d_k_d1;
     DevBuf d_st_qt, d_st_d, d_counts, d_offsets, d_sens;
     DevBuf d_sub_qt, d_sub_d;
@@ -497,7 +498,7 @@
     bool sweep2_recorded = false;
     long long seq = 0;
     void for_each_buf(void (*fn)(DevBuf&, void*), void* arg) {
-        DevBuf* bufs[] = {&d_up[0], &d_up[1], &d_up[2], &d_items, &d_rp_s0, &d_rp_i0, &d_rp_s1, &d_cp_s0, &d_cp_i0, &d_cp_s1, &d_k_i0, &d_k_d0,
+        DevBuf* bufs[] = {&d_up[0], &d_up[1], &d_up[2], &d_items, &d_rp_s0, &d_rp_i0, &d_rp_s1, &d_rp_cls, &d_cp_s0, &d_cp_i0, &d_cp_s1, &d_k_i0, &d_k_d0,
                           &d_k_d1, &d_st_qt, &d_st_d, &d_counts, &d_offsets, &d_sens, &d_sub_qt, &d_sub_d, &d_fix_count, &d_fix_list, &d_tu,
                           &d_tv, &d_cand, &d_cand_count, &d_best, &d_second, &d_cmp_tu, &d_live_idx, &d_row_pair, &d_row_src,
                           &d_vpairs, &d_vpf, &d_vitems, &d_lists, &d_colmask, &d_gtot, &d_grow0, &d_cnt, &d_mrow, &d_summary, &d_overflow,
@@ -628,7 +629,8 @@
     float q8_level = 0.f;
     int q8_direct = 1;
     int q8_route = 1;
-    MsfmRouteKnobs route_knobs() const { return MsfmRouteKnobs{prefilter, q8_route, q8_direct, q8_level}; }
+    int fwd_classes = 1;
+    MsfmRouteKnobs route_knobs() const { return MsfmRouteKnobs{prefilter, q8_route, q8_direct, q8_level, fwd_classes}; }
     DeferredFrees deferred;
     long long cmp_rows_hint = 0;
     long long hint_rows_ub = 0;
diff --git a/monocularsfm_amd/csrc/msfm_hostutil.h b/monocularsfm_amd/csrc/msfm_hostutil.h
--- a/monocularsfm_amd/csrc/msfm_hostutil.h
+++ b/monocularsfm_amd/csrc/msfm_hostutil.h
@@ -1,4 +1,5 @@
 #pragma once
+#include <cmath>
 #include <vector>
 
 #if defined(__HIPCC__)
@@ -25,6 +26,21 @@
 MSFM_HD int msfm_cp_hi(int code) { return code >> 8; }
 MSFM_HD bool msfm_cp_has_second(int code) { return (code & 255) != 255; }
 MSFM_HD int msfm_cp_gap(int code) { const int c = code & 255; return ((16 + (c & 15)) << (c >> 4)) - 16; }
+
+inline float msfm_class_scale(float inv) { return std::nextafter((float)(2.0 / (double)inv * (1.0 + 1e-6)), INFINITY); }
+MSFM_HD float msfm_class_slack(float err_a_max, float err_b_max, float scale) { return (err_a_max + err_b_max) * scale; }
+MSFM_HD float msfm_class_bound(float s1, float slack) {
+    if (!(s1 < 3.0e38f)) return __builtin_huge_valf();
+    const float r = sqrtf(s1 + 2.f) * (1.f + 3e-5f) + slack * (1.f + 3e-5f);
+    return r * r * (1.f + 1e-6f);
+}
+MSFM_HD unsigned msfm_class_mask(const float* cls_s, float s1, float slack) {
+    const float x = msfm_class_bound(s1, slack);
+    if (!(x < 3.0e38f)) return 0xffffffffu;
+    unsigned m = 0;
+    for (int k = 0; k < 32; ++k) m |= (cls_s[k] <= x ? 1u : 0u) << k;
+    return m;
+}
 
 inline std::vector<long long> msfm_pipeline_marks(long long total, long long n_sub, double taper) {
     std::vector<long long> marks;
@@ -53,12 +69,12 @@
     const long long partials = 8LL * n1pad + (route == 3 ? 4LL : 8LL) * (long long)blocks512 * n2pad;
     if (route == 2) return common + partials + 128LL * ((long long)n1 + n2) + 16384;
     const long long bits = blocks512 < 32 ? blocks512 : 32;
-    const long long cmp_rows = ((long long)n1 + (long long)n2 * bits) / (route == 4 ? 8 : 16) + 1024;
+    const long long cmp_rows = ((long long)n1 * (route == 5 ? 7 : 1) + (long long)n2 * bits) / (route == 4 ? 8 : 16) + 1024;
     return common + partials + (route == 3 ? 120LL : 84LL) * cmp_rows;
 }
 
 constexpr float kQ8DirectMaxLevel = 0.625f;
-struct MsfmRouteKnobs { int prefilter, q8_route, q8_direct; float q8_level; };
+struct MsfmRouteKnobs { int prefilter, q8_route, q8_direct; float q8_level; int fwd_classes; };
 inline bool msfm_compact_sweep2(int prune, float ratio) { return prune != 0 && ratio > 0.f && ratio <= 0.95f; }
 inline bool msfm_twin_route_on(const MsfmRouteKnobs& k) { return k.prefilter == 1 && k.q8_route != 0; }
 inline bool msfm_fine_twins(const MsfmRouteKnobs& k) { return k.q8_direct == 2 || (k.q8_direct == 1 && k.q8_level <= kQ8DirectMaxLevel); }
@@ -76,6 +92,7 @@
     MsfmRouteKind kind = kRouteDense;
     std::vector<char> twin;
     long long demoted_pairs = 0;
+    bool fwd_classes = false;
     bool compact() const { return kind != kRouteDense; }
     bool q8() const { return kind >= kRouteQ8Direct; }
 };
@@ -105,6 +122,7 @@
     if (q8 && k.q8_route < 2 && (twin_pairs == 0 || twin_rows < 2 * 1024 * twin_pairs)) q8 = false;
     if (q8) {
         r.kind = mixed ? kRouteQ8Mixed : (fine ? kRouteQ8Direct : kRouteQ8Refine);
+        r.fwd_classes = r.kind == kRouteQ8Direct && k.fwd_classes != 0;
         for (std::size_t p = 0; p < pairs.size(); ++p) r.twin[p] = pairs[p].valid && pairs[p].use && pairs[p].a_twin && pairs[p].b_twin;
         return r;
     }
@@ -120,6 +138,7 @@
     if (!msfm_compact_sweep2(prune, ratio)) return 2;
     if (k.prefilter == 1 && msfm_byte_pair(a_is_u8, b_is_u8)) return 3;
     if (msfm_twin_route_on(k) && k.q8_level > 0.f && !msfm_fine_twins(k)) return 4;
+    if (msfm_twin_route_on(k) && k.q8_level > 0.f && k.fwd_classes != 0) return 5;
     return 1;
 }
 
diff --git a/monocularsfm_amd/csrc/msfm_kernels.hip.h b/monocularsfm_amd/csrc/msfm_kernels.hip.h
--- a/monocularsfm_amd/csrc/msfm_kernels.hip.h
+++ b/monocularsfm_amd/csrc/msfm_kernels.hip.h
@@ -81,7 +81,8 @@
     int a_blk;
     int bt_begin, bt_end;
     int range;
-    int pad[3];
+    int col0, stride;
+    int pad;
 };
 
 struct Top2 {
diff --git a/monocularsfm_amd/csrc/msfm_match.hip b/monocularsfm_amd/csrc/msfm_match.hip
--- a/monocularsfm_amd/csrc/msfm_match.hip
+++ b/monocularsfm_amd/csrc/msfm_match.hip
@@ -143,6 +143,7 @@
     if (const char* e = std::getenv("MSFM_BYTE_DETECT")) ctx->byte_detect = e[0] != '0';
     if (const char* e = std::getenv("MSFM_UPLOAD_THREADS")) ctx->copy_helper = std::atoi(e) != 1;
     if (const char* e = std::getenv("MSFM_Q8_DIRECT")) ctx->q8_direct = e[0] == '2' ? 2 : (e[0] != '0');
+    if (const char* e = std::getenv("MSFM_FWD_CLASSES")) ctx->fwd_classes = e[0] != '0';
     if (const char* e = std::getenv("MSFM_Q8")) ctx->q8_route = e[0] == '2' ? 2 : (e[0] != '0');
     if (const char* e = std::getenv("MSFM_IN_FLIGHT"))
         if (std::atoi(e) >= 1 && std::atoi(e) <= kInFlight) ctx->in_flight = std::atoi(e);
@@ -306,6 +307,9 @@
     to.demoted_pairs += d.demoted_pairs;
     to.mixed_route_sub_batches += d.mixed_route_sub_batches;
     to.memory_shrinks += d.memory_shrinks;
+    to.fwd_class_groups += d.fwd_class_groups;
+    to.sweep2_fwd_descriptor_pairs += d.sweep2_fwd_descriptor_pairs;
+    to.sweep2_rev_descriptor_pairs += d.sweep2_rev_descriptor_pairs;
 }
 
 int drain_streams(msfm_ctx* ctx) {
diff --git a/monocularsfm_amd/csrc/msfm_plan.hip.h b/monocularsfm_amd/csrc/msfm_plan.hip.h
--- a/monocularsfm_amd/csrc/msfm_plan.hip.h
+++ b/monocularsfm_amd/csrc/msfm_plan.hip.h
@@ -11,6 +11,7 @@
     int ranges;
     int b_h0;
     const int* b_n2;
+    int col0, stride;
 };
 
 struct PlanSummary {
@@ -20,6 +21,9 @@
     long long cand_elems;
     long long items_needed;
     long long swept_desc_pairs;
+    long long swept_fwd;
+    int class_groups;
+    int pad;
 };
 
 struct PlanOut {
@@ -58,7 +62,8 @@
                                                         const int* __restrict__ gtot, PlanOut out) {
     MSFM_TAIL_PRIO();
     const int lane = threadIdx.x;
-    long long base_rows = 0, base_cand = 0, tot_swept = 0;
+    long long base_rows = 0, base_cand = 0, tot_swept = 0, tot_fwd = 0;
+    int n_class = 0;
     int carry_f = 0, carry_r = 0;
 #pragma unroll 1
     for (int g0 = 0; g0 < n_groups; g0 += 64) {
@@ -75,6 +80,8 @@
         }
         const int capu = plan_group_cap_units(rows), ablocks = (int)(rows512 / kPfWgRows);
         tot_swept += swept;
+        if (dir == 0) tot_fwd += swept;
+        if (in && rows > 0 && groups[g].stride > 1) n_class += 1;
         const int ir = plan_wave_scan(ablocks), ic = plan_wave_scan(capu);
         int vf = dir == 0 ? items : 0, vr = dir == 1 ? items : 0;
         const int f0 = vf, r0 = vr;
@@ -94,7 +101,11 @@
         carry_r += __shfl(vr, 56 + (lane & 7));
     }
 #pragma unroll
-    for (int d = 1; d < 64; d <<= 1) tot_swept += __shfl_xor(tot_swept, d);
+    for (int d = 1; d < 64; d <<= 1) {
+        tot_swept += __shfl_xor(tot_swept, d);
+        tot_fwd += __shfl_xor(tot_fwd, d);
+        n_class += __shfl_xor(n_class, d);
+    }
     int n_items = carry_f + carry_r;
 #pragma unroll
     for (int d = 1; d < 8; d <<= 1) n_items = max(n_items, __shfl_xor(n_items, d));
@@ -108,6 +119,9 @@
         sm.cand_elems = base_cand * 1024;
         sm.items_needed = n8;
         sm.swept_desc_pairs = tot_swept;
+        sm.swept_fwd = tot_fwd;
+        sm.class_groups = n_class;
+        sm.pad = 0;
         *out.summary = sm;
     }
 }
@@ -169,7 +183,7 @@
     MSFM_PLAN_FENCE();
     out.grow0[g] = ok ? row0 : -1;
     if (!ok) return;
-    const int nblk = G->bt_end - G->bt_begin, ranges = G->ranges, bt0 = G->bt_begin;
+    const int nblk = G->bt_end - G->bt_begin, ranges = G->ranges, bt0 = G->bt_begin, col0 = G->col0, stride = G->stride;
     long long k = out.gpos[3 * (long long)g + 2] + (G->dir == 1 ? out.fwd_items_x[g & 7] : 0);
     for (int rg = 0; rg < ranges; ++rg) {
         const int t0 = bt0 + (int)((long long)nblk * rg / ranges), t1 = bt0 + (int)((long long)nblk * (rg + 1) / ranges);
@@ -180,6 +194,8 @@
             w->bt_begin = t0;
             w->bt_end = t1;
             w->range = rg;
+            w->col0 = col0;
+            w->stride = stride;
         }
     }
 }
@@ -229,7 +245,8 @@
     const _Float16* src = dir ? pp.b_h : pp.a_h;
     const int* n2 = dir ? pp.b_n2 : pp.a_n2;
     const bool with_n2 = cmp_n2 != nullptr && n2 != nullptr;
-    const int bits = dir ? pl.rev_bits : 1, member0 = dir ? pl.rev_member0 : pl.fwd_member;
+    const int bits = dir ? pl.rev_bits : pl.fwd_bits, member0 = dir ? pl.rev_member0 : pl.fwd_member;
+    const bool masked = dir || pl.fwd_bits > 1;
     __shared__ int hist[32];
     __shared__ long long base[32];
     float t4[4], n4[4];
@@ -239,7 +256,7 @@
     for (int j = 0; j < 4; ++j) {
         const int e = e_begin + (int)threadIdx.x + j * 256, ec = e < n ? e : n - 1;
         t4[j] = tuv[off + ec];
-        m4[j] = dir ? colmask[off + ec] : 1u;
+        m4[j] = masked ? colmask[off + ec] : 1u;
         n4[j] = nrm[ec];
         if (with_n2) x4[j] = n2[ec];
         if (e >= n) t4[j] = -f_inf();
diff --git a/monocularsfm_amd/csrc/msfm_prefilter.hip.h b/monocularsfm_amd/csrc/msfm_prefilter.hip.h
--- a/monocularsfm_amd/csrc/msfm_prefilter.hip.h
+++ b/monocularsfm_amd/csrc/msfm_prefilter.hip.h
@@ -42,7 +42,7 @@
     int use;
     int i8;
     int a_h0, b_h0;
-    int pad;
+    float cls_slack;
     const float* a_err;
     const float* b_err;
     const int* a_n2;
@@ -88,7 +88,7 @@
     int fwd_member;
     int rev_member0;
     int rev_bits;
-    int pad;
+    int fwd_bits;
 };
 
 
diff --git a/monocularsfm_amd/csrc/msfm_q8.hip.h b/monocularsfm_amd/csrc/msfm_q8.hip.h
--- a/monocularsfm_amd/csrc/msfm_q8.hip.h
+++ b/monocularsfm_amd/csrc/msfm_q8.hip.h
@@ -5,7 +5,7 @@
 __global__ void pf_prune_q8_kernel(const PairDesc* __restrict__ pairs, const PfPair* __restrict__ pf, const PfPair* __restrict__ pfq,
                                    const float* __restrict__ rp_s0, const float* __restrict__ rp_s1, const float* __restrict__ cp_s0,
                                    unsigned* __restrict__ colmask, float* __restrict__ tuv, PruneParams pr, PlanCounts plan,
-                                   float inv, int direct) {
+                                   float inv, int direct, const unsigned* __restrict__ rp_cls ) {
     MSFM_TAIL_PRIO();
     const PairDesc pd = pairs[blockIdx.y];
     const PfPair pp = pf[blockIdx.y];
@@ -14,7 +14,8 @@
     if (!pq.use) return;
     const int e = blockIdx.x * blockDim.x + threadIdx.x;
     bool row_live = false;
-    unsigned col_bits = 0;
+    unsigned col_bits = 0, row_bits = 0;
+    const bool classes = rp_cls != nullptr && plan.pp_plan != nullptr && plan.pp_plan[blockIdx.y].fwd_bits == 32;
     auto lower = [&](float s0, float err) -> float { return fmaxf(sqrtf(fmaxf(s0, 0.f)) * inv * (1.f - 1e-6f) - err, 0.f); };
     auto upper = [&](float s1, float err) -> float { return sqrtf(s1 + 2.f) * inv * (1.f + 1e-6f) + err; };
     auto dead = [&](float s0, float s1, float err) -> bool {
@@ -34,6 +35,7 @@
     const bool in_r = e < pd.n1pad, in_c = e < pd.n2pad;
     const int er = in_r ? e : 0, ec = in_c ? e : 0;
     const float ld_rs0 = rp_s0[pd.rp_off + er], ld_rs1 = rp_s1[pd.rp_off + er];
+    const unsigned ld_cls = classes ? rp_cls[pd.rp_off + er] : 0u;
     const float ld_aerr = pq.a_err[min(er, pd.n1 - 1)], ld_anrm = pp.a_nrm[er];
     const float ld_berr = pq.b_err[min(ec, pd.n2 - 1)], ld_bnrm = pp.b_nrm[ec];
     int ld_cp[16];
@@ -41,10 +43,12 @@
     for (int p = 0; p < 16; ++p) ld_cp[p] = cpk[pd.cp_off + (long long)min(p, nb - 1) * pd.n2pad + ec];
     if (in_r) {
         float s0 = f_inf(), s1 = f_inf();
+        unsigned cls = ld_cls;
         v2_merge(s0, s1, ld_rs0, ld_rs1);
         for (int p = 1; p < pd.ranges; ++p) {
             const long long o = pd.rp_off + (long long)p * pd.n1pad + e;
             v2_merge(s0, s1, rp_s0[o], rp_s1[o]);
+            if (classes) cls |= rp_cls[o];
         }
         bool live = e < pd.n1;
         const float err = live ? (ld_aerr + pq.b_c) * (1.f + 1e-6f) : 0.f;
@@ -53,6 +57,11 @@
         if (live && direct) T = threshold(upper(s1, err), ld_anrm, pp.b_nrm_max);
         tuv[pp.tu_off + e] = T;
         row_live = live;
+        if (classes) {
+            if (pd.n2 < 32) cls &= (1u << pd.n2) - 1u;
+            row_bits = live ? cls : 0u;
+            colmask[pp.tu_off + e] = row_bits;
+        }
     }
     if (in_c) {
         float s0 = f_inf(), s1 = f_inf();
@@ -99,11 +108,19 @@
     if (plan.pp_plan) {
         const PlanPair pl = plan.pp_plan[blockIdx.y];
         if (pl.fwd_member < 0) return;
-        __shared__ int hist[33];
-        if (threadIdx.x < 33) hist[threadIdx.x] = 0;
+        __shared__ int hist[64];
+        if (threadIdx.x < 64) hist[threadIdx.x] = 0;
         __syncthreads();
-        const unsigned long long rl = __ballot(row_live);
-        if ((threadIdx.x & 63) == 0 && rl) atomicAdd(&hist[32], __popcll(rl));
+        if (classes) {
+            while (row_bits) {
+                const int bit = __builtin_ctz(row_bits);
+                row_bits &= row_bits - 1;
+                atomicAdd(&hist[32 + bit], 1);
+            }
+        } else {
+            const unsigned long long rl = __ballot(row_live);
+            if ((threadIdx.x & 63) == 0 && rl) atomicAdd(&hist[32], __popcll(rl));
+        }
         if (!direct) {
             const unsigned long long cl = __ballot(col_bits != 0u);
             if ((threadIdx.x & 63) == 0 && cl) atomicAdd(&hist[0], __popcll(cl));
@@ -115,11 +132,12 @@
             }
         }
         __syncthreads();
-        if (threadIdx.x == 0 && hist[32]) {
-            atomicAdd(&plan.cnt[pl.fwd_member], hist[32]);
-            atomicAdd(&plan.gtot[plan.member_group[pl.fwd_member]], hist[32]);
+        const int rows_mine = hist[32 + (threadIdx.x & 31)];
+        if ((int)threadIdx.x < pl.fwd_bits && rows_mine) {
+            atomicAdd(&plan.cnt[pl.fwd_member + threadIdx.x], rows_mine);
+            atomicAdd(&plan.gtot[plan.member_group[pl.fwd_member + threadIdx.x]], rows_mine);
         }
-        const int mine = direct ? hist[threadIdx.x < 33 ? threadIdx.x : 0] : hist[0];
+        const int mine = direct ? hist[threadIdx.x < 32 ? threadIdx.x : 0] : hist[0];
         if ((int)threadIdx.x < pl.rev_bits && mine) {
             atomicAdd(&plan.cnt[pl.rev_member0 + threadIdx.x], mine);
             atomicAdd(&plan.gtot[plan.member_group[pl.rev_member0 + threadIdx.x]], mine);
diff --git a/monocularsfm_amd/csrc/msfm_sweep.hip.h b/monocularsfm_amd/csrc/msfm_sweep.hip.h
--- a/monocularsfm_amd/csrc/msfm_sweep.hip.h
+++ b/monocularsfm_amd/csrc/msfm_sweep.hip.h
@@ -62,11 +62,43 @@
     float* thr_w = sThr + wave * (kPfRing * 64);
 
     const unsigned lane_off = (unsigned)(wave * 1024 + lane * 16);
+    const int stride = PASS == 3 ? __builtin_amdgcn_readfirstlane(item.stride > 1 ? item.stride : 1) : 1;
+    const int gcol0 = PASS == 3 ? __builtin_amdgcn_readfirstlane(item.stride > 1 ? item.col0 : 0) : 0;
+    const bool strided = stride > 1;
+    const int last_row = pd.n2pad - 1;
+    auto strided_off = [&](int piece, int tc, bool clamp) -> unsigned {
+        const int g = piece * 64 + lane, r = g / 17, q = g - 17 * r;
+        int row = gcol0 + (tc * kPfBT + r) * stride;
+        if (clamp) row = min(row, last_row);
+        return (unsigned)row * (unsigned)kPfRowBytes + (unsigned)q * 16u;
+    };
+    unsigned soff0 = 0, soff1 = 0, soff2 = 0;
+    if (PASS == 3 && strided) {
+        soff0 = strided_off(wave, 0, false);
+        soff1 = strided_off(wave + 8, 0, false);
+        soff2 = strided_off(16, 0, false);
+    }
     auto dma_tile = [&](int tt) {
         const int tc = tt < t_end ? tt : t_end - 1;
         const int sl = (tt - t_begin) & (kPfRing - 1);
+        char* l = sB + sl * kPfTileBytes + wave * 1024;
+        if (PASS == 3 && strided) {
+            unsigned o0, o1, o2;
+            if ((tc + 1) * kPfBT > pd.n2) {
+                o0 = strided_off(wave, tc, true), o1 = strided_off(wave + 8, tc, true), o2 = strided_off(16, tc, true);
+            } else {
+                const unsigned adv = (unsigned)tc * (unsigned)(kPfBT * kPfRowBytes) * (unsigned)stride;
+                o0 = soff0 + adv, o1 = soff1 + adv, o2 = soff2 + adv;
+            }
+            __builtin_amdgcn_global_load_lds((const __attribute__((address_space(1))) void*)(gB + o0), (__attribute__((address_space(3))) void*)l, 16, 0, 0);
+            __builtin_amdgcn_global_load_lds((const __attribute__((address_space(1))) void*)(gB + o1),
+                                             (__attribute__((address_space(3))) void*)(l + 8192), 16, 0, 0);
+            if (wave == 0)
+                __builtin_amdgcn_global_load_lds((const __attribute__((address_space(1))) void*)(gB + o2),
+                                                 (__attribute__((address_space(3))) void*)(l + 16384), 16, 0, 0);
+            return;
+        }
         const unsigned off = (unsigned)tc * (unsigned)kPfTileBytes + lane_off;
-        char* l = sB + sl * kPfTileBytes + wave * 1024;
         __builtin_amdgcn_global_load_lds((const __attribute__((address_space(1))) void*)(gB + off), (__attribute__((address_space(3))) void*)l, 16, 0, 0);
         __builtin_amdgcn_global_load_lds((const __attribute__((address_space(1))) void*)(gB + (off + 8192u)),
                                          (__attribute__((address_space(3))) void*)(l + 8192), 16, 0, 0);
@@ -229,7 +261,7 @@
         }
         n_buf += __popcll(mm);
     };
-    auto scan_hits3 = [&](const f16v (&a0)[kPfRB], const f16v (&a1)[kPfRB], int col0) {
+    auto scan_hits3 = [&](const f16v (&a0)[kPfRB], const f16v (&a1)[kPfRB], int col0, int col_step) {
         unsigned nm[2] = {0u, 0u};
 #pragma unroll
         for (int blk = 0; blk < 2; ++blk)
@@ -241,7 +273,7 @@
 #pragma unroll 1
         for (int blk = 0; blk < 2; ++blk) {
             unsigned hm = ~(blk ? nm[1] : nm[0]);
-            const int col = col0 + blk * 32;
+            const int col = blk ? col0 + col_step : col0;
             for (unsigned long long mm = __ballot(hm != 0u); mm != 0ull; mm = __ballot(hm != 0u)) {
                 const bool hit = hm != 0u;
                 const int k = __clz((int)hm);
@@ -325,7 +357,17 @@
 #pragma unroll
                     for (int r = 0; r < 16; ++r) rs0[rb][r] = max3f(rs0[rb][r], accA[rb][r], accB[rb][r]);
             } else if (PASS == 3) {
-                scan_hits3(accA, accB, t * kPfBT + lcol);
+                if (strided && (t + 1) * kPfBT > pd.n2) {
+                    const bool v0 = t * kPfBT + lcol < pd.n2, v1 = t * kPfBT + 32 + lcol < pd.n2;
+#pragma unroll
+                    for (int rb = 0; rb < kPfRB; ++rb)
+#pragma unroll
+                        for (int r = 0; r < 16; ++r) {
+                            accA[rb][r] = v0 ? accA[rb][r] : -1.f;
+                            accB[rb][r] = v1 ? accB[rb][r] : -1.f;
+                        }
+                }
+                scan_hits3(accA, accB, gcol0 + (t * kPfBT + lcol) * stride, 32 * stride);
             } else {
                 const float* thr = thr_w + sl * 64;
                 scan_hits2(accA, -0.5f * thr[lcol], t * kPfBT + lcol);
diff --git a/monocularsfm_amd/csrc/msfm_sweep_i8.hip.h b/monocularsfm_amd/csrc/msfm_sweep_i8.hip.h
--- a/monocularsfm_amd/csrc/msfm_sweep_i8.hip.h
+++ b/monocularsfm_amd/csrc/msfm_sweep_i8.hip.h
@@ -31,7 +31,8 @@
     const PairDesc* __restrict__ pairs, const PfPair* __restrict__ pf, const WorkItem* __restrict__ items,
     float* __restrict__ rp_s0, float* __restrict__ rp_s1, float* __restrict__ cp_s0, const float* __restrict__ tu,
     int2* __restrict__ cand, unsigned long long* __restrict__ cand_count, const int* __restrict__ n_items_dev, int n_items_host,
-    int* __restrict__ dyn_next, int* __restrict__ cand_val ) {
+    int* __restrict__ dyn_next, int* __restrict__ cand_val ,
+    unsigned* __restrict__ rp_cls ) {
     static_assert(PASS == 1 || PASS == 3, "sweep 1 and the compacted sweep 2");
     typedef const __attribute__((address_space(1))) float* gfloat_p;
     typedef const __attribute__((address_space(1))) i4v* gi4_p;
@@ -336,7 +337,22 @@
             }
             const long long o = pd.rp_off + (long long)item.range * pd.n1pad + item.a_blk * kPfWgRows + wave * kI8WaveRows + lane;
             rp_s0[o] = m0 > kI8PadTest ? (float)(-2 * (m0 - item_k)) : f_inf();
-            rp_s1[o] = m1 > kI8PadTest ? (float)(-2 * (m1 - item_k)) : f_inf();
+            const float s1 = m1 > kI8PadTest ? (float)(-2 * (m1 - item_k)) : f_inf();
+            rp_s1[o] = s1;
+            if (rp_cls) {
+                const float x = msfm_class_bound(s1, pp.cls_slack);
+                unsigned mask = 0xffffffffu;
+                if (x < 3.0e38f) {
+                    mask = 0u;
+#pragma unroll 8
+                    for (int k = 0; k < 32; ++k) {
+                        const int v = tr[lane * 33 + k];
+                        const bool keep = v > kI8PadTest && (float)(-2 * (v - item_k)) <= x;
+                        mask |= (keep ? 1u : 0u) << k;
+                    }
+                }
+                rp_cls[o] = mask;
+            }
         }
     }
     }
```

Result: slower. 5217 billion (-7.2%).
